# CV-Project2025/Project-NeRF

Hardware: AMD Instinct MI355X
Metric: train rays/sec + 800x800 render FPS, NeRF-Synthetic Lego; PSNR parity (higher is better)
Workload: dtype bf16; 1 GPU; Part 2 vanilla NeRF train step (L10/L4 Fourier, 8x256 skip-4 MLP, view 128), batch sampling included; rays_per_gpu=4096, samples_per_ray=64, global_rays=4096, parallelism=ray-dp1, weights=random init (seed 0), frames=100 x 800x800 RGBA resident in HBM (uniform noise)

## Files before the change

### include/nerf_hip.h

```cpp
#ifndef NERF_HIP_H
#define NERF_HIP_H

#include <stddef.h>
#include <stdint.h>

#ifdef __cplusplus
extern "C" {
#endif

#define NERF_OK 0
#define NERF_EINVAL (-22)
#define NERF_ELAUNCH (-5)
#define NERF_ENOSYS (-38)

#define NERF_ABI_VERSION 4

typedef void* nerf_stream_t;

const char* nerf_last_error(void);
int nerf_abi_version(void);

int nerf_set_option(const char* name, int value);
int nerf_get_option(const char* name, int* value_out);

int nerf_sample_rays(const float* rays_o, const float* rays_d, const float* u,
                     int64_t n_rays, int n_samples, float near_plane, float far_plane,
                     float* z_out, float* pts_out, float* dirs_out, nerf_stream_t stream);

int nerf_gather_rays(const float* images, const float* poses, const int64_t* img_idx, const int64_t* pix_y,
                     const int64_t* pix_x, int64_t batch, int n_images, int H, int W, float focal,
                     float scene_scale, float* rays_o, float* rays_d, float* rgba, nerf_stream_t stream);

int nerf_gather_batch(const float* images, const float* poses, const int64_t* flat_idx, int64_t batch, int n_images,
                      int H, int W, float focal, float scene_scale, const float* bg, float* rays_o, float* rays_d,
                      float* rgba, float* target, nerf_stream_t stream);

int nerf_train_batch(const float* images, const float* poses, int n_images, int H, int W, float focal,
                     float scene_scale, const float* bg, uint64_t seed, uint64_t counter, int64_t batch,
                     int n_samples, float near_plane, float far_plane, int perturb, float* rays_o, float* rays_d,
                     float* rgba, float* target, float* z_out, nerf_stream_t stream);

int nerf_train_batch_shard(const float* images, const float* poses, int n_images, int H, int W, float focal,
                     float scene_scale, const float* bg, uint64_t seed, uint64_t counter, int64_t first_ray, int64_t batch,
                     int n_samples, float near_plane, float far_plane, int perturb, float* rays_o, float* rays_d,
                     float* rgba, float* target, float* z_out, nerf_stream_t stream);

int nerf_active_mask(const float* pts, int64_t n, const uint8_t* binary_grid, int resolution,
                     float bound, uint8_t* mask_out, int64_t* idx_out, nerf_stream_t stream);

int nerf_sample_compact(const float* rays_o, const float* rays_d, const float* u, int64_t n_rays,
                        int n_samples, float near_plane, float far_plane, const uint8_t* binary_grid,
                        int resolution, float bound, float* z_out, int* slot_of_sample, float* pts_compact,
                        float* dirs_compact, unsigned* active_count, nerf_stream_t stream);
int nerf_sample_compact_jitter(const float* rays_o, const float* rays_d, uint64_t seed, uint64_t counter,
                               int64_t n_rays, int n_samples, float near_plane, float far_plane,
                               const uint8_t* binary_grid, int resolution, float bound, float* z_out,
                               int* slot_of_sample, float* pts_compact, float* dirs_compact,
                               unsigned* active_count, nerf_stream_t stream);
int nerf_sample_compact_jitter_shard(const float* rays_o, const float* rays_d, uint64_t seed, uint64_t counter,
                                     int64_t first_ray, int64_t n_rays, int n_samples, float near_plane, float far_plane,
                                     const uint8_t* binary_grid, int resolution, float bound, float* z_out,
                                     int* slot_of_sample, float* pts_compact, float* dirs_compact,
                                     unsigned* active_count, nerf_stream_t stream);
#define NERF_COMPACT_CHAIN_WORDS 40
int nerf_sample_compact_jitter_chain(const float* rays_o, const float* rays_d, uint64_t seed, uint64_t counter,
                                     int64_t first_ray, int64_t n_rays, int n_samples, float near_plane, float far_plane,
                                     const uint8_t* binary_grid, int resolution, float bound, float* z_out,
                                     int* slot_of_sample, float* pts_compact, float* dirs_compact,
                                     unsigned* chain_state, int turn, unsigned* count_host, unsigned seq, nerf_stream_t stream);

size_t nerf_sample_compact_ordered_scratch_bytes(int64_t n_rays, int n_samples);
int nerf_sample_compact_ordered(const float* rays_o, const float* rays_d, const float* u, int draw, uint64_t seed, uint64_t counter,
                                int64_t first_ray, int64_t n_rays, int n_samples, float near_plane, float far_plane,
                                const uint8_t* binary_grid, int resolution, float bound, float* z_out, int* slot_of_sample,
                                float* pts_compact, float* dirs_compact, unsigned* active_count, void* scratch,
                                size_t scratch_bytes, nerf_stream_t stream);

int nerf_sample_pdf(const float* z_coarse, const float* weights, const float* u, int64_t n_rays,
                    int n_coarse, int n_fine, float* z_out, nerf_stream_t stream);

int nerf_grid_lattice(float bound, int resolution, float* pts_out, nerf_stream_t stream);
int nerf_grid_update(const float* sigma, float* grid, uint8_t* binary_grid, int64_t n_cells,
                     float decay, int dynamic, float threshold, unsigned long long* active_count,
                     nerf_stream_t stream);

int nerf_fourier_encode(const float* x, int64_t n, int dim, int n_freq, float* out,
                        nerf_stream_t stream);

int nerf_composite_fwd(const float* rgb, const float* sigma, const float* z, const float* rays_d,
                       const float* bg, int64_t bg_rows, const float* extra,
                       int64_t n_rays, int n_samples,
                       float* out_rgb, float* out_depth, float* out_acc,
                       float* extra_map, float* weights_out, nerf_stream_t stream);

int nerf_composite_bwd(const float* rgb, const float* sigma, const float* z, const float* rays_d,
                       const float* bg, int64_t bg_rows, const float* extra,
                       const float* g_rgb, const float* g_depth, const float* g_acc,
                       const float* g_extra, int64_t n_rays, int n_samples,
                       float* d_rgb, float* d_sigma, float* d_extra, nerf_stream_t stream);

int nerf_composite_fwd_indexed(const float* rgb_compact, const float* sigma_compact, const int* slot_of_sample,
                               const float* z, const float* rays_d, const float* bg, int64_t bg_rows,
                               int64_t n_rays, int n_samples, float* out_rgb, float* out_depth,
                               float* out_acc, nerf_stream_t stream);
int nerf_composite_bwd_indexed(const float* rgb_compact, const float* sigma_compact, const int* slot_of_sample,
                               const float* z, const float* rays_d, const float* bg, int64_t bg_rows,
                               const float* g_rgb, const float* g_depth, const float* g_acc, int64_t n_rays,
                               int n_samples, float* d_rgb_compact, float* d_sigma_compact,
                               nerf_stream_t stream);

#define NERF_MLP_PARAM_COUNT 595844

size_t nerf_mlp_packed_bytes(void);
int nerf_mlp_pack(const float* params_f32, void* packed, nerf_stream_t stream);
int nerf_mlp_pack_streams(const float* params_f32, void* packed, int which, nerf_stream_t stream);

size_t nerf_mlp_stash_bytes(int64_t n);
int nerf_mlp_fwd(const void* packed, const float* rays_o, const float* rays_d, const float* z,
                 int64_t n, int n_samples, float* rgb, float* sigma, void* stash,
                 nerf_stream_t stream);

int nerf_mlp_fwd_encoded(const void* packed, const float* x_enc, const float* d_enc, int64_t n, float* rgb,
                         float* sigma, void* stash, nerf_stream_t stream);

size_t nerf_mlp_bwd_workspace_bytes(int64_t n);
int nerf_mlp_bwd(const void* packed, const void* stash, const float* rgb, const float* sigma,
                 const float* d_rgb, const float* d_sigma, int64_t n, float* grads_f32,
                 void* workspace, nerf_stream_t stream);
int nerf_mlp_bwd_dgrad(const void* packed, const void* stash, const float* rgb, const float* sigma,
                       const float* d_rgb, const float* d_sigma, int64_t n, void* workspace,
                       nerf_stream_t stream);
int nerf_mlp_bwd_dgrad_ex(const void* packed, const void* stash, const float* rgb, const float* sigma,
                          const float* d_rgb, const float* d_sigma, int64_t n, void* workspace,
                          const float* amax_dev, nerf_stream_t stream);
int64_t nerf_mlp_wgrad_part_split(void);
int nerf_mlp_bwd_wgrad_part(const void* stash, const void* workspace, int64_t n, float* grads_f32, int part,
                            nerf_stream_t stream);
int nerf_mlp_bwd_wgrad(const void* stash, const void* workspace, int64_t n, float* grads_f32,
                       nerf_stream_t stream);

int nerf_hash_encode_fwd(const float* pts, int64_t n, const float* table, int n_levels,
                         const float* scale_host, const unsigned* res_host, const unsigned* size_host,
                         const unsigned* offset_host, const unsigned* dense_host, float bound,
                         float* out_f32, void* out_nat_bf16, unsigned* idx_out, nerf_stream_t stream);
int nerf_hash_encode_fwd_f16(const float* pts, int64_t n, const void* table_f16, int n_levels,
                         const float* scale_host, const unsigned* res_host, const unsigned* size_host,
                         const unsigned* offset_host, const unsigned* dense_host, float bound,
                         float* out_f32, void* out_nat_bf16, nerf_stream_t stream);
int nerf_hash_encode_fwd_nat(const float* pts, int64_t n, const float* table_f32, const void* table_f16, int n_levels,
                             const float* scale_host, const unsigned* res_host, const unsigned* size_host,
                             const unsigned* offset_host, const unsigned* dense_host, float bound,
                             void* out_nat, int nat_dtype, nerf_stream_t stream);
int nerf_hash_encode_fwd_nat_tables(const float* pts, int64_t n, const void* tables_f16, int n_tables, int64_t table_stride,
                                    int n_levels, const float* scale_host, const unsigned* res_host, const unsigned* size_host,
                                    const unsigned* offset_host, const unsigned* dense_host, float bound, void* out_nat,
                                    int64_t out_stride_bytes, int nat_dtype, nerf_stream_t stream);
int nerf_f32_to_f16(const float* src, void* dst_f16, int64_t n, nerf_stream_t stream);
int nerf_hash_encode_bwd(const float* pts, int64_t n, int n_levels, const float* scale_host,
                         const unsigned* res_host, const unsigned* size_host, const unsigned* offset_host,
                         const unsigned* dense_host, float bound, const float* d_feat, float* d_table,
                         nerf_stream_t stream);
int nerf_hash_encode_bwd_levels(const float* pts, int64_t n, int n_levels, const float* scale_host,
                         const unsigned* res_host, const unsigned* size_host, const unsigned* offset_host,
                         const unsigned* dense_host, float bound, const float* d_feat, float* d_table, int first_level, int end_level,
                         nerf_stream_t stream);
size_t nerf_hash_encode_bwd_workspace_bytes(int64_t n, int n_levels);
int nerf_hash_encode_bwd_ws(const float* pts, int64_t n, int n_levels, const float* scale_host,
                         const unsigned* res_host, const unsigned* size_host, const unsigned* offset_host,
                         const unsigned* dense_host, float bound, const float* d_feat, float* d_table, int first_level, int end_level,
                         void* workspace, size_t workspace_bytes, nerf_stream_t stream);
int nerf_hash_encode_bwd_ws_store(const float* pts, int64_t n, int n_levels, const float* scale_host,
                                  const unsigned* res_host, const unsigned* size_host, const unsigned* offset_host,
                                  const unsigned* dense_host, float bound, const float* d_feat, float* d_table,
                                  int first_level, int end_level, void* workspace, size_t workspace_bytes,
                                  nerf_stream_t stream);
size_t nerf_hash_encode_bwd_tables_workspace_bytes(int64_t n, int n_levels, int n_tables);
int nerf_hash_encode_bwd_ws_store_tables(const float* pts, int64_t n, int n_tables, int64_t table_stride, int n_levels,
                                         const float* scale_host, const unsigned* res_host, const unsigned* size_host,
                                         const unsigned* offset_host, const unsigned* dense_host, float bound,
                                         const float* d_feat, int64_t dfeat_stride, float* d_table, void* workspace,
                                         size_t workspace_bytes, nerf_stream_t stream);
int nerf_hash_encode_bwd_ws_store_tables_spec(const float* pts, int64_t n, int n_tables, int64_t table_stride, int n_levels,
                                              const float* scale_host, const unsigned* res_host, const unsigned* size_host,
                                              const unsigned* offset_host, const unsigned* dense_host, float bound,
                                              const float* d_feat, int64_t dfeat_stride, float* d_table, void* workspace,
                                              size_t workspace_bytes, void* status_host, nerf_stream_t stream);
int nerf_hash_encode_fwd_f16_hist(const float* pts, int64_t n, const void* table_f16, int n_levels,
                                  const float* scale_host, const unsigned* res_host, const unsigned* size_host,
                                  const unsigned* offset_host, const unsigned* dense_host, float bound,
                                  void* out_nat_bf16, void* bwd_workspace, size_t bwd_workspace_bytes, nerf_stream_t stream);
#define NERF_AMAX_WORDS 32
int nerf_hash_encode_bwd_ws_slots(void* workspace, int64_t n, int n_levels, void** amax_bits_out, void** grad_lm_out);
int nerf_hash_encode_bwd_ws_store_precounted(const float* pts, int64_t n, int n_levels, const float* scale_host,
                                             const unsigned* res_host, const unsigned* size_host,
                                             const unsigned* offset_host, const unsigned* dense_host, float bound,
                                             float* d_table, void* workspace, size_t workspace_bytes, nerf_stream_t stream);
int nerf_hash_encode_bwd_spec_begin(void* workspace, nerf_stream_t stream);
int nerf_hash_encode_bwd_ws_store_spec(const float* pts, int64_t n, int n_levels, const float* scale_host,
                                       const unsigned* res_host, const unsigned* size_host, const unsigned* offset_host,
                                       const unsigned* dense_host, float bound, const float* d_feat, float* d_table, void* workspace,
                                       size_t workspace_bytes, void* status_host, nerf_stream_t stream);
int nerf_imlp_bwd_amax(const void* packed, void* workspace, const float* rgb, const float* sigma, const float* d_rgb,
                       const float* d_sigma, int64_t n, float* grads_f32, float* d_feat, void* amax_bits, nerf_stream_t stream);
const void* nerf_hash_encode_bwd_spec_status(const void* workspace);

int nerf_hash_encode_bwd_input(const float* pts, int64_t n, const float* table, int n_levels,
                               const float* scale_host, const unsigned* res_host, const unsigned* size_host,
                               const unsigned* offset_host, const unsigned* dense_host, float bound,
                               const float* d_feat, float* d_pts, nerf_stream_t stream);
int nerf_hash_encode_bwd_input_f16(const float* pts, int64_t n, const void* table_f16, int n_levels,
                                   const float* scale_host, const unsigned* res_host, const unsigned* size_host,
                                   const unsigned* offset_host, const unsigned* dense_host, float bound,
                                   const float* d_feat, float* d_pts, nerf_stream_t stream);
int nerf_hash_encode_bwd_input_f16_accum(const float* pts, int64_t n, const void* table_f16, int n_levels,
                                         const float* scale_host, const unsigned* res_host, const unsigned* size_host,
                                         const unsigned* offset_host, const unsigned* dense_host, float bound,
                                         const float* d_feat, float* d_pts, nerf_stream_t stream);
int nerf_hash_encode_bwd_input_lm_f16(const float* pts, int64_t n, const void* table_f16, int n_levels,
                                      const float* scale_host, const unsigned* res_host, const unsigned* size_host,
                                      const unsigned* offset_host, const unsigned* dense_host, float bound,
                                      const void* grad_lm, float* d_pts, int accumulate, nerf_stream_t stream);


size_t nerf_imlp_packed_bytes(void);
size_t nerf_imlp_workspace_bytes(int64_t n);
size_t nerf_imlp_hash_operand_offset(int64_t n);
int nerf_imlp_pack(const float* params_f32, void* packed, nerf_stream_t stream);
int nerf_imlp_fwd(const void* packed, void* workspace, const float* dirs, int64_t n, float* rgb,
                  float* sigma, int train, nerf_stream_t stream);
int nerf_imlp_fwd_encoded(const void* packed, void* workspace, const float* x_enc, const float* d_enc, int64_t n,
                          float* rgb, float* sigma, int train, nerf_stream_t stream);
int nerf_imlp_bwd(const void* packed, void* workspace, const float* rgb, const float* sigma,
                  const float* d_rgb, const float* d_sigma, int64_t n, float* grads_f32,
                  float* d_feat, nerf_stream_t stream);
int nerf_imlp_bwd_lm(const void* packed, void* workspace, const float* rgb, const float* sigma,
                     const float* d_rgb, const float* d_sigma, int64_t n, float* grads_f32,
                     void* grad_lm, void* amax_bits, nerf_stream_t stream);

size_t nerf_render_rays_workspace_bytes(int64_t chunk_rays, int n_samples);
int nerf_render_rays_fwd(const void* packed, const float* rays_o, const float* rays_d, int64_t n_rays,
                         int n_samples, float near_plane, float far_plane, const float* bg, int64_t bg_rows,
                         int64_t chunk_rays, void* workspace, float* out_rgb, float* out_depth, float* out_acc,
                         nerf_stream_t stream);

#define NERF_SUM_WS_FLOATS 12288
int nerf_composite_mse_bwd(const float* rgb, const float* sigma, const int* slot_of_sample, const float* z,
                           const float* rays_d, const float* bg, int64_t bg_rows, const float* target,
                           float loss_weight, int64_t n_rays, int n_samples, float* pred_out, float* loss_accum,
                           float* d_rgb, float* d_sigma, float* amax_accum, float* sum_ws, nerf_stream_t stream);
int nerf_composite_mse_reg_bwd(const float* rgb, const float* sigma, const int* slot_of_sample, const float* z,
                               const float* rays_d, const float* bg, int64_t bg_rows, const float* target,
                               float loss_weight, const float* extra, float reg_weight, int64_t n_rays, int n_samples,
                               float* pred_out, float* extra_map, float* loss_accum, float* reg_accum, float* d_rgb,
                               float* d_sigma, float* d_extra, float* sum_ws, nerf_stream_t stream);

int nerf_adam_step(float* params, const float* grads, float* exp_avg, float* exp_avg_sq,
                   int64_t n, int step, float lr, float beta1, float beta2, float eps,
                   float weight_decay, const float* grad_scale_dev, nerf_stream_t stream);

#define NERF_NORMSQ_WS_FLOATS 4136
int nerf_tv_normsq(const float* params, float* grads, int64_t n, float tv_weight, float grad_scale,
                   float* normsq_dev, nerf_stream_t stream);
int nerf_tv_normsq_accum(const float* params, float* grads, int64_t n, float tv_weight, float grad_scale,
                         float* normsq_dev, nerf_stream_t stream);
int nerf_tv_normsq_accum_tables(const float* params, float* grads, int64_t n, int n_tables, float tv_weight, float grad_scale,
                                float* normsq_dev, nerf_stream_t stream);
int nerf_adamw_clip_step(float* params, const float* grads, float* exp_avg, float* exp_avg_sq, int64_t n,
                         int step, float lr, float beta1, float beta2, float eps, float weight_decay,
                         const float* normsq_dev, float max_norm, float grad_scale, nerf_stream_t stream);
int nerf_adamw_clip_step_shadow(float* params, const float* grads, float* exp_avg, float* exp_avg_sq, int64_t n,
                         int step, float lr, float beta1, float beta2, float eps, float weight_decay,
                         const float* normsq_dev, float max_norm, float grad_scale, void* params_f16_out, nerf_stream_t stream);

size_t nerf_tv_codes_bytes(int64_t n);
int nerf_tv_normsq_codes(const float* params, const float* grads, int64_t n, int n_tables, float tv_weight, float grad_scale,
                         float* normsq_dev, int accumulate, void* tv_codes, nerf_stream_t stream);
int nerf_adamw_clip_step_tv(float* params, const float* grads, float* exp_avg, float* exp_avg_sq, int64_t n, int step, float lr,
                            float beta1, float beta2, float eps, float weight_decay, const float* normsq_dev, float max_norm,
                            float grad_scale, const void* tv_codes, int64_t tv_split, float tv_weight_lo, int64_t seg_lo,
                            float tv_weight_hi, int64_t seg_hi, int64_t lr_split, float lr_hi, void* params_f16_out,
                            nerf_stream_t stream);

int nerf_tv_normsq_codes_piece(const float* params, const float* grads, int64_t n, int64_t table_elems, int halo, float tv_weight,
                               float grad_scale, float* normsq_dev, int accumulate, void* tv_codes, nerf_stream_t stream);
int nerf_adamw_clip_step_tv_piece(float* params, const float* grads, float* exp_avg, float* exp_avg_sq, int64_t n, int step, float lr,
                                  float beta1, float beta2, float eps, float weight_decay, const float* normsq_dev, float max_norm,
                                  float grad_scale, const void* tv_codes, float tv_weight, int64_t table_elems, int halo_lo,
                                  void* params_f16_out, nerf_stream_t stream);

int nerf_clip_adamw_small(float* params, float* grads, float* exp_avg, float* exp_avg_sq, int64_t n, int step, float lr, float beta1,
                          float beta2, float eps, float weight_decay, float max_norm, float grad_scale, float* normsq_out,
                          int zero_grads, nerf_stream_t stream);

int64_t nerf_p4_param_count(void);
size_t nerf_p4_packed_bytes(void);
size_t nerf_p4_workspace_bytes(int64_t n);
size_t nerf_p4_workspace_offset(int64_t n, int which);
int nerf_p4_pack(const float* params_f32, void* packed, nerf_stream_t stream);
int nerf_p4_sample_inputs(const int* slot_of_sample, const float* pts_compact, const float* ray_times, int64_t n_rays,
                          int n_samples, float coord_noise_std, float time_noise_std, uint64_t seed, uint64_t counter,
                          int64_t first_ray, float* x_deform, float* t_deform, nerf_stream_t stream);
int nerf_p4_deform_fwd(const void* packed, const float* params_f32, void* workspace, const float* pts, const float* t_deform,
                       const float* blend, int64_t n, float* delta_x, float* x_canonical, int train, nerf_stream_t stream);
int nerf_p4_canon_fwd(const void* packed, void* workspace, const float* t_deform, const float* dirs, int64_t n, float* rgb,
                      float* sigma, int train, nerf_stream_t stream);
int nerf_p4_canon_bwd(const void* packed, void* workspace, const float* rgb, const float* sigma, const float* d_rgb,
                      const float* d_sigma, int64_t n, float* grads_f32, void* amax_bits, void* grad_lm, nerf_stream_t stream);
int nerf_p4_deform_bwd(const void* packed, const float* params_f32, void* workspace, const float* d_delta_x, int64_t n,
                       float* grads_f32, void* amax_bits, void* grad_lm, nerf_stream_t stream);

int64_t nerf_p3_deform_param_count(void);
size_t nerf_p3_deform_packed_bytes(void);
size_t nerf_p3_deform_workspace_bytes(int64_t n);
int nerf_p3_deform_pack(const float* params_f32, void* packed, nerf_stream_t stream);
int nerf_p3_deform_fwd(const void* packed, void* workspace, const float* x_code, const float* pts, const float* t_deform,
                       int64_t n, float* delta_x, float* x_canonical, int train, nerf_stream_t stream);
int nerf_p3_deform_bwd(const void* packed, void* workspace, const float* d_delta_x, int64_t n, float* grads_f32,
                       nerf_stream_t stream);

int64_t nerf_p3_canon_param_count(int time_dim);
size_t nerf_p3_canon_packed_bytes(void);
size_t nerf_p3_canon_workspace_bytes(int64_t n);
int nerf_p3_canon_pack(const float* params_f32, int time_dim, void* packed, nerf_stream_t stream);
int nerf_p3_canon_fwd(const void* packed, void* workspace, const float* x, const float* t, const float* dirs, int64_t n,
                      float* rgb, float* sigma, int train, nerf_stream_t stream);
int nerf_p3_canon_bwd(const void* packed, void* workspace, const float* x, const float* rgb, const float* sigma,
                      const float* d_rgb, const float* d_sigma, int64_t n, int time_dim, float* grads_f32, float* d_x,
                      nerf_stream_t stream);

#ifdef __cplusplus
}
#endif
#endif
```

### project-nerf_amd/_lib.py

```python
import ctypes
import os

_HERE = os.path.dirname(os.path.abspath(__file__))
LIB_PATH = os.path.join(_HERE, "libnerf_hip.so")

c_f32p = ctypes.c_void_p
c_ptr = ctypes.c_void_p
i64 = ctypes.c_int64
i32 = ctypes.c_int
f32 = ctypes.c_float
size_t = ctypes.c_size_t

PROTOTYPES = {
    "nerf_last_error": (ctypes.c_char_p, []),
    "nerf_abi_version": (i32, []),
    "nerf_set_option": (i32, [ctypes.c_char_p, i32]),
    "nerf_get_option": (i32, [ctypes.c_char_p, ctypes.POINTER(i32)]),
    "nerf_sample_rays": (i32, [c_ptr, c_ptr, c_ptr, i64, i32, f32, f32, c_ptr, c_ptr, c_ptr, c_ptr]),
    "nerf_gather_rays": (i32, [c_ptr, c_ptr, c_ptr, c_ptr, c_ptr, i64, i32, i32, i32, f32, f32, c_ptr, c_ptr, c_ptr, c_ptr]),
    "nerf_gather_batch": (i32, [c_ptr, c_ptr, c_ptr, i64, i32, i32, i32, f32, f32, c_ptr, c_ptr, c_ptr, c_ptr, c_ptr, c_ptr]),
    "nerf_train_batch": (i32, [c_ptr, c_ptr, i32, i32, i32, f32, f32, c_ptr, ctypes.c_uint64, ctypes.c_uint64, i64, i32, f32, f32,
                               i32, c_ptr, c_ptr, c_ptr, c_ptr, c_ptr, c_ptr]),
    "nerf_train_batch_shard": (i32, [c_ptr, c_ptr, i32, i32, i32, f32, f32, c_ptr, ctypes.c_uint64, ctypes.c_uint64, i64, i64, i32, f32, f32,
                                     i32, c_ptr, c_ptr, c_ptr, c_ptr, c_ptr, c_ptr]),
    "nerf_active_mask": (i32, [c_ptr, i64, c_ptr, i32, f32, c_ptr, c_ptr, c_ptr]),
    "nerf_sample_compact": (i32, [c_ptr, c_ptr, c_ptr, i64, i32, f32, f32, c_ptr, i32, f32, c_ptr, c_ptr, c_ptr, c_ptr, c_ptr, c_ptr]),
    "nerf_sample_compact_jitter": (i32, [c_ptr, c_ptr, ctypes.c_uint64, ctypes.c_uint64, i64, i32, f32, f32, c_ptr, i32, f32,
                                         c_ptr, c_ptr, c_ptr, c_ptr, c_ptr, c_ptr]),
    "nerf_sample_compact_jitter_shard": (i32, [c_ptr, c_ptr, ctypes.c_uint64, ctypes.c_uint64, i64, i64, i32, f32, f32, c_ptr, i32, f32,
                                               c_ptr, c_ptr, c_ptr, c_ptr, c_ptr, c_ptr]),
    "nerf_sample_compact_jitter_chain": (i32, [c_ptr, c_ptr, ctypes.c_uint64, ctypes.c_uint64, i64, i64, i32, f32, f32, c_ptr, i32, f32,
                                               c_ptr, c_ptr, c_ptr, c_ptr, c_ptr, i32, c_ptr, ctypes.c_uint32, c_ptr]),
    "nerf_composite_fwd_indexed": (i32, [c_ptr, c_ptr, c_ptr, c_ptr, c_ptr, c_ptr, i64, i64, i32, c_ptr, c_ptr, c_ptr, c_ptr]),
    "nerf_composite_bwd_indexed": (i32, [c_ptr, c_ptr, c_ptr, c_ptr, c_ptr, c_ptr, i64, c_ptr, c_ptr, c_ptr, i64, i32, c_ptr, c_ptr, c_ptr]),
    "nerf_sample_pdf": (i32, [c_ptr, c_ptr, c_ptr, i64, i32, i32, c_ptr, c_ptr]),
    "nerf_grid_lattice": (i32, [f32, i32, c_ptr, c_ptr]),
    "nerf_grid_update": (i32, [c_ptr, c_ptr, c_ptr, i64, f32, i32, f32, c_ptr, c_ptr]),
    "nerf_fourier_encode": (i32, [c_ptr, i64, i32, i32, c_ptr, c_ptr]),
    "nerf_composite_fwd": (i32, [c_ptr, c_ptr, c_ptr, c_ptr, c_ptr, i64, c_ptr, i64, i32,
                                 c_ptr, c_ptr, c_ptr, c_ptr, c_ptr, c_ptr]),
    "nerf_composite_bwd": (i32, [c_ptr, c_ptr, c_ptr, c_ptr, c_ptr, i64, c_ptr, c_ptr, c_ptr, c_ptr,
                                 c_ptr, i64, i32, c_ptr, c_ptr, c_ptr, c_ptr]),
    "nerf_render_rays_workspace_bytes": (size_t, [i64, i32]),
    "nerf_render_rays_fwd": (i32, [c_ptr, c_ptr, c_ptr, i64, i32, f32, f32, c_ptr, i64, i64, c_ptr, c_ptr, c_ptr, c_ptr, c_ptr]),
    "nerf_mlp_packed_bytes": (size_t, []),
    "nerf_mlp_pack": (i32, [c_ptr, c_ptr, c_ptr]),
    "nerf_mlp_pack_streams": (i32, [c_ptr, c_ptr, i32, c_ptr]),
    "nerf_mlp_stash_bytes": (size_t, [i64]),
    "nerf_mlp_fwd": (i32, [c_ptr, c_ptr, c_ptr, c_ptr, i64, i32, c_ptr, c_ptr, c_ptr, c_ptr]),
    "nerf_mlp_fwd_encoded": (i32, [c_ptr, c_ptr, c_ptr, i64, c_ptr, c_ptr, c_ptr, c_ptr]),
    "nerf_mlp_bwd_workspace_bytes": (size_t, [i64]),
    "nerf_mlp_bwd": (i32, [c_ptr, c_ptr, c_ptr, c_ptr, c_ptr, c_ptr, i64, c_ptr, c_ptr, c_ptr]),
    "nerf_mlp_bwd_dgrad": (i32, [c_ptr, c_ptr, c_ptr, c_ptr, c_ptr, c_ptr, i64, c_ptr, c_ptr]),
    "nerf_mlp_bwd_wgrad": (i32, [c_ptr, c_ptr, i64, c_ptr, c_ptr]),
    "nerf_mlp_bwd_dgrad_ex": (i32, [c_ptr, c_ptr, c_ptr, c_ptr, c_ptr, c_ptr, i64, c_ptr, c_ptr, c_ptr]),
    "nerf_composite_mse_bwd": (i32, [c_ptr, c_ptr, c_ptr, c_ptr, c_ptr, c_ptr, i64, c_ptr, f32, i64, i32, c_ptr, c_ptr,
                                     c_ptr, c_ptr, c_ptr, c_ptr, c_ptr]),
    "nerf_mlp_wgrad_part_split": (i64, []),
    "nerf_mlp_bwd_wgrad_part": (i32, [c_ptr, c_ptr, i64, c_ptr, i32, c_ptr]),
    "nerf_hash_encode_fwd": (i32, [c_ptr, i64, c_ptr, i32, c_ptr, c_ptr, c_ptr, c_ptr, c_ptr, f32, c_ptr, c_ptr, c_ptr, c_ptr]),
    "nerf_hash_encode_fwd_f16": (i32, [c_ptr, i64, c_ptr, i32, c_ptr, c_ptr, c_ptr, c_ptr, c_ptr, f32, c_ptr, c_ptr, c_ptr]),
    "nerf_hash_encode_fwd_nat": (i32, [c_ptr, i64, c_ptr, c_ptr, i32, c_ptr, c_ptr, c_ptr, c_ptr, c_ptr, f32, c_ptr, i32, c_ptr]),
    "nerf_hash_encode_fwd_nat_tables": (i32, [c_ptr, i64, c_ptr, i32, i64, i32, c_ptr, c_ptr, c_ptr, c_ptr, c_ptr, f32, c_ptr, i64, i32, c_ptr]),
    "nerf_f32_to_f16": (i32, [c_ptr, c_ptr, i64, c_ptr]),
    "nerf_hash_encode_bwd": (i32, [c_ptr, i64, i32, c_ptr, c_ptr, c_ptr, c_ptr, c_ptr, f32, c_ptr, c_ptr, c_ptr]),
    "nerf_hash_encode_bwd_levels": (i32, [c_ptr, i64, i32, c_ptr, c_ptr, c_ptr, c_ptr, c_ptr, f32, c_ptr, c_ptr, i32, i32, c_ptr]),
    "nerf_hash_encode_bwd_workspace_bytes": (size_t, [i64, i32]),
    "nerf_hash_encode_bwd_ws": (i32, [c_ptr, i64, i32, c_ptr, c_ptr, c_ptr, c_ptr, c_ptr, f32, c_ptr, c_ptr, i32, i32, c_ptr, size_t, c_ptr]),
    "nerf_hash_encode_bwd_ws_store": (i32, [c_ptr, i64, i32, c_ptr, c_ptr, c_ptr, c_ptr, c_ptr, f32, c_ptr, c_ptr, i32, i32, c_ptr, size_t, c_ptr]),
    "nerf_hash_encode_bwd_tables_workspace_bytes": (size_t, [i64, i32, i32]),
    "nerf_hash_encode_bwd_ws_store_tables": (i32, [c_ptr, i64, i32, i64, i32, c_ptr, c_ptr, c_ptr, c_ptr, c_ptr, f32, c_ptr, i64, c_ptr, c_ptr, size_t, c_ptr]),
    "nerf_hash_encode_bwd_ws_store_tables_spec": (i32, [c_ptr, i64, i32, i64, i32, c_ptr, c_ptr, c_ptr, c_ptr, c_ptr, f32, c_ptr, i64, c_ptr, c_ptr, size_t,
                                                        c_ptr, c_ptr]),
    "nerf_hash_encode_fwd_f16_hist": (i32, [c_ptr, i64, c_ptr, i32, c_ptr, c_ptr, c_ptr, c_ptr, c_ptr, f32, c_ptr, c_ptr, size_t, c_ptr]),
    "nerf_hash_encode_bwd_ws_slots": (i32, [c_ptr, i64, i32, ctypes.POINTER(c_ptr), ctypes.POINTER(c_ptr)]),
    "nerf_hash_encode_bwd_ws_store_precounted": (i32, [c_ptr, i64, i32, c_ptr, c_ptr, c_ptr, c_ptr, c_ptr, f32, c_ptr, c_ptr, size_t, c_ptr]),
    "nerf_hash_encode_bwd_spec_begin": (i32, [c_ptr, c_ptr]),
    "nerf_hash_encode_bwd_ws_store_spec": (i32, [c_ptr, i64, i32, c_ptr, c_ptr, c_ptr, c_ptr, c_ptr, f32, c_ptr, c_ptr, c_ptr, size_t, c_ptr, c_ptr]),
    "nerf_imlp_bwd_amax": (i32, [c_ptr, c_ptr, c_ptr, c_ptr, c_ptr, c_ptr, i64, c_ptr, c_ptr, c_ptr, c_ptr]),
    "nerf_hash_encode_bwd_spec_status": (c_ptr, [c_ptr]),
    "nerf_imlp_bwd_lm": (i32, [c_ptr, c_ptr, c_ptr, c_ptr, c_ptr, c_ptr, i64, c_ptr, c_ptr, c_ptr, c_ptr]),
    "nerf_hash_encode_bwd_input": (i32, [c_ptr, i64, c_ptr, i32, c_ptr, c_ptr, c_ptr, c_ptr, c_ptr, f32, c_ptr, c_ptr, c_ptr]),
    "nerf_hash_encode_bwd_input_f16": (i32, [c_ptr, i64, c_ptr, i32, c_ptr, c_ptr, c_ptr, c_ptr, c_ptr, f32, c_ptr, c_ptr, c_ptr]),
    "nerf_hash_encode_bwd_input_f16_accum": (i32, [c_ptr, i64, c_ptr, i32, c_ptr, c_ptr, c_ptr, c_ptr, c_ptr, f32, c_ptr, c_ptr, c_ptr]),
    "nerf_hash_encode_bwd_input_lm_f16": (i32, [c_ptr, i64, c_ptr, i32, c_ptr, c_ptr, c_ptr, c_ptr, c_ptr, f32, c_ptr, c_ptr, i32, c_ptr]),
    "nerf_imlp_packed_bytes": (size_t, []),
    "nerf_imlp_workspace_bytes": (size_t, [i64]),
    "nerf_imlp_hash_operand_offset": (size_t, [i64]),
    "nerf_imlp_pack": (i32, [c_ptr, c_ptr, c_ptr]),
    "nerf_imlp_fwd": (i32, [c_ptr, c_ptr, c_ptr, i64, c_ptr, c_ptr, i32, c_ptr]),
    "nerf_imlp_fwd_encoded": (i32, [c_ptr, c_ptr, c_ptr, c_ptr, i64, c_ptr, c_ptr, i32, c_ptr]),
    "nerf_imlp_bwd": (i32, [c_ptr, c_ptr, c_ptr, c_ptr, c_ptr, c_ptr, i64, c_ptr, c_ptr, c_ptr]),
    "nerf_adam_step": (i32, [c_ptr, c_ptr, c_ptr, c_ptr, i64, i32, f32, f32, f32, f32, f32, c_ptr, c_ptr]),
    "nerf_tv_normsq": (i32, [c_ptr, c_ptr, i64, f32, f32, c_ptr, c_ptr]),
    "nerf_tv_normsq_accum": (i32, [c_ptr, c_ptr, i64, f32, f32, c_ptr, c_ptr]),
    "nerf_tv_normsq_accum_tables": (i32, [c_ptr, c_ptr, i64, i32, f32, f32, c_ptr, c_ptr]),
    "nerf_composite_mse_reg_bwd": (i32, [c_ptr, c_ptr, c_ptr, c_ptr, c_ptr, c_ptr, i64, c_ptr, f32, c_ptr, f32, i64, i32, c_ptr, c_ptr,
                                         c_ptr, c_ptr, c_ptr, c_ptr, c_ptr, c_ptr, c_ptr]),
    "nerf_sample_compact_ordered_scratch_bytes": (size_t, [i64, i32]),
    "nerf_sample_compact_ordered": (i32, [c_ptr, c_ptr, c_ptr, i32, ctypes.c_uint64, ctypes.c_uint64, i64, i64, i32, f32, f32, c_ptr, i32, f32,
                                          c_ptr, c_ptr, c_ptr, c_ptr, c_ptr, c_ptr, size_t, c_ptr]),
    "nerf_p4_param_count": (i64, []),
    "nerf_p4_packed_bytes": (size_t, []),
    "nerf_p4_workspace_bytes": (size_t, [i64]),
    "nerf_p4_workspace_offset": (size_t, [i64, i32]),
    "nerf_p4_pack": (i32, [c_ptr, c_ptr, c_ptr]),
    "nerf_p4_sample_inputs": (i32, [c_ptr, c_ptr, c_ptr, i64, i32, f32, f32, ctypes.c_uint64, ctypes.c_uint64, i64, c_ptr, c_ptr, c_ptr]),
    "nerf_p4_deform_fwd": (i32, [c_ptr, c_ptr, c_ptr, c_ptr, c_ptr, c_ptr, i64, c_ptr, c_ptr, i32, c_ptr]),
    "nerf_p4_canon_fwd": (i32, [c_ptr, c_ptr, c_ptr, c_ptr, i64, c_ptr, c_ptr, i32, c_ptr]),
    "nerf_p4_canon_bwd": (i32, [c_ptr, c_ptr, c_ptr, c_ptr, c_ptr, c_ptr, i64, c_ptr, c_ptr, c_ptr, c_ptr]),
    "nerf_p4_deform_bwd": (i32, [c_ptr, c_ptr, c_ptr, c_ptr, i64, c_ptr, c_ptr, c_ptr, c_ptr]),
    "nerf_p3_deform_param_count": (i64, []),
    "nerf_p3_deform_packed_bytes": (size_t, []),
    "nerf_p3_deform_workspace_bytes": (size_t, [i64]),
    "nerf_p3_deform_pack": (i32, [c_ptr, c_ptr, c_ptr]),
    "nerf_p3_deform_fwd": (i32, [c_ptr, c_ptr, c_ptr, c_ptr, c_ptr, i64, c_ptr, c_ptr, i32, c_ptr]),
    "nerf_p3_deform_bwd": (i32, [c_ptr, c_ptr, c_ptr, i64, c_ptr, c_ptr]),
    "nerf_p3_canon_param_count": (i64, [i32]),
    "nerf_p3_canon_packed_bytes": (size_t, []),
    "nerf_p3_canon_workspace_bytes": (size_t, [i64]),
    "nerf_p3_canon_pack": (i32, [c_ptr, i32, c_ptr, c_ptr]),
    "nerf_p3_canon_fwd": (i32, [c_ptr, c_ptr, c_ptr, c_ptr, c_ptr, i64, c_ptr, c_ptr, i32, c_ptr]),
    "nerf_p3_canon_bwd": (i32, [c_ptr, c_ptr, c_ptr, c_ptr, c_ptr, c_ptr, c_ptr, i64, i32, c_ptr, c_ptr, c_ptr]),
    "nerf_tv_codes_bytes": (size_t, [i64]),
    "nerf_tv_normsq_codes": (i32, [c_ptr, c_ptr, i64, i32, f32, f32, c_ptr, i32, c_ptr, c_ptr]),
    "nerf_clip_adamw_small": (i32, [c_ptr, c_ptr, c_ptr, c_ptr, i64, i32, f32, f32, f32, f32, f32, f32, f32, c_ptr, i32, c_ptr]),
    "nerf_adamw_clip_step_tv": (i32, [c_ptr, c_ptr, c_ptr, c_ptr, i64, i32, f32, f32, f32, f32, f32, c_ptr, f32, f32, c_ptr, i64, f32, i64,
                                      f32, i64, i64, f32, c_ptr, c_ptr]),
    "nerf_tv_normsq_codes_piece": (i32, [c_ptr, c_ptr, i64, i64, i32, f32, f32, c_ptr, i32, c_ptr, c_ptr]),
    "nerf_adamw_clip_step_tv_piece": (i32, [c_ptr, c_ptr, c_ptr, c_ptr, i64, i32, f32, f32, f32, f32, f32, c_ptr, f32, f32, c_ptr, f32, i64, i32,
                                            c_ptr, c_ptr]),
    "nerf_adamw_clip_step": (i32, [c_ptr, c_ptr, c_ptr, c_ptr, i64, i32, f32, f32, f32, f32, f32, c_ptr, f32, f32, c_ptr]),
    "nerf_adamw_clip_step_shadow": (i32, [c_ptr, c_ptr, c_ptr, c_ptr, i64, i32, f32, f32, f32, f32, f32, c_ptr, f32, f32, c_ptr, c_ptr]),
}

ABI_VERSION = 4

_lib = None


class NerfHipError(RuntimeError):
    pass


def load():
    global _lib
    if _lib is not None:
        return _lib
    if not os.path.exists(LIB_PATH):
        raise NerfHipError(
            f"{LIB_PATH} not found: build it with `python project-nerf_amd/build.py` "
            "(hipcc --offload-arch=gfx950).  There is no fallback path.")
    import torch
    lib = ctypes.CDLL(LIB_PATH, mode=ctypes.RTLD_GLOBAL)
    for name, (res, args) in PROTOTYPES.items():
        fn = getattr(lib, name)
        fn.restype = res
        fn.argtypes = args
    if lib.nerf_abi_version() != ABI_VERSION:
        raise NerfHipError(f"ABI version mismatch: {LIB_PATH} reports {lib.nerf_abi_version()}, this binding was written against "
                           f"{ABI_VERSION} (rebuild with `python project-nerf_amd/build.py`)")
    _lib = lib
    return lib


NORMSQ_WS_FLOATS = 4136
COMPACT_CHAIN_WORDS = 40
SUM_WS_FLOATS = 12288


def set_option(name: str, value: int) -> None:
    check(load().nerf_set_option(name.encode(), int(value)), f"nerf_set_option({name})")


def get_option(name: str) -> int:
    out = i32(0)
    check(load().nerf_get_option(name.encode(), ctypes.byref(out)), f"nerf_get_option({name})")
    return out.value


def check(code, what):
    if code != 0:
        msg = load().nerf_last_error().decode("utf-8", "replace")
        raise NerfHipError(f"{what} failed ({code}): {msg}")
```

### project-nerf_amd/csrc/adam.hip

```cpp
#include "common.h"

namespace nerf {

typedef float f4 __attribute__((ext_vector_type(4)));

__device__ __forceinline__ void adam_update(float& p, float g, float& m, float& v, float lr, float beta1, float beta2,
                                            float eps, float wd, float inv_bc1, float inv_sqrt_bc2) {
  float pi = p;
  if (wd != 0.0f) pi *= (1.0f - lr * wd);
  const float mi = beta1 * m + (1.0f - beta1) * g;
  const float vi = beta2 * v + (1.0f - beta2) * g * g;
  m = mi;
  v = vi;
  p = pi - (lr * inv_bc1) * (mi / (sqrtf(vi) * inv_sqrt_bc2 + eps));
}

template <bool VEC>
__device__ __forceinline__ void adam_sweep(float* __restrict__ p, const float* __restrict__ g, float* __restrict__ m,
                                           float* __restrict__ v, int64_t n, float gs, float lr, float beta1, float beta2,
                                           float eps, float wd, float inv_bc1, float inv_sqrt_bc2, _Float16* __restrict__ shadow = nullptr) {
  const int64_t tid = blockIdx.x * (int64_t)blockDim.x + threadIdx.x, stride = (int64_t)gridDim.x * blockDim.x;
  const int64_t n4 = VEC ? n / 4 : 0;
  for (int64_t i = tid; i < n4; i += stride) {
    f4 pp = reinterpret_cast<f4*>(p)[i], mm = reinterpret_cast<f4*>(m)[i], vv = reinterpret_cast<f4*>(v)[i];
    const f4 gg = reinterpret_cast<const f4*>(g)[i];
#pragma unroll
    for (int e = 0; e < 4; ++e) {
      float pe = pp[e], me = mm[e], ve = vv[e];
      adam_update(pe, gg[e] * gs, me, ve, lr, beta1, beta2, eps, wd, inv_bc1, inv_sqrt_bc2);
      pp[e] = pe; mm[e] = me; vv[e] = ve;
    }
    reinterpret_cast<f4*>(m)[i] = mm;
    reinterpret_cast<f4*>(v)[i] = vv;
    reinterpret_cast<f4*>(p)[i] = pp;
    if (shadow != nullptr) {
      typedef _Float16 h4 __attribute__((ext_vector_type(4)));
      h4 hh = {(_Float16)pp[0], (_Float16)pp[1], (_Float16)pp[2], (_Float16)pp[3]};
      reinterpret_cast<h4*>(shadow)[i] = hh;
    }
  }
  for (int64_t i = 4 * n4 + tid; i < n; i += stride) {
    adam_update(p[i], g[i] * gs, m[i], v[i], lr, beta1, beta2, eps, wd, inv_bc1, inv_sqrt_bc2);
    if (shadow != nullptr) shadow[i] = (_Float16)p[i];
  }
}

template <bool VEC>
__global__ void __launch_bounds__(256)
adam_kernel(float* __restrict__ p, const float* __restrict__ g, float* __restrict__ m,
            float* __restrict__ v, int64_t n, float lr, float beta1, float beta2, float eps, float wd,
            float inv_bc1, float inv_sqrt_bc2, const float* __restrict__ grad_scale) {
  adam_sweep<VEC>(p, g, m, v, n, grad_scale ? *grad_scale : 1.0f, lr, beta1, beta2, eps, wd, inv_bc1, inv_sqrt_bc2);
}

__host__ inline bool aligned16(const void* a, const void* b, const void* c, const void* d) {
  return (((uintptr_t)a | (uintptr_t)b | (uintptr_t)c | (uintptr_t)d) & 15) == 0;
}

}

extern "C" int nerf_adam_step(float* params, const float* grads, float* exp_avg, float* exp_avg_sq,
                              int64_t n, int step, float lr, float beta1, float beta2, float eps,
                              float weight_decay, const float* grad_scale_dev, nerf_stream_t stream) {
  NERF_REQUIRE(n >= 0 && step >= 1, "nerf_adam_step: n=%lld step=%d", (long long)n, step);
  if (n == 0) return NERF_OK;
  NERF_REQUIRE(params && grads && exp_avg && exp_avg_sq, "nerf_adam_step: NULL pointer");
  const double bc1 = 1.0 - pow((double)beta1, step), bc2 = 1.0 - pow((double)beta2, step);
  int64_t blocks = (n / 4 + 255) / 256 + 1;
  if (blocks > 2048) blocks = 2048;
  if (nerf::aligned16(params, grads, exp_avg, exp_avg_sq))
    hipLaunchKernelGGL(nerf::adam_kernel<true>, dim3((int)blocks), dim3(256), 0, nerf::as_stream(stream), params,
                       grads, exp_avg, exp_avg_sq, n, lr, beta1, beta2, eps, weight_decay,
                       (float)(1.0 / bc1), (float)(1.0 / sqrt(bc2)), grad_scale_dev);
  else
    hipLaunchKernelGGL(nerf::adam_kernel<false>, dim3((int)blocks), dim3(256), 0, nerf::as_stream(stream), params,
                       grads, exp_avg, exp_avg_sq, n, lr, beta1, beta2, eps, weight_decay,
                       (float)(1.0 / bc1), (float)(1.0 / sqrt(bc2)), grad_scale_dev);
  return nerf::check_launch("nerf_adam_step");
}

namespace nerf {

__device__ __forceinline__ float sgn(float x) { return (x > 0.0f) - (x < 0.0f); }

__device__ __forceinline__ float tv_term(float prev, float cur, float next, bool has_prev, bool has_next) {
  float t = 0.0f;
  if (has_prev) t += sgn(cur - prev);
  if (has_next) t -= sgn(next - cur);
  return t;
}

template <bool VEC>
__global__ void __launch_bounds__(256)
tv_normsq_kernel(const float* __restrict__ p, float* __restrict__ g, int64_t n, float tv_scale, float grad_scale,
                 float* __restrict__ normsq, int64_t seg) {
  auto starts = [seg](int64_t e) { return e == 0 || e == seg || e == 2 * seg || e == 3 * seg; };
  const bool rewrite = tv_scale != 0.0f || grad_scale != 1.0f;
  float local = 0.0f;
  const int64_t tid = blockIdx.x * (int64_t)blockDim.x + threadIdx.x, stride = (int64_t)gridDim.x * blockDim.x;
  const int64_t n4 = VEC ? n / 4 : 0;
  for (int64_t i = tid; i < n4; i += stride) {
    f4 gg = reinterpret_cast<f4*>(g)[i];
    gg[0] *= grad_scale; gg[1] *= grad_scale; gg[2] *= grad_scale; gg[3] *= grad_scale;
    if (tv_scale != 0.0f) {
      const f4 pp = reinterpret_cast<const f4*>(p)[i];
      const int64_t e0 = 4 * i;
      const bool has_prev = !starts(e0), has_next = e0 + 4 < n && !starts(e0 + 4);
      const float before = has_prev ? p[e0 - 1] : 0.0f, after = has_next ? p[e0 + 4] : 0.0f;
      gg[0] += tv_scale * tv_term(before, pp[0], pp[1], has_prev, true);
      gg[1] += tv_scale * tv_term(pp[0], pp[1], pp[2], true, true);
      gg[2] += tv_scale * tv_term(pp[1], pp[2], pp[3], true, true);
      gg[3] += tv_scale * tv_term(pp[2], pp[3], after, true, has_next);
    }
    if (rewrite) reinterpret_cast<f4*>(g)[i] = gg;
    local += gg[0] * gg[0] + gg[1] * gg[1] + gg[2] * gg[2] + gg[3] * gg[3];
  }
  for (int64_t i = 4 * n4 + tid; i < n; i += stride) {
    float gi = g[i] * grad_scale;
    if (tv_scale != 0.0f) {
      const bool has_prev = !starts(i), has_next = i + 1 < n && !starts(i + 1);
      gi += tv_scale * tv_term(has_prev ? p[i - 1] : 0.0f, p[i], has_next ? p[i + 1] : 0.0f, has_prev, has_next);
    }
    if (rewrite) g[i] = gi;
    local += gi * gi;
  }
  __shared__ float part[4];
  local = wave_sum(local);
  if ((threadIdx.x & 63) == 0) part[threadIdx.x >> 6] = local;
  __syncthreads();
  const float val[1] = {(part[0] + part[1]) + (part[2] + part[3])};
  float* const out[1] = {normsq};
  ordered_block_sum<1>(val, out, reinterpret_cast<unsigned*>(normsq + 1));
}

template <bool VEC>
__global__ void __launch_bounds__(256)
adamw_clip_kernel(float* __restrict__ p, const float* __restrict__ g, float* __restrict__ m, float* __restrict__ v,
                  int64_t n, float lr, float beta1, float beta2, float eps, float wd, float inv_bc1,
                  float inv_sqrt_bc2, const float* __restrict__ normsq, float max_norm, float extra_scale,
                  _Float16* __restrict__ shadow) {
  float gs = extra_scale;
  if (normsq != nullptr && max_norm > 0.0f) {
    const float coef = max_norm / (sqrtf(*normsq * extra_scale * extra_scale) + 1e-6f);
    gs *= coef < 1.0f ? coef : 1.0f;
  }
  adam_sweep<VEC>(p, g, m, v, n, gs, lr, beta1, beta2, eps, wd, inv_bc1, inv_sqrt_bc2, shadow);
}

__device__ __forceinline__ int tv_code_at(const uint8_t* __restrict__ codes, int64_t i) {
  return i < 0 ? 0 : (int)((codes[i >> 2] >> (2 * (int)(i & 3))) & 3u) - 1;
}

__global__ void __launch_bounds__(256)
tv_normsq_codes_kernel(const float* __restrict__ p, const float* __restrict__ g, int64_t n, float tv_scale, float grad_scale,
                       float* __restrict__ normsq, int64_t seg, uint8_t* __restrict__ codes, int accumulate) {
  auto starts = [seg](int64_t e) { return e == 0 || e == seg || e == 2 * seg || e == 3 * seg; };
  float local = 0.0f;
  const int64_t n4 = (n + 3) / 4;
  for (int64_t q = blockIdx.x * (int64_t)blockDim.x + threadIdx.x; q < n4; q += (int64_t)gridDim.x * blockDim.x) {
    const int64_t e0 = 4 * q;
    float pp[6], gg[4];
#pragma unroll
    for (int e = 0; e < 4; ++e) { pp[1 + e] = e0 + e < n ? p[e0 + e] : 0.0f; gg[e] = e0 + e < n ? g[e0 + e] : 0.0f; }
    if (tv_scale != 0.0f) {
      pp[0] = e0 > 0 ? p[e0 - 1] : 0.0f;
      pp[5] = e0 + 4 < n ? p[e0 + 4] : 0.0f;
      unsigned byte = 0;
      int s_prev = !starts(e0) ? (int)sgn(pp[1] - pp[0]) : 0;
// ... 407 lines not shown
```

### project-nerf_amd/csrc/composite.hip

```cpp
#include "common.h"

namespace nerf {

constexpr int kMaxPerLane = 16;

template <int K>
struct RayCtx {
  float e[K];
  float alpha[K];
  float q[K];
  float T[K];
  float z[K];
  float delta[K];
};

__device__ __forceinline__ int64_t row_of(const int* __restrict__ slots, int64_t dense_index) {
  return slots == nullptr ? dense_index : (int64_t)slots[dense_index];
}

template <int K>
__device__ __forceinline__ void ray_setup(const float* __restrict__ sigma, const float* __restrict__ z,
                                          const float* __restrict__ rays_d, const int* __restrict__ slots,
                                          int64_t r, int S, int lane, RayCtx<K>& c, float* sig_out, int64_t* row_out) {
  const float dx = rays_d[r * 3 + 0], dy = rays_d[r * 3 + 1], dz = rays_d[r * 3 + 2];
// ... 25 lines not shown
    local *= c.q[k];
  }
  const float incl = wave_inclusive_prod(local);
  float run = dpp_row_shr<1>(incl, 1.0f);
  {
    const float p15 = lane_read(incl, 15), p31 = lane_read(incl, 31), p47 = lane_read(incl, 47);
    if (lane == 16) run = p15;
    if (lane == 32) run = p31;
    if (lane == 48) run = p47;
    if (lane == 0) run = 1.0f;
  }
#pragma unroll
  for (int k = 0; k < K; ++k) {
    c.T[k] = run;
    run *= c.q[k];
  }
}

template <int K>
__global__ void __launch_bounds__(256)
composite_fwd_kernel(const float* __restrict__ rgb, const float* __restrict__ sigma,
                     const float* __restrict__ z, const float* __restrict__ rays_d,
                     const float* __restrict__ bg, int64_t bg_rows, const float* __restrict__ extra,
                     const int* __restrict__ slots, int64_t R, int S, float* __restrict__ out_rgb,
                     float* __restrict__ out_depth, float* __restrict__ out_acc, float* __restrict__ extra_map,
                     float* __restrict__ weights_out) {
  const int lane = threadIdx.x & 63;
  const int64_t wave = (blockIdx.x * (int64_t)blockDim.x + threadIdx.x) >> 6;
  const int64_t nwave = ((int64_t)gridDim.x * blockDim.x) >> 6;
  for (int64_t r = wave; r < R; r += nwave) {
    RayCtx<K> c;
    float sg[K];
    int64_t row[K];
    ray_setup<K>(sigma, z, rays_d, slots, r, S, lane, c, sg, row);
    float a0 = 0.f, a1 = 0.f, a2 = 0.f, ad = 0.f, aw = 0.f, x0 = 0.f, x1 = 0.f, x2 = 0.f;
#pragma unroll
    for (int k = 0; k < K; ++k) {
      const int s = lane * K + k;
      if (s < S) {
        const float w = c.alpha[k] * c.T[k];
        if (row[k] >= 0) {
          const float* p = rgb + row[k] * 3;
          a0 += w * p[0];
          a1 += w * p[1];
          a2 += w * p[2];
        }
        ad += w * c.z[k];
        aw += w;
        if (extra != nullptr && row[k] >= 0) {
          const float* q = extra + row[k] * 3;
          x0 += w * q[0];
          x1 += w * q[1];
          x2 += w * q[2];
        }
        if (weights_out != nullptr) weights_out[r * S + s] = w;
      }
    }
    a0 = wave_sum(a0); a1 = wave_sum(a1); a2 = wave_sum(a2);
    ad = wave_sum(ad); aw = wave_sum(aw);
    if (extra != nullptr) { x0 = wave_sum(x0); x1 = wave_sum(x1); x2 = wave_sum(x2); }
    if (lane == 0) {
      if (bg != nullptr) {
        const float* b = bg + (bg_rows > 1 ? r * 3 : 0);
        const float rest = 1.0f - aw;
        a0 += rest * b[0];
        a1 += rest * b[1];
        a2 += rest * b[2];
      }
      out_rgb[r * 3 + 0] = a0;
      out_rgb[r * 3 + 1] = a1;
      out_rgb[r * 3 + 2] = a2;
      out_depth[r] = ad;
      out_acc[r] = aw;
      if (extra_map != nullptr) {
        extra_map[r * 3 + 0] = x0;
        extra_map[r * 3 + 1] = x1;
        extra_map[r * 3 + 2] = x2;
      }
    }
  }
}

template <int K>
__global__ void __launch_bounds__(256)
composite_bwd_kernel(const float* __restrict__ rgb, const float* __restrict__ sigma,
                     const float* __restrict__ z, const float* __restrict__ rays_d,
                     const float* __restrict__ bg, int64_t bg_rows, const float* __restrict__ extra,
                     const float* __restrict__ g_rgb, const float* __restrict__ g_depth,
                     const float* __restrict__ g_acc, const float* __restrict__ g_extra,
                     const int* __restrict__ slots, int64_t R, int S,
                     float* __restrict__ d_rgb, float* __restrict__ d_sigma, float* __restrict__ d_extra) {
  const int lane = threadIdx.x & 63;
  const int64_t wave = (blockIdx.x * (int64_t)blockDim.x + threadIdx.x) >> 6;
  const int64_t nwave = ((int64_t)gridDim.x * blockDim.x) >> 6;
  for (int64_t r = wave; r < R; r += nwave) {
    RayCtx<K> c;
    float sg[K];
    int64_t row[K];
    ray_setup<K>(sigma, z, rays_d, slots, r, S, lane, c, sg, row);
    const float gr0 = g_rgb[r * 3 + 0], gr1 = g_rgb[r * 3 + 1], gr2 = g_rgb[r * 3 + 2];
    const float gd = g_depth ? g_depth[r] : 0.0f;
    float ga = g_acc ? g_acc[r] : 0.0f;
    if (bg != nullptr) {
      const float* b = bg + (bg_rows > 1 ? r * 3 : 0);
      ga -= gr0 * b[0] + gr1 * b[1] + gr2 * b[2];
    }
    float gx0 = 0.f, gx1 = 0.f, gx2 = 0.f;
    if (g_extra != nullptr) { gx0 = g_extra[r * 3 + 0]; gx1 = g_extra[r * 3 + 1]; gx2 = g_extra[r * 3 + 2]; }
    float G[K], w[K];
    float local = 0.0f;
#pragma unroll
    for (int k = 0; k < K; ++k) {
      const int s = lane * K + k;
      G[k] = 0.0f;
      w[k] = 0.0f;
      if (s < S) {
        w[k] = c.alpha[k] * c.T[k];
        float g = gd * c.z[k] + ga;
        if (row[k] >= 0) {
          const float* p = rgb + row[k] * 3;
          g += gr0 * p[0] + gr1 * p[1] + gr2 * p[2];
          float* o = d_rgb + row[k] * 3;
          o[0] = w[k] * gr0;
          o[1] = w[k] * gr1;
          o[2] = w[k] * gr2;
        }
        if (extra != nullptr && g_extra != nullptr && row[k] >= 0) {
          const float* q = extra + row[k] * 3;
          g += gx0 * q[0] + gx1 * q[1] + gx2 * q[2];
          if (d_extra != nullptr) {
            float* oe = d_extra + row[k] * 3;
            oe[0] = w[k] * gx0;
            oe[1] = w[k] * gx1;
            oe[2] = w[k] * gx2;
          }
        }
        G[k] = g;
        local += g * w[k];
      }
    }
    float after = wave_exclusive_suffix_sum(local);
#pragma unroll
    for (int k = K - 1; k >= 0; --k) {
      const int s = lane * K + k;
      if (s < S && row[k] >= 0) {
        const float dalpha = G[k] * c.T[k] - after / c.q[k];
        d_sigma[row[k]] = dalpha * c.delta[k] * c.e[k];
      }
      after += G[k] * w[k];
    }
  }
}

template <int K>
__global__ void __launch_bounds__(256)
composite_mse_bwd_kernel(const float* __restrict__ rgb, const float* __restrict__ sigma, const float* __restrict__ z,
                         const float* __restrict__ rays_d, const float* __restrict__ bg, int64_t bg_rows,
                         const float* __restrict__ target, float loss_weight, const int* __restrict__ slots, int64_t R, int S,
                         float* __restrict__ pred_out, float* __restrict__ loss_out, float* __restrict__ d_rgb,
                         float* __restrict__ d_sigma, float* __restrict__ amax_out,
                         const float* __restrict__ extra, float reg_weight, float* __restrict__ d_extra,
                         float* __restrict__ reg_out, float* __restrict__ extra_map, unsigned* __restrict__ sum_ws) {
  const int lane = threadIdx.x & 63;
  const int64_t wave = (blockIdx.x * (int64_t)blockDim.x + threadIdx.x) >> 6;
  const int64_t nwave = ((int64_t)gridDim.x * blockDim.x) >> 6;
  float loss_local = 0.0f, amax = 0.0f, reg_local = 0.0f;
  for (int64_t r = wave; r < R; r += nwave) {
    RayCtx<K> c;
    float sg[K];
    int64_t row[K];
    ray_setup<K>(sigma, z, rays_d, slots, r, S, lane, c, sg, row);
    float col[K][3], w[K];
    float a0 = 0.f, a1 = 0.f, a2 = 0.f, aw = 0.f;
    float m0 = 0.f, m1 = 0.f, m2 = 0.f;
#pragma unroll
    for (int k = 0; k < K; ++k) {
      const int s = lane * K + k;
      w[k] = 0.0f;
      col[k][0] = col[k][1] = col[k][2] = 0.0f;
      if (s < S) {
        w[k] = c.alpha[k] * c.T[k];
        if (row[k] >= 0) {
          const float* p = rgb + row[k] * 3;
          col[k][0] = p[0]; col[k][1] = p[1]; col[k][2] = p[2];
          a0 += w[k] * p[0]; a1 += w[k] * p[1]; a2 += w[k] * p[2];
          if (extra != nullptr) {
            const float* e = extra + row[k] * 3;
            m0 += w[k] * e[0]; m1 += w[k] * e[1]; m2 += w[k] * e[2];
          }
        }
        aw += w[k];
      }
    }
    a0 = wave_sum(a0); a1 = wave_sum(a1); a2 = wave_sum(a2); aw = wave_sum(aw);
    float gm0 = 0.f, gm1 = 0.f, gm2 = 0.f;
    if (extra != nullptr) {
      m0 = wave_sum(m0); m1 = wave_sum(m1); m2 = wave_sum(m2);
      gm0 = 2.0f * reg_weight * m0; gm1 = 2.0f * reg_weight * m1; gm2 = 2.0f * reg_weight * m2;
      if (lane == 0) {
        reg_local += reg_weight * (m0 * m0 + m1 * m1 + m2 * m2);
        if (extra_map != nullptr) { extra_map[r * 3 + 0] = m0; extra_map[r * 3 + 1] = m1; extra_map[r * 3 + 2] = m2; }
      }
    }
    float b0 = 0.f, b1 = 0.f, b2 = 0.f;
    if (bg != nullptr) {
      const float* b = bg + (bg_rows > 1 ? r * 3 : 0);
      b0 = b[0]; b1 = b[1]; b2 = b[2];
      const float rest = 1.0f - aw;
      a0 += rest * b0; a1 += rest * b1; a2 += rest * b2;
    }
    const float e0 = a0 - target[r * 3 + 0], e1 = a1 - target[r * 3 + 1], e2 = a2 - target[r * 3 + 2];
    if (lane == 0) {
      loss_local += (e0 * e0 + e1 * e1 + e2 * e2) * loss_weight;
      if (pred_out != nullptr) { pred_out[r * 3 + 0] = a0; pred_out[r * 3 + 1] = a1; pred_out[r * 3 + 2] = a2; }
    }
    const float gr0 = 2.0f * e0 * loss_weight, gr1 = 2.0f * e1 * loss_weight, gr2 = 2.0f * e2 * loss_weight;
    const float ga = -(gr0 * b0 + gr1 * b1 + gr2 * b2);
    float G[K], local = 0.0f;
#pragma unroll
    for (int k = 0; k < K; ++k) {
      const int s = lane * K + k;
      G[k] = 0.0f;
      if (s < S) {
        float g = ga;
        if (row[k] >= 0) {
          g += gr0 * col[k][0] + gr1 * col[k][1] + gr2 * col[k][2];
          if (extra != nullptr) {
            const float* e = extra + row[k] * 3;
            g += gm0 * e[0] + gm1 * e[1] + gm2 * e[2];
            float* oe = d_extra + row[k] * 3;
            oe[0] = w[k] * gm0; oe[1] = w[k] * gm1; oe[2] = w[k] * gm2;
          }
          float* o = d_rgb + row[k] * 3;
          const float d0 = w[k] * gr0, d1 = w[k] * gr1, d2 = w[k] * gr2;
          o[0] = d0; o[1] = d1; o[2] = d2;
          if (amax_out != nullptr)
            amax = fmaxf(amax, fmaxf(fabsf(d0 * col[k][0] * (1.0f - col[k][0])),
                                     fmaxf(fabsf(d1 * col[k][1] * (1.0f - col[k][1])), fabsf(d2 * col[k][2] * (1.0f - col[k][2])))));
        }
        G[k] = g;
        local += g * w[k];
      }
    }
    float after = wave_exclusive_suffix_sum(local);
#pragma unroll
    for (int k = K - 1; k >= 0; --k) {
      const int s = lane * K + k;
      if (s < S && row[k] >= 0) {
        const float dalpha = G[k] * c.T[k] - after / c.q[k];
        const float ds = dalpha * c.delta[k] * c.e[k];
        d_sigma[row[k]] = ds;
        if (amax_out != nullptr && sg[k] > 0.0f) amax = fmaxf(amax, fabsf(ds));
      }
      after += G[k] * w[k];
    }
  }
  __shared__ float part[12];
  loss_local = wave_sum(loss_local);
  reg_local = wave_sum(reg_local);
#pragma unroll
  for (int off = 32; off > 0; off >>= 1) amax = fmaxf(amax, __shfl_xor(amax, off));
  if (lane == 0) { part[threadIdx.x >> 6] = loss_local; part[4 + (threadIdx.x >> 6)] = amax; part[8 + (threadIdx.x >> 6)] = reg_local; }
  __syncthreads();
  if (sum_ws != nullptr) {
    if (threadIdx.x == 0) {
      float* ws = reinterpret_cast<float*>(sum_ws);
      ws[blockIdx.x] = (part[0] + part[1]) + (part[2] + part[3]);
      ws[gridDim.x + blockIdx.x] = (part[8] + part[9]) + (part[10] + part[11]);
      ws[2 * gridDim.x + blockIdx.x] = fmaxf(fmaxf(part[4], part[5]), fmaxf(part[6], part[7]));
    }
    return;
  }
  if (threadIdx.x == 0) {
    atomicAdd(loss_out, (part[0] + part[1]) + (part[2] + part[3]));
    if (reg_out != nullptr) atomicAdd(reg_out, (part[8] + part[9]) + (part[10] + part[11]));
    if (amax_out != nullptr) {
      const float m = fmaxf(fmaxf(part[4], part[5]), fmaxf(part[6], part[7]));
      if (m == m && m < 3.0e38f) atomicMax(reinterpret_cast<unsigned*>(amax_out), __builtin_bit_cast(unsigned, m));
    }
  }
}

__global__ void __launch_bounds__(256) composite_sums_kernel(const float* __restrict__ ws, int n_blocks, float* __restrict__ loss_out,
                                                             float* __restrict__ reg_out, float* __restrict__ amax_out) {
  __shared__ float part[3][4];
  float s0 = 0.0f, s1 = 0.0f, m = 0.0f;
  for (int b = threadIdx.x; b < n_blocks; b += 256) {
    s0 += ws[b];
    s1 += ws[n_blocks + b];
    const float v = ws[2 * n_blocks + b];
    if (v == v && v < 3.0e38f) m = fmaxf(m, v);
  }
  s0 = wave_sum(s0);
  s1 = wave_sum(s1);
#pragma unroll
  for (int off = 32; off > 0; off >>= 1) m = fmaxf(m, __shfl_xor(m, off));
  if ((threadIdx.x & 63) == 0) { part[0][threadIdx.x >> 6] = s0; part[1][threadIdx.x >> 6] = s1; part[2][threadIdx.x >> 6] = m; }
  __syncthreads();
  if (threadIdx.x == 0) {
    *loss_out += (part[0][0] + part[0][1]) + (part[0][2] + part[0][3]);
    if (reg_out != nullptr) *reg_out += (part[1][0] + part[1][1]) + (part[1][2] + part[1][3]);
    if (amax_out != nullptr) *amax_out = fmaxf(*amax_out, fmaxf(fmaxf(part[2][0], part[2][1]), fmaxf(part[2][2], part[2][3])));
  }
}

static int per_lane(int S) {
  const int k = (S + 63) / 64;
  return k <= 4 ? k : (k <= 6 ? 6 : (k <= 8 ? 8 : (k <= 12 ? 12 : 16)));
}

}

using namespace nerf;

#define DISPATCH_K(K, KERNEL, ...)                                                        \
  switch (K) {                                                                            \
    case 1: hipLaunchKernelGGL(KERNEL<1>, grid, dim3(256), 0, as_stream(stream), __VA_ARGS__); break; \
    case 2: hipLaunchKernelGGL(KERNEL<2>, grid, dim3(256), 0, as_stream(stream), __VA_ARGS__); break; \
    case 3: hipLaunchKernelGGL(KERNEL<3>, grid, dim3(256), 0, as_stream(stream), __VA_ARGS__); break; \
    case 4: hipLaunchKernelGGL(KERNEL<4>, grid, dim3(256), 0, as_stream(stream), __VA_ARGS__); break; \
    case 6: hipLaunchKernelGGL(KERNEL<6>, grid, dim3(256), 0, as_stream(stream), __VA_ARGS__); break; \
    case 8: hipLaunchKernelGGL(KERNEL<8>, grid, dim3(256), 0, as_stream(stream), __VA_ARGS__); break; \
    case 12: hipLaunchKernelGGL(KERNEL<12>, grid, dim3(256), 0, as_stream(stream), __VA_ARGS__); break; \
    default: hipLaunchKernelGGL(KERNEL<16>, grid, dim3(256), 0, as_stream(stream), __VA_ARGS__); break; \
  }

static int composite_fwd_impl(const float* rgb, const float* sigma, const float* z, const float* rays_d,
                              const float* bg, int64_t bg_rows, const float* extra, const int* slots,
                              int64_t n_rays, int n_samples, float* out_rgb, float* out_depth, float* out_acc,
                              float* extra_map, float* weights_out, nerf_stream_t stream) {
  NERF_REQUIRE(n_rays >= 0 && n_samples >= 1 && n_samples <= 64 * kMaxPerLane,
               "nerf_composite_fwd: n_rays=%lld n_samples=%d (max %d)", (long long)n_rays, n_samples,
               64 * kMaxPerLane);
  if (n_rays == 0) return NERF_OK;
  NERF_REQUIRE(rgb && sigma && z && rays_d && out_rgb && out_depth && out_acc,
               "nerf_composite_fwd: NULL pointer");
  NERF_REQUIRE(bg == nullptr || bg_rows == 1 || bg_rows == n_rays, "nerf_composite_fwd: bg_rows=%lld",
               (long long)bg_rows);
  NERF_REQUIRE((extra == nullptr) == (extra_map == nullptr), "nerf_composite_fwd: extra/extra_map mismatch");
  int64_t blocks = (n_rays + 3) / 4;
  if (blocks > 256 * 8) blocks = 256 * 8;
  const dim3 grid((int)blocks);
  DISPATCH_K(per_lane(n_samples), composite_fwd_kernel, rgb, sigma, z, rays_d, bg, bg_rows, extra, slots, n_rays,
             n_samples, out_rgb, out_depth, out_acc, extra_map, weights_out);
  return check_launch("nerf_composite_fwd");
}

extern "C" int nerf_composite_fwd(const float* rgb, const float* sigma, const float* z,
                                  const float* rays_d, const float* bg, int64_t bg_rows,
                                  const float* extra, int64_t n_rays, int n_samples, float* out_rgb,
                                  float* out_depth, float* out_acc, float* extra_map,
                                  float* weights_out, nerf_stream_t stream) {
  return composite_fwd_impl(rgb, sigma, z, rays_d, bg, bg_rows, extra, nullptr, n_rays, n_samples, out_rgb, out_depth,
                            out_acc, extra_map, weights_out, stream);
}

extern "C" int nerf_composite_fwd_indexed(const float* rgb_compact, const float* sigma_compact, const int* slot_of_sample,
                                          const float* z, const float* rays_d, const float* bg, int64_t bg_rows,
                                          int64_t n_rays, int n_samples, float* out_rgb, float* out_depth,
                                          float* out_acc, nerf_stream_t stream) {
  NERF_REQUIRE(n_rays == 0 || slot_of_sample != nullptr, "nerf_composite_fwd_indexed: slot map is NULL");
  return composite_fwd_impl(rgb_compact, sigma_compact, z, rays_d, bg, bg_rows, nullptr, slot_of_sample, n_rays, n_samples,
                            out_rgb, out_depth, out_acc, nullptr, nullptr, stream);
}

static int composite_bwd_impl(const float* rgb, const float* sigma, const float* z, const float* rays_d,
                              const float* bg, int64_t bg_rows, const float* extra, const float* g_rgb,
                              const float* g_depth, const float* g_acc, const float* g_extra, const int* slots,
                              int64_t n_rays, int n_samples, float* d_rgb, float* d_sigma, float* d_extra,
                              nerf_stream_t stream) {
  NERF_REQUIRE(n_rays >= 0 && n_samples >= 1 && n_samples <= 64 * kMaxPerLane,
               "nerf_composite_bwd: n_rays=%lld n_samples=%d", (long long)n_rays, n_samples);
  if (n_rays == 0) return NERF_OK;
  NERF_REQUIRE(rgb && sigma && z && rays_d && g_rgb && d_rgb && d_sigma, "nerf_composite_bwd: NULL pointer");
  NERF_REQUIRE(bg == nullptr || bg_rows == 1 || bg_rows == n_rays, "nerf_composite_bwd: bg_rows=%lld",
               (long long)bg_rows);
  int64_t blocks = (n_rays + 3) / 4;
  if (blocks > 256 * 8) blocks = 256 * 8;
  const dim3 grid((int)blocks);
  DISPATCH_K(per_lane(n_samples), composite_bwd_kernel, rgb, sigma, z, rays_d, bg, bg_rows, extra, g_rgb,
             g_depth, g_acc, g_extra, slots, n_rays, n_samples, d_rgb, d_sigma, d_extra);
  return check_launch("nerf_composite_bwd");
}

extern "C" int nerf_composite_bwd(const float* rgb, const float* sigma, const float* z,
                                  const float* rays_d, const float* bg, int64_t bg_rows,
                                  const float* extra, const float* g_rgb, const float* g_depth,
                                  const float* g_acc, const float* g_extra, int64_t n_rays,
                                  int n_samples, float* d_rgb, float* d_sigma, float* d_extra,
                                  nerf_stream_t stream) {
  return composite_bwd_impl(rgb, sigma, z, rays_d, bg, bg_rows, extra, g_rgb, g_depth, g_acc, g_extra, nullptr, n_rays,
                            n_samples, d_rgb, d_sigma, d_extra, stream);
}

extern "C" int nerf_composite_bwd_indexed(const float* rgb_compact, const float* sigma_compact, const int* slot_of_sample,
                                          const float* z, const float* rays_d, const float* bg, int64_t bg_rows,
                                          const float* g_rgb, const float* g_depth, const float* g_acc, int64_t n_rays,
                                          int n_samples, float* d_rgb_compact, float* d_sigma_compact,
                                          nerf_stream_t stream) {
  NERF_REQUIRE(n_rays == 0 || slot_of_sample != nullptr, "nerf_composite_bwd_indexed: slot map is NULL");
  return composite_bwd_impl(rgb_compact, sigma_compact, z, rays_d, bg, bg_rows, nullptr, g_rgb, g_depth, g_acc, nullptr,
                            slot_of_sample, n_rays, n_samples, d_rgb_compact, d_sigma_compact, nullptr, stream);
}

static int64_t mse_blocks(int64_t n_rays, bool partials) {
  int n_cu = 256;
  (void)device_cu_count(&n_cu);
  const int per_cu = partials ? 8 : (options().composite_wgs_per_cu < 1 ? 1 : options().composite_wgs_per_cu);
  int64_t cap = (int64_t)n_cu * per_cu;
  if (cap > kOrderedSumMaxBlocks) cap = kOrderedSumMaxBlocks;
  const int64_t blocks = (n_rays + 3) / 4;
  return blocks < cap ? blocks : cap;
}
static int finish_sums(const float* sum_ws, unsigned n_blocks, float* loss, float* reg, float* amax, nerf_stream_t stream) {
  static_assert(NERF_SUM_WS_FLOATS >= 3 * kOrderedSumMaxBlocks, "three partials per workgroup");
  if (sum_ws == nullptr) return NERF_OK;
  hipLaunchKernelGGL(composite_sums_kernel, dim3(1), dim3(256), 0, as_stream(stream), sum_ws, (int)n_blocks, loss, reg, amax);
  return check_launch("nerf_composite_mse_bwd (sums)");
}

extern "C" int nerf_composite_mse_bwd(const float* rgb, const float* sigma, const int* slot_of_sample, const float* z,
                                      const float* rays_d, const float* bg, int64_t bg_rows, const float* target,
                                      float loss_weight, int64_t n_rays, int n_samples, float* pred_out, float* loss_accum,
                                      float* d_rgb, float* d_sigma, float* amax_accum, float* sum_ws, nerf_stream_t stream) {
  NERF_REQUIRE(n_rays >= 0 && n_samples >= 1 && n_samples <= 64 * kMaxPerLane,
               "nerf_composite_mse_bwd: n_rays=%lld n_samples=%d (max %d)", (long long)n_rays, n_samples, 64 * kMaxPerLane);
  if (n_rays == 0) return NERF_OK;
  NERF_REQUIRE(rgb && sigma && z && rays_d && target && loss_accum && d_rgb && d_sigma, "nerf_composite_mse_bwd: NULL pointer");
  NERF_REQUIRE(bg == nullptr || bg_rows == 1 || bg_rows == n_rays, "nerf_composite_mse_bwd: bg_rows=%lld", (long long)bg_rows);
  const dim3 grid((unsigned)mse_blocks(n_rays, sum_ws != nullptr));
  DISPATCH_K(per_lane(n_samples), composite_mse_bwd_kernel, rgb, sigma, z, rays_d, bg, bg_rows, target, loss_weight,
             slot_of_sample, n_rays, n_samples, pred_out, loss_accum, d_rgb, d_sigma, amax_accum,
             (const float*)nullptr, 0.0f, (float*)nullptr, (float*)nullptr, (float*)nullptr, reinterpret_cast<unsigned*>(sum_ws));
  if (int rc = check_launch("nerf_composite_mse_bwd"); rc != NERF_OK) return rc;
  return finish_sums(sum_ws, grid.x, loss_accum, nullptr, amax_accum, stream);
}

extern "C" int nerf_composite_mse_reg_bwd(const float* rgb, const float* sigma, const int* slot_of_sample, const float* z,
                                          const float* rays_d, const float* bg, int64_t bg_rows, const float* target,
                                          float loss_weight, const float* extra, float reg_weight, int64_t n_rays, int n_samples,
                                          float* pred_out, float* extra_map, float* loss_accum, float* reg_accum, float* d_rgb,
                                          float* d_sigma, float* d_extra, float* sum_ws, nerf_stream_t stream) {
  NERF_REQUIRE(n_rays >= 0 && n_samples >= 1 && n_samples <= 64 * kMaxPerLane,
               "nerf_composite_mse_reg_bwd: n_rays=%lld n_samples=%d (max %d)", (long long)n_rays, n_samples, 64 * kMaxPerLane);
  if (n_rays == 0) return NERF_OK;
  NERF_REQUIRE(rgb && sigma && z && rays_d && target && loss_accum && d_rgb && d_sigma && extra && d_extra && reg_accum,
               "nerf_composite_mse_reg_bwd: NULL pointer");
  NERF_REQUIRE(bg == nullptr || bg_rows == 1 || bg_rows == n_rays, "nerf_composite_mse_reg_bwd: bg_rows=%lld", (long long)bg_rows);
  const dim3 grid((unsigned)mse_blocks(n_rays, sum_ws != nullptr));
  DISPATCH_K(per_lane(n_samples), composite_mse_bwd_kernel, rgb, sigma, z, rays_d, bg, bg_rows, target, loss_weight,
             slot_of_sample, n_rays, n_samples, pred_out, loss_accum, d_rgb, d_sigma, (float*)nullptr, extra, reg_weight, d_extra,
             reg_accum, extra_map, reinterpret_cast<unsigned*>(sum_ws));
  if (int rc = check_launch("nerf_composite_mse_reg_bwd"); rc != NERF_OK) return rc;
  return finish_sums(sum_ws, grid.x, loss_accum, reg_accum, nullptr, stream);
}
```

### project-nerf_amd/csrc/mlp_bwd.hip

```cpp
#include "mlp_chain.h"
#include "mlp_stash.h"

namespace nerf {
using namespace plan;

struct BwdArgs {
  const char* packed;
  const float* rgb;
  const float* sigma;
  const float* d_rgb;
  const float* d_sigma;
  int64_t n, n_pad;
  const uint4* st_mask;
  __bf16* dsmall;
  __bf16* dhv;
  __bf16* dfeat;
  __bf16* dh;
  float* amax;
  const float* amax_src;
};

__device__ __forceinline__ void out_derivs(const BwdArgs& a, int64_t n, float& g0, float& g1, float& g2, float& gs) {
  const float r0 = a.rgb[n * 3 + 0], r1 = a.rgb[n * 3 + 1], r2 = a.rgb[n * 3 + 2];
  g0 = a.d_rgb[n * 3 + 0] * r0 * (1.0f - r0);
  g1 = a.d_rgb[n * 3 + 1] * r1 * (1.0f - r1);
  g2 = a.d_rgb[n * 3 + 2] * r2 * (1.0f - r2);
  gs = a.sigma[n] > 0.0f ? a.d_sigma[n] : 0.0f;
}

__global__ void __launch_bounds__(256) bwd_amax_kernel(const BwdArgs a) {
  float m = 0.0f;
  for (int64_t n = blockIdx.x * 256 + threadIdx.x; n < a.n; n += (int64_t)gridDim.x * 256) {
    float g0, g1, g2, gs;
    out_derivs(a, n, g0, g1, g2, gs);
    m = fmaxf(fmaxf(m, fabsf(g0)), fmaxf(fmaxf(fabsf(g1), fabsf(g2)), fabsf(gs)));
  }
#pragma unroll
  for (int off = 32; off > 0; off >>= 1) m = fmaxf(m, __shfl_xor(m, off));
  __shared__ float part[4];
  if ((threadIdx.x & 63) == 0) part[threadIdx.x >> 6] = m;
  __syncthreads();
  if (threadIdx.x == 0) {
    m = fmaxf(fmaxf(part[0], part[1]), fmaxf(part[2], part[3]));
    if (m == m && m < 3.0e38f) atomicMax(reinterpret_cast<unsigned*>(a.amax), __builtin_bit_cast(unsigned, m));
  }
}

__global__ void __launch_bounds__(kChainThreads, 2) mlp_bwd_kernel(const BwdArgs a) {
  extern __shared__ __attribute__((aligned(16))) char smem[];
  const int tid = threadIdx.x, lane = tid & 63;
  const int wave = __builtin_amdgcn_readfirstlane(tid >> 6);
  const int col = lane & 31, half = lane >> 5;

  WeightRing<true> ring;
  ring.init(a.packed + kPackBwdOff, smem + kBiasLdsBytes, wave, lane);
  ring.prologue();
  const char* a_base = nullptr;

  const int64_t n_tiles = a.n_pad / kTileSamples;
  for (int64_t tile = blockIdx.x; tile < n_tiles; tile += gridDim.x) {
    const bool more = tile + gridDim.x < n_tiles;
    const int64_t wave_tile = tile * 8 + wave;
    const int64_t n = wave_tile * kWaveSamples + col;
    const bool live = n < a.n;

    float g0 = 0.f, g1 = 0.f, g2 = 0.f, gs = 0.f;
    if (live) out_derivs(a, n, g0, g1, g2, gs);
    bf16x8 small;
#pragma unroll
    for (int j = 0; j < 8; ++j) small[j] = (__bf16)0.0f;
    if (half == 0) {
      small[0] = (__bf16)g0; small[1] = (__bf16)g1; small[2] = (__bf16)g2; small[3] = (__bf16)gs;
    }
    stash_nat(a.dsmall, wave_tile, 1, 0, col, half, small);

    uint4 mask;
    auto load_mask = [&](int layer) { mask = a.st_mask[(tile * 9 + layer) * kChainThreads + tid]; };
    auto grad_epi = [&](bf16x8* out, __bf16* stash, int width, bool masked) {
      return [=, &mask](auto mc, f32x16 acc) {
        constexpr int m = decltype(mc)::value;
        if (masked) {
          const uint32_t words[4] = {mask.x, mask.y, mask.z, mask.w};
          const uint32_t bits = words[m >> 1] >> (16 * (m & 1));
#pragma unroll
          for (int r = 0; r < 16; ++r) acc[r] = (bits >> r) & 1u ? acc[r] : 0.0f;
        }
        acc_to_operand(acc, out[2 * m], out[2 * m + 1]);
        stash_block(stash, wave_tile, width / 32, m, col, half, out[2 * m], out[2 * m + 1]);
      };
    };

    bf16x8 gA[16], gB[16];
    {
      bf16x8 in[1];
      in[0] = small;
      if (half == 0) in[0][3] = (__bf16)0.0f;
      load_mask(8);
      run_step<true, B_RGB, 1, true>(ring, a_base, more, in, nullptr, half, grad_epi(gA, a.dhv, 128, true));
    }
    {
      bf16x8 in[8];
#pragma unroll
      for (int i = 0; i < 8; ++i) in[i] = gA[i];
      run_step<true, B_VIEW, 8, true>(ring, a_base, more, in, nullptr, half, grad_epi(gB, a.dfeat, 256, false));
    }
    {
      bf16x8 in[17];
#pragma unroll
      for (int i = 0; i < 16; ++i) in[i] = gB[i];
#pragma unroll
      for (int j = 0; j < 8; ++j) in[16][j] = (__bf16)0.0f;
      if (half == 0) in[16][0] = (__bf16)gs;
      load_mask(7);
      run_step<true, B_HEAD, 17, true>(ring, a_base, more, in, nullptr, half, grad_epi(gA, a.dh + 7 * a.n_pad * 256, 256, true));
    }
    load_mask(6);
    run_step<true, B_PTS7, 16, true>(ring, a_base, more, gA, nullptr, half, grad_epi(gB, a.dh + 6 * a.n_pad * 256, 256, true));
    load_mask(5);
    run_step<true, B_PTS6, 16, true>(ring, a_base, more, gB, nullptr, half, grad_epi(gA, a.dh + 5 * a.n_pad * 256, 256, true));
    load_mask(4);
    run_step<true, B_PTS5, 16, true>(ring, a_base, more, gA, nullptr, half, grad_epi(gB, a.dh + 4 * a.n_pad * 256, 256, true));
    load_mask(3);
    run_step<true, B_PTS4, 16, true>(ring, a_base, more, gB, nullptr, half, grad_epi(gA, a.dh + 3 * a.n_pad * 256, 256, true));
    load_mask(2);
    run_step<true, B_PTS3, 16, true>(ring, a_base, more, gA, nullptr, half, grad_epi(gB, a.dh + 2 * a.n_pad * 256, 256, true));
    load_mask(1);
    run_step<true, B_PTS2, 16, true>(ring, a_base, more, gB, nullptr, half, grad_epi(gA, a.dh + 1 * a.n_pad * 256, 256, true));
    load_mask(0);
    run_step<true, B_PTS1, 16, true>(ring, a_base, more, gA, nullptr, half, grad_epi(gB, a.dh + 0 * a.n_pad * 256, 256, true));
  }
}

}

#include <stddef.h>
#include "mlp_stream_asm.h"

namespace nerf {

static_assert(offsetof(BwdArgs, n_pad) == 48 && offsetof(BwdArgs, st_mask) == 56 && offsetof(BwdArgs, dhv) == 72 &&
              offsetof(BwdArgs, dfeat) == 80 && offsetof(BwdArgs, dh) == 88, "kernarg offsets used by the stream asm");

template <bool IMG16>
__global__ void __launch_bounds__(kChainThreads, 2) mlp_bwd_stream_kernel(const BwdArgs a) {
  extern __shared__ __attribute__((aligned(16))) char smem[];
  const int tid = threadIdx.x, lane = tid & 63;
  const int wave = __builtin_amdgcn_readfirstlane(tid >> 6);
  const int col = lane & 31, half = lane >> 5;

  WeightRing<true> ring;
  ring.init(a.packed + kPackBwdOff, smem + kBiasLdsBytes, wave, lane);
  ring.template issue<0>(0);
  ring.template issue<1>(1);
  asm volatile("s_waitcnt vmcnt(0)" ::: "memory");
  __syncthreads();

  const unsigned ab0 = lds_addr(smem + kBiasLdsBytes) + 16u * lane, ab1 = ab0 + kRingSlotBytes;
  const unsigned ldsw = __builtin_amdgcn_readfirstlane(lds_addr(smem + kBiasLdsBytes) + 1024u * wave);
  const unsigned voff = 1024u * wave + 16u * lane;
  const char* src = a.packed + kPackBwdOff;
  const void* karg = (const void*)__builtin_amdgcn_kernarg_segment_ptr();

  float gscale = 1.0f;
  if constexpr (!IMG16) {
    set_fp8_saturate();
    const float amax_in = *a.amax_src;
    if (a.amax_src != a.amax && blockIdx.x == 0 && tid == 0) *a.amax = amax_in;
    gscale = __builtin_bit_cast(float, __builtin_amdgcn_readfirstlane(__builtin_bit_cast(int, grad_image_scale(amax_in))));
  }
  const int64_t n_tiles = a.n_pad / kTileSamples;
  for (int64_t tile = blockIdx.x; tile < n_tiles; tile += gridDim.x) {
    const int64_t wave_tile = tile * 8 + wave;
    const int64_t n = wave_tile * kWaveSamples + col;
    const bool live = n < a.n;
    float g0 = 0.f, g1 = 0.f, g2 = 0.f, gs = 0.f;
    if (live) out_derivs(a, n, g0, g1, g2, gs);
    bf16x8 small, in_rgb, in_sigma;
#pragma unroll
    for (int j = 0; j < 8; ++j) small[j] = in_sigma[j] = (__bf16)0.0f;
    if (half == 0) {
      small[0] = (__bf16)g0; small[1] = (__bf16)g1; small[2] = (__bf16)g2; small[3] = (__bf16)gs;
      in_sigma[0] = (__bf16)gs;
    }
    if constexpr (IMG16) stash_nat(a.dsmall, wave_tile, 1, 0, col, half, small);
    else stash_nat8<true>(reinterpret_cast<char*>(a.dsmall), wave_tile, 1, 0, col, half, small, gscale);
    in_rgb = small;
    in_rgb[3] = (__bf16)0.0f;

    const unsigned lane32 = IMG16 ? block_lane_offset(col, half) : block8_lane_offset(col, half);
    const unsigned blk = IMG16 ? 2048u : 1024u;
    const unsigned so8 = (unsigned)wave_tile * (8u * blk) + lane32, so4 = (unsigned)wave_tile * (4u * blk) + lane32;
    const unsigned mo0 = (unsigned)tile * (72u * 512u * 2u) + 2u * tid;
    const bool more = tile + gridDim.x < n_tiles;
    const unsigned mo0n = more ? (unsigned)(tile + gridDim.x) * (72u * 512u * 2u) + 2u * tid : mo0;
    const unsigned first = __builtin_amdgcn_readfirstlane(tile == (int64_t)blockIdx.x ? 1u : 0u);
    if constexpr (IMG16) bwd16_stream_pass(ab0, ab1, in_rgb, in_sigma, src, voff, ldsw, so8, so4, mo0, mo0n, first, karg, gscale);
    else bwd_stream_pass(ab0, ab1, in_rgb, in_sigma, src, voff, ldsw, so8, so4, mo0, mo0n, first, karg, gscale);
  }
  asm volatile("s_waitcnt vmcnt(0)" ::: "memory");
}

}

using namespace nerf;

int nerf_launch_wgrad(const char* stash, const StashLayout& sl, const char* work, const BwdLayout& bl,
                      int64_t n, float* grads, int part, hipStream_t stream, size_t zero_lo, size_t zero_hi);

extern "C" size_t nerf_mlp_bwd_workspace_bytes(int64_t n) { return n > 0 ? bwd_layout(n).total : 0; }

static int launch_dgrad(const void* packed, const void* stash, const float* rgb, const float* sigma,
                        const float* d_rgb, const float* d_sigma, int64_t n, void* workspace,
                        const float* amax_dev, nerf_stream_t stream) {
  NERF_REQUIRE(n > 0 && n < (int64_t)1 << 31, "nerf_mlp_bwd: n=%lld out of range", (long long)n);
  NERF_REQUIRE(packed && stash && rgb && sigma && d_rgb && d_sigma && workspace, "nerf_mlp_bwd: NULL pointer");
  NERF_REQUIRE(((uintptr_t)packed & 255) == 0 && ((uintptr_t)stash & 255) == 0 && ((uintptr_t)workspace & 255) == 0,
               "nerf_mlp_bwd: packed/stash/workspace must be 256-byte aligned");
  const StashLayout sl = stash_layout(n);
  const BwdLayout bl = bwd_layout(n);
  BwdArgs a{};
  a.packed = static_cast<const char*>(packed);
  a.rgb = rgb; a.sigma = sigma; a.d_rgb = d_rgb; a.d_sigma = d_sigma;
  a.n = n; a.n_pad = bl.n_pad;
  a.st_mask = reinterpret_cast<const uint4*>(static_cast<const char*>(stash) + sl.mask);
  char* w = static_cast<char*>(workspace);
  a.dsmall = reinterpret_cast<__bf16*>(w + bl.dsmall);
  a.dhv = reinterpret_cast<__bf16*>(w + bl.dhv);
  a.dfeat = reinterpret_cast<__bf16*>(w + bl.dfeat);
  a.dh = reinterpret_cast<__bf16*>(w + bl.dh);
  a.amax = reinterpret_cast<float*>(w + bl.amax);
  a.amax_src = amax_dev != nullptr ? amax_dev : a.amax;
  int n_cu = 0;
  if (int rc = device_cu_count(&n_cu); rc != NERF_OK) return rc;
  const bool stream_family = chain_use_stream(n, true);
  const void* kernel = stream_family ? (bl.fp8 ? (const void*)mlp_bwd_stream_kernel<false> : (const void*)mlp_bwd_stream_kernel<true>)
                                     : (const void*)mlp_bwd_kernel;
  if (int rc = ensure_dynamic_lds(kernel, kChainLds, "nerf_mlp_bwd"); rc != NERF_OK) return rc;
  const int64_t tiles = bl.n_pad / kTileSamples;
  if (options().chain_grid > 0 && options().chain_grid < n_cu) n_cu = options().chain_grid;
  const int grid = (int)(tiles < n_cu ? tiles : n_cu);
  if (bl.fp8 && amax_dev == nullptr) {
    if (hipMemsetAsync(a.amax, 0, sizeof(float), as_stream(stream)) != hipSuccess)
      return fail(NERF_ELAUNCH, "nerf_mlp_bwd: memset failed");
    const int64_t want = (n + 1023) / 1024;
    hipLaunchKernelGGL(bwd_amax_kernel, dim3((int)(want < 1024 ? want : 1024)), dim3(256), 0, as_stream(stream), a);
  }
  if (stream_family && bl.fp8)
    hipLaunchKernelGGL(mlp_bwd_stream_kernel<false>, dim3(grid), dim3(kChainThreads), kChainLds, as_stream(stream), a);
  else if (stream_family)
    hipLaunchKernelGGL(mlp_bwd_stream_kernel<true>, dim3(grid), dim3(kChainThreads), kChainLds, as_stream(stream), a);
  else
    hipLaunchKernelGGL(mlp_bwd_kernel, dim3(grid), dim3(kChainThreads), kChainLds, as_stream(stream), a);
  return check_launch("nerf_mlp_bwd (dgrad chain)");
}

static int launch_wgrad(const void* stash, const void* workspace, int64_t n, float* grads_f32, int part,
                        nerf_stream_t stream) {
  NERF_REQUIRE(grads_f32 != nullptr, "nerf_mlp_bwd: grads_f32 is NULL");
  NERF_REQUIRE(part >= 0 && part <= 2, "nerf_mlp_bwd_wgrad_part: part=%d (0 all, 1 late layers, 2 early layers)", part);
  const size_t lo = part == 1 ? (size_t)plan::kW4 : 0, hi = part == 2 ? (size_t)plan::kW4 : (size_t)plan::kParamCount;
  if (n == 0) {
    if (hipMemsetAsync(grads_f32 + lo, 0, sizeof(float) * (hi - lo), as_stream(stream)) != hipSuccess)
      return fail(NERF_ELAUNCH, "nerf_mlp_bwd: memset failed");
    return NERF_OK;
  }
  NERF_REQUIRE(stash && workspace, "nerf_mlp_bwd: NULL pointer");
  return nerf_launch_wgrad(static_cast<const char*>(stash), stash_layout(n), static_cast<const char*>(workspace),
                           bwd_layout(n), n, grads_f32, part, as_stream(stream), lo, hi);
}

extern "C" int nerf_mlp_bwd_dgrad(const void* packed, const void* stash, const float* rgb, const float* sigma,
                                  const float* d_rgb, const float* d_sigma, int64_t n, void* workspace,
                                  nerf_stream_t stream) {
  if (n == 0) return NERF_OK;
  return launch_dgrad(packed, stash, rgb, sigma, d_rgb, d_sigma, n, workspace, nullptr, stream);
}

extern "C" int nerf_mlp_bwd_dgrad_ex(const void* packed, const void* stash, const float* rgb, const float* sigma,
                                     const float* d_rgb, const float* d_sigma, int64_t n, void* workspace,
                                     const float* amax_dev, nerf_stream_t stream) {
  if (n == 0) return NERF_OK;
  return launch_dgrad(packed, stash, rgb, sigma, d_rgb, d_sigma, n, workspace, amax_dev, stream);
}

extern "C" int nerf_mlp_bwd_wgrad(const void* stash, const void* workspace, int64_t n, float* grads_f32,
                                  nerf_stream_t stream) {
  return launch_wgrad(stash, workspace, n, grads_f32, 0, stream);
}

extern "C" int64_t nerf_mlp_wgrad_part_split(void) { return plan::kW4; }

extern "C" int nerf_mlp_bwd_wgrad_part(const void* stash, const void* workspace, int64_t n, float* grads_f32, int part,
                                       nerf_stream_t stream) {
  return launch_wgrad(stash, workspace, n, grads_f32, part, stream);
}

extern "C" int nerf_mlp_bwd(const void* packed, const void* stash, const float* rgb, const float* sigma,
                            const float* d_rgb, const float* d_sigma, int64_t n, float* grads_f32,
                            void* workspace, nerf_stream_t stream) {
  NERF_REQUIRE(n >= 0, "nerf_mlp_bwd: n=%lld", (long long)n);
  if (n > 0) {
    const int rc = launch_dgrad(packed, stash, rgb, sigma, d_rgb, d_sigma, n, workspace, nullptr, stream);
    if (rc != NERF_OK) return rc;
  }
  return launch_wgrad(stash, workspace, n, grads_f32, 0, stream);
}
```

### project-nerf_amd/csrc/mlp_pack.hip

```cpp
#include "common.h"
#include "mlp_plan.h"

namespace nerf {
using namespace plan;

struct FragTable {
  int v[kFwdFrags + kBwdFrags];
};

constexpr FragTable make_frag_table() {
  FragTable t{};
  int f = 0;
  for (int kind = 0; kind < kNumKinds; ++kind) {
    const int ks = step_ks(kind);
    for (int m = 0; m < step_of(kind).mt; ++m)
      for (int k = 0; k < ks; ++k) t.v[f++] = (kind << 16) | (m << 8) | k;
  }
  return t;
}
__constant__ FragTable g_frag_table = make_frag_table();

__device__ __forceinline__ int src_index(int kind, int row, int k, bool nat) {
  if (kind <= F_PTS7) {
    const int l = kind;
    const int in_dim = pts_in_dim(l);
    int col;
    if (l == 0) col = k < 63 ? k : -1;
    else if (l == 4) col = nat ? (k < 63 ? 256 + k : -1) : k;
    else col = k;
    return col < 0 ? -1 : pts_weight_off(l) + row * in_dim + col;
  }
  switch (kind) {
    case F_HEAD: return row < 256 ? kWFeat + row * 256 + k : (row == 256 ? kWSigma + k : -1);
    case F_VIEW: return nat ? (k < 27 ? kWView + row * 283 + 256 + k : -1) : kWView + row * 283 + k;
    case F_RGB: return row < 3 ? kWRgb + row * 128 + k : -1;
    case B_RGB: return k < 3 ? kWRgb + k * 128 + row : -1;
    case B_VIEW: return kWView + k * 283 + row;
    case B_HEAD: return nat ? (k == 0 ? kWSigma + row : -1) : kWFeat + k * 256 + row;
    default: {
      const int l = 7 - (kind - B_PTS7);
      return pts_weight_off(l) + k * pts_in_dim(l) + row;
    }
  }
}

__global__ void __launch_bounds__(256) pack16_kernel(const float* __restrict__ params, __bf16* __restrict__ packed_fwd16) {
  const int total = kFwdFrags * 64;
  for (int t = blockIdx.x * blockDim.x + threadIdx.x; t < total; t += gridDim.x * blockDim.x) {
    const int frag = t >> 6, lane = t & 63;
    const int desc = g_frag_table.v[frag];
    const int kind = desc >> 16, mt = (desc >> 8) & 0xFF, ks = desc & 0xFF;
    const Step st = step_of(kind);
    const int row = mt * 32 + 16 * (ks & 1) + (lane & 15), q = lane >> 4;
    const bool nat = ks >= st.ks_acc;
    const int kk = nat ? (ks - st.ks_acc) >> 1 : ks >> 1;
    typedef __bf16 bf16x8 __attribute__((ext_vector_type(8)));
    bf16x8 out;
#pragma unroll
    for (int j = 0; j < 8; ++j) {
      const int k = nat ? 32 * kk + 8 * q + j : 32 * kk + 16 * (j >> 2) + 4 * q + (j & 3);
      const int src = src_index(kind, row, k, nat);
      out[j] = (__bf16)(src >= 0 ? params[src] : 0.0f);
    }
    *reinterpret_cast<bf16x8*>(packed_fwd16 + (size_t)frag * 512 + lane * 8) = out;
  }
}

__global__ void __launch_bounds__(256)
pack_kernel(const float* __restrict__ params, __bf16* __restrict__ packed_fwd,
            __bf16* __restrict__ packed_bwd, float* __restrict__ bias) {
  const int total = (kFwdFrags + kBwdFrags) * 64;
  for (int t = blockIdx.x * blockDim.x + threadIdx.x; t < total; t += gridDim.x * blockDim.x) {
    const int frag = t >> 6, lane = t & 63;
    const int desc = g_frag_table.v[frag];
    const int kind = desc >> 16, mt = (desc >> 8) & 0xFF, ks = desc & 0xFF;
    const Step st = step_of(kind);
    const int row = mt * 32 + (lane & 31), h = lane >> 5;
    const bool nat = ks >= st.ks_acc;
    typedef __bf16 bf16x8 __attribute__((ext_vector_type(8)));
    bf16x8 out;
#pragma unroll
    for (int j = 0; j < 8; ++j) {
      int k;
      if (nat) k = 16 * (ks - st.ks_acc) + 8 * h + j;
      else k = 32 * (ks >> 1) + 16 * (ks & 1) + 8 * (j >> 2) + 4 * h + (j & 3);
      const int src = src_index(kind, row, k, nat);
      out[j] = (__bf16)(src >= 0 ? params[src] : 0.0f);
    }
    __bf16* dst = frag < kFwdFrags ? packed_fwd + (size_t)frag * 512 : packed_bwd + (size_t)(frag - kFwdFrags) * 512;
    *reinterpret_cast<bf16x8*>(dst + lane * 8) = out;
  }
  for (int i = blockIdx.x * blockDim.x + threadIdx.x; i < kBiasFloats; i += gridDim.x * blockDim.x) {
    float b = 0.0f;
    if (i < 2048) b = params[pts_bias_off(i >> 8) + (i & 255)];
    else if (i < 2048 + 288) { const int r = i - 2048; b = r < 256 ? params[kBFeat + r] : (r == 256 ? params[kBSigma] : 0.0f); }
    else if (i < 2048 + 288 + 128) b = params[kBView + (i - 2048 - 288)];
    else { const int r = i - 2048 - 288 - 128; b = r < 3 ? params[kBRgb + r] : 0.0f; }
    bias[i] = b;
  }
}

}

extern "C" size_t nerf_mlp_packed_bytes(void) { return nerf::plan::kPackBytes; }

extern "C" int nerf_mlp_pack_streams(const float* params_f32, void* packed, int which, nerf_stream_t stream) {
  using namespace nerf;
  NERF_REQUIRE(params_f32 && packed, "nerf_mlp_pack: NULL pointer");
  NERF_REQUIRE(((uintptr_t)packed & 255) == 0, "nerf_mlp_pack: packed buffer must be 256-byte aligned");
  NERF_REQUIRE(which >= 1 && which <= 3, "nerf_mlp_pack_streams: which=%d (1 training streams + biases, 2 inference stream, 3 all)", which);
  char* base = static_cast<char*>(packed);
  if (which & 1)
    hipLaunchKernelGGL(pack_kernel, dim3(512), dim3(256), 0, as_stream(stream), params_f32,
                       reinterpret_cast<__bf16*>(base + plan::kPackFwdOff),
                       reinterpret_cast<__bf16*>(base + plan::kPackBwdOff),
                       reinterpret_cast<float*>(base + plan::kPackBiasOff));
  if (which & 2)
    hipLaunchKernelGGL(pack16_kernel, dim3(304), dim3(256), 0, as_stream(stream), params_f32,
                       reinterpret_cast<__bf16*>(base + plan::kPackFwd16Off));
  return check_launch("nerf_mlp_pack");
}

extern "C" int nerf_mlp_pack(const float* params_f32, void* packed, nerf_stream_t stream) {
  return nerf_mlp_pack_streams(params_f32, packed, 3, stream);
}
```

### project-nerf_amd/csrc/mlp_wgrad.h

```cpp
#pragma once
#include <hip/hip_runtime.h>
#include <stdint.h>

namespace nerf {

constexpr int kMaxJobs = 12;
constexpr int kWgStages = 4;
constexpr int kWgStageA = 16 * 1024, kWgStageB = 16 * 1024, kWgStageN = 4 * 1024;
constexpr int kWgStageBytes = kWgStageA + kWgStageB + kWgStageN;
constexpr int kWgLds = kWgStages * kWgStageBytes;
constexpr int kWgScratch = 256;
constexpr int kMaxTiles = 10;
constexpr size_t kSmallSlabBytes = 8u << 20;

struct WgradJob {
  const char* a;
  const char* b_acc;
  const char* b_nat;
  int a_bytes;
  int b_acc_bytes, b_nat_bytes;
  int a_nat;
  int mt_a;
  int nt_acc, nt_nat, ones;
  int split_n;
  int kind;
  int w_off, w_ld;
  int o_row0, o_valid;
  int acc_valid, acc_col0;
  int nat_valid, nat_col0;
  int bias_off, bias_nat_col;
  const char* a2;
  int w2_off, bias2_off, o2_row, n2;
  long long cost0;
  int cost;
  long long slab_off;
  int part0, n_parts, p_stride;
};

struct WgradArgs {
  WgradJob jobs[kMaxJobs];
  int n_jobs;
  int wave_tiles;
  long long total_cost;
  float* grads;
  float* slab;
  int slab_accumulate;
  const float* amax;
  int k16;
  int debug;
};


int wgrad_launch(WgradArgs& args, int64_t n_samples, float* grads, hipStream_t stream, float* slab = nullptr,
                 size_t slab_bytes = 0, size_t zero_lo = 0, size_t zero_hi = 0);

}
```

### project-nerf_amd/csrc/mlp_wgrad.hip

```cpp
#include <stdlib.h>
#include "mlp_chain.h"
#include "mlp_stash.h"
#include "mlp_wgrad.h"

namespace nerf {
using namespace plan;

typedef short s16x4 __attribute__((ext_vector_type(4)));
typedef short s16x8 __attribute__((ext_vector_type(8)));
typedef __attribute__((address_space(3))) s16x4* lds_s16x4_t;

__device__ __forceinline__ void dma_1k(const char* gsrc_lane, unsigned lds_dst) {
  unsigned keep;
  asm volatile("s_mov_b32 %0, m0\n\ts_mov_b32 m0, %2\n\ts_nop 0\n\tglobal_load_lds_dwordx4 %1, off nt\n\ts_mov_b32 m0, %0"
               : "=&s"(keep) : "v"(gsrc_lane), "s"(lds_dst) : "memory");
}

template <int STRIDE>
__device__ __forceinline__ bf16x8 tr_frag(const char* p) {
  const s16x4 lo = __builtin_amdgcn_ds_read_tr16_b64_v4i16((lds_s16x4_t)(p));
  const s16x4 hi = __builtin_amdgcn_ds_read_tr16_b64_v4i16((lds_s16x4_t)(p + STRIDE));
  s16x8 v = {lo[0], lo[1], lo[2], lo[3], hi[0], hi[1], hi[2], hi[3]};
  return __builtin_bit_cast(bf16x8, v);
}
// ... 495 lines not shown
      continue;
    }
#pragma unroll
    for (int s = 0; s < 2; ++s) {
      bf16x8 af = SPLIT ? tr_frag<128>(pa + 512 * s) : tr_frag<256>(pa + 1024 * s);
      if (SPLIT && g.fhalf) {
#pragma unroll
        for (int e = 0; e < 8; ++e) af[e] = (__bf16)0.0f;
      }
      if constexpr (SPLIT) {
        if (wave < NT_ACC) acc[0] = __builtin_amdgcn_mfma_f32_32x32x16_bf16(af, tr_frag<256>(pb + 1024 * s), acc[0], 0, 0, 0);
        if (ONES && wave == NT_ACC % 8) acc[1] = __builtin_amdgcn_mfma_f32_32x32x16_bf16(af, ones, acc[1], 0, 0, 0);
      } else {
        bf16x8 bf[NT_ACC + NT_NAT + 1];
#pragma unroll
        for (int k = 0; k < NT_ACC; ++k) bf[k] = tr_frag<256>(pb + k * 2048 + 1024 * s);
#pragma unroll
        for (int k = 0; k < NT_NAT; ++k) bf[NT_ACC + k] = tr_frag<128>(pn + k * 2048 + 512 * s);
        bf[NT_ACC + NT_NAT] = ones;
#pragma unroll
        for (int k = 0; k < NT; ++k) acc[k] = __builtin_amdgcn_mfma_f32_32x32x16_bf16(af, bf[k], acc[k], 0, 0, 0);
        __builtin_amdgcn_sched_group_barrier(0x100, 2 * (1 + NT_ACC + NT_NAT), 0);
        __builtin_amdgcn_sched_group_barrier(0x008, NT, 0);
        __builtin_amdgcn_sched_barrier(0);
      }
    }
  }

  flush_tiles<NT_ACC, NT_NAT, ONES, SPLIT, FP8, NT>(args, job, acc, g, active);
}

template <bool FP8>
__global__ void __launch_bounds__(512, 2) mlp_wgrad_kernel(const WgradArgs args) {
  extern __shared__ __attribute__((aligned(16))) char smem[];
  LaneGeo g;
  g.lane = threadIdx.x & 63;
  g.wave = __builtin_amdgcn_readfirstlane(threadIdx.x >> 6);
  const int grp = g.lane >> 4, i16 = g.lane & 15, q = i16 >> 2, p = i16 & 3;
  const int hh = grp >> 1;
  g.fhalf = grp & 1;
  g.off_acc = 512 * hh + 128 * g.fhalf + 64 * (p & 1) + 16 * q + 8 * (p >> 1);
  g.off_nat = 32 * (8 * hh + q) + 16 * (p >> 1) + 8 * (p & 1) + 1024 * g.fhalf;
  const int q8 = i16 >> 1, p8 = i16 & 1;
  g.off_acc8 = 256 * hh + 32 * q8 + 16 * g.fhalf + 8 * p8;
  g.off_nat8 = 512 * g.fhalf + 16 * (8 * hh + q8) + 8 * p8;

  const long long lo = args.total_cost * blockIdx.x / gridDim.x;
  const long long hi = args.total_cost * (blockIdx.x + 1) / gridDim.x;
  for (int j = 0; j < args.n_jobs; ++j) {
    const WgradJob job = args.jobs[j];
    const long long j0 = job.cost0, j1 = job.cost0 + (long long)job.cost * args.wave_tiles;
    if (hi <= j0 || lo >= j1) continue;
    const long long a0 = lo > j0 ? lo - j0 : 0, a1 = (hi < j1 ? hi : j1) - j0;
    const int wt0 = (int)((a0 + job.cost - 1) / job.cost), wt1 = (int)((a1 + job.cost - 1) / job.cost);
    if (wt0 >= wt1) continue;
    if constexpr (FP8) {
      switch (job.kind) {
        case 0: run_job8<8, 0, true>(args, job, wt0, wt1, smem, g); break;
        case 1: run_job8<8, 2, false>(args, job, wt0, wt1, smem, g); break;
        case 2: run_job8<0, 2, false>(args, job, wt0, wt1, smem, g); break;
        case 3: run_job8<8, 1, false>(args, job, wt0, wt1, smem, g); break;
        case 4: run_job<8, 0, true, true, true>(args, job, wt0, wt1, smem, g); break;
        default: run_job<4, 0, true, true, true>(args, job, wt0, wt1, smem, g); break;
      }
    } else {
    switch (job.kind) {
      case 0: run_job16<16, 16, 0, 8, 0, true, false>(args, job, wt0, wt1, smem, g); break;
      case 1: run_job16<16, 16, 4, 8, 2, false, false>(args, job, wt0, wt1, smem, g); break;
      case 2: run_job16<16, 0, 4, 0, 2, false, false>(args, job, wt0, wt1, smem, g); break;
      case 3: run_job16<8, 16, 2, 8, 1, false, false>(args, job, wt0, wt1, smem, g); break;
      case 4: run_job16<1, 16, 0, 8, 0, true, true>(args, job, wt0, wt1, smem, g); break;
      case 5: run_job16<1, 8, 0, 4, 0, true, true>(args, job, wt0, wt1, smem, g); break;
      case 13: run_job16<16, 16, 0, 8, 0, true, false, true>(args, job, wt0, wt1, smem, g); break;
      case 14: run_job16<16, 0, 6, 0, 3, false, false, false, NatStage>(args, job, wt0, wt1, smem, g); break;
      case 6: run_job<0, 1, false, false, false>(args, job, wt0, wt1, smem, g); break;
      case 7: run_job<2, 0, false, false, false>(args, job, wt0, wt1, smem, g); break;
      case 8: run_job<1, 1, false, false, false>(args, job, wt0, wt1, smem, g); break;
      default: run_job<2, 0, false, true, false>(args, job, wt0, wt1, smem, g); break;
    }
    }
  }
}

template <bool P4>
__global__ void __launch_bounds__(512, P4 ? 4 : 6) mlp_wgrad_small_kernel(const WgradArgs args) {
  using Stage = std::conditional_t<P4, SmallStageP4, SmallStage>;
  extern __shared__ __attribute__((aligned(16))) char smem[];
  LaneGeo g;
  g.lane = threadIdx.x & 63;
  g.wave = __builtin_amdgcn_readfirstlane(threadIdx.x >> 6);
  const int grp = g.lane >> 4, i16 = g.lane & 15, q = i16 >> 2, p = i16 & 3;
  const int hh = grp >> 1;
  g.fhalf = grp & 1;
  g.off_acc = 512 * hh + 128 * g.fhalf + 64 * (p & 1) + 16 * q + 8 * (p >> 1);
  g.off_nat = 32 * (8 * hh + q) + 16 * (p >> 1) + 8 * (p & 1) + 1024 * g.fhalf;
  g.off_acc8 = g.off_nat8 = 0;
  const long long lo = args.total_cost * blockIdx.x / gridDim.x;
  const long long hi = args.total_cost * (blockIdx.x + 1) / gridDim.x;
  for (int j = 0; j < args.n_jobs; ++j) {
    const WgradJob job = args.jobs[j];
    const long long j0 = job.cost0, j1 = job.cost0 + (long long)job.cost * args.wave_tiles;
    if (hi <= j0 || lo >= j1) continue;
    const long long a0 = lo > j0 ? lo - j0 : 0, a1 = (hi < j1 ? hi : j1) - j0;
    const int wt0 = (int)((a0 + job.cost - 1) / job.cost), wt1 = (int)((a1 + job.cost - 1) / job.cost);
    if (wt0 >= wt1) continue;
    if constexpr (P4) {
      switch (job.kind) {
        case 10: run_job16<4, 4, 0, 2, 0, true, false, false, Stage>(args, job, wt0, wt1, smem, g); continue;
        case 11: run_job16<4, 4, 2, 2, 1, false, false, false, Stage>(args, job, wt0, wt1, smem, g); continue;
        case 12: run_job16<4, 0, 4, 0, 2, false, false, false, Stage>(args, job, wt0, wt1, smem, g); continue;
        default: break;
      }
    }
    switch (job.kind) {
      case 6: run_job16<4, 0, 2, 0, 1, false, false, false, Stage>(args, job, wt0, wt1, smem, g); break;
      case 7:
        if (job.mt_a == 2) run_job16<4, 4, 0, 2, 0, false, false, false, Stage>(args, job, wt0, wt1, smem, g);
        else run_job16<2, 4, 0, 2, 0, false, false, false, Stage>(args, job, wt0, wt1, smem, g);
        break;
      case 8: run_job16<4, 2, 2, 1, 1, false, false, false, Stage>(args, job, wt0, wt1, smem, g); break;
      default: run_job16<1, 4, 0, 2, 0, false, true, false, Stage>(args, job, wt0, wt1, smem, g); break;
    }
  }
}

__global__ void __launch_bounds__(256) wgrad_reduce_kernel(const WgradArgs args) {
  const WgradJob& job = args.jobs[blockIdx.y];
  const int n_w = job.o_valid * job.w_ld, n_b = n_w + job.o_valid, n_all = n_b + job.n2;
  const float* tile = args.slab + job.slab_off;
  for (int i = blockIdx.x * blockDim.x + threadIdx.x; i < n_all; i += gridDim.x * blockDim.x) {
    float s0 = 0.0f, s1 = 0.0f, s2 = 0.0f, s3 = 0.0f;
    int t = 0;
    for (; t + 4 <= job.n_parts; t += 4) {
      s0 += tile[(long long)(t + 0) * job.p_stride + i];
      s1 += tile[(long long)(t + 1) * job.p_stride + i];
      s2 += tile[(long long)(t + 2) * job.p_stride + i];
      s3 += tile[(long long)(t + 3) * job.p_stride + i];
    }
    for (; t < job.n_parts; ++t) s0 += tile[(long long)t * job.p_stride + i];
    const float sum = (s0 + s1) + (s2 + s3);
    float* dst = i < n_w ? args.grads + job.w_off + i
               : i < n_b ? ((job.ones || job.bias_nat_col >= 0) ? args.grads + job.bias_off + (i - n_w) : nullptr)
               : i < n_all - 1 ? args.grads + job.w2_off + (i - n_b)
                               : args.grads + job.bias2_off;
    if (dst != nullptr) *dst = args.slab_accumulate ? *dst + sum : sum;
  }
}

}

using namespace nerf;

int nerf_launch_wgrad(const char* stash, const StashLayout& sl, const char* work, const BwdLayout& bl,
                      int64_t n, float* grads, int part, hipStream_t stream, size_t zero_lo, size_t zero_hi) {
  WgradArgs args{};
  const size_t np = (size_t)sl.n_pad, eb = sl.fp8 ? 1 : 2;
  if (sl.fp8 != bl.fp8) return fail(NERF_EINVAL, "nerf_mlp_bwd: stash and workspace disagree on the image width");
  args.amax = sl.fp8 ? reinterpret_cast<const float*>(work + bl.amax) : nullptr;
  const char* xenc = stash + sl.xenc;
  const char* denc = stash + sl.denc;
  auto st_h = [&](int l) { return stash + sl.h + (size_t)l * np * 256 * eb; };
  auto dh = [&](int l) { return work + bl.dh + (size_t)l * np * 256 * eb; };
  int nj = 0;
  auto add = [&](WgradJob j) {
    args.jobs[nj++] = j;
  };
  {
    WgradJob j{};
    j.a = dh(0); j.a_bytes = 16384; j.mt_a = 8;
    j.b_nat = xenc; j.b_nat_bytes = 4096; j.nt_nat = 2;
    j.w_off = kW0; j.w_ld = 63; j.o_valid = 256; j.nat_valid = 63; j.nat_col0 = 0;
    j.bias_off = kB0; j.bias_nat_col = 63; j.kind = 2;
    add(j);
  }
  for (int l = 1; l < 8; ++l) {
    WgradJob j{};
    j.a = dh(l); j.a_bytes = 16384; j.mt_a = 8;
    j.b_acc = st_h(l - 1); j.b_acc_bytes = 16384; j.nt_acc = 8;
    j.w_off = pts_weight_off(l); j.w_ld = pts_in_dim(l); j.o_valid = 256; j.acc_valid = 256;
    j.bias_off = pts_bias_off(l);
    if (l == 4) {
      j.b_nat = xenc; j.b_nat_bytes = 4096; j.nt_nat = 2; j.nat_valid = 63; j.nat_col0 = 256; j.bias_nat_col = 63;
      j.kind = 1;
    } else {
      j.ones = 1; j.bias_nat_col = -1; j.kind = 0;
    }
    add(j);
  }
  {
    WgradJob j{};
    j.a = work + bl.dfeat; j.a_bytes = 16384; j.mt_a = 8;
    j.b_acc = st_h(7); j.b_acc_bytes = 16384; j.nt_acc = 8; j.ones = 1; j.bias_nat_col = -1;
    j.w_off = kWFeat; j.w_ld = 256; j.o_valid = 256; j.acc_valid = 256; j.bias_off = kBFeat; j.kind = 0;
    if (!sl.fp8) {
      j.a2 = work + bl.dsmall; j.w2_off = kWSigma; j.bias2_off = kBSigma; j.o2_row = 3; j.n2 = 257; j.kind = 13;
    }
    add(j);
  }
  if (sl.fp8) {
    WgradJob j{};
    j.a = work + bl.dsmall; j.a_bytes = 1024; j.a_nat = 1; j.mt_a = 1; j.split_n = 1;
    j.b_acc = st_h(7); j.b_acc_bytes = 16384; j.nt_acc = 8; j.ones = 1; j.bias_nat_col = -1;
    j.w_off = kWSigma; j.w_ld = 256; j.o_row0 = 3; j.o_valid = 1; j.acc_valid = 256; j.bias_off = kBSigma; j.kind = 4;
    add(j);
  }
  {
    WgradJob j{};
    j.a = work + bl.dhv; j.a_bytes = 8192; j.mt_a = 4;
    j.b_acc = stash + sl.feat; j.b_acc_bytes = 16384; j.nt_acc = 8;
    j.b_nat = denc; j.b_nat_bytes = 2048; j.nt_nat = 1; j.nat_valid = 27; j.nat_col0 = 256; j.bias_nat_col = 27;
    j.w_off = kWView; j.w_ld = 283; j.o_valid = 128; j.acc_valid = 256; j.bias_off = kBView; j.kind = 3;
    add(j);
  }
  {
    WgradJob j{};
    j.a = work + bl.dsmall; j.a_bytes = 1024; j.a_nat = 1; j.mt_a = 1; j.split_n = 1;
    j.b_acc = stash + sl.hv; j.b_acc_bytes = 8192; j.nt_acc = 4; j.ones = 1; j.bias_nat_col = -1;
    j.w_off = kWRgb; j.w_ld = 128; j.o_row0 = 0; j.o_valid = 3; j.acc_valid = 128; j.bias_off = kBRgb; j.kind = 5;
    add(j);
  }
  if (part != 0) {
    const int lo = part == 1 ? 4 : 0, hi = part == 1 ? nj : 4;
    for (int j = lo; j < hi; ++j) args.jobs[j - lo] = args.jobs[j];
    nj = hi - lo;
  }
  args.n_jobs = nj;
  float* slab = bl.slab_bytes ? reinterpret_cast<float*>(const_cast<char*>(work) + bl.slab) : nullptr;
  return wgrad_launch(args, n, grads, stream, slab, bl.slab_bytes, zero_lo, zero_hi);
}

int nerf::wgrad_launch(WgradArgs& args, int64_t n, float* grads, hipStream_t stream, float* slab, size_t slab_bytes,
                       size_t zero_lo, size_t zero_hi) {
  int nj = args.n_jobs;
  const int overhead = options().wgrad_overhead;
  for (int j = 0; j < nj; ++j) {
    WgradJob& jb = args.jobs[j];
    const int bytes = jb.a_bytes + jb.b_acc_bytes + jb.b_nat_bytes + (jb.a2 ? 1024 : 0);
    jb.cost = bytes + overhead;
    if (args.amax != nullptr) {
      const int nt = jb.nt_acc + jb.nt_nat + jb.ones;
      const int per_simd = jb.split_n ? (jb.nt_acc > 4 ? 3 : 2) : (jb.mt_a > 4 ? 2 : 1) * nt;
      const int t_mfma = (jb.split_n || options().wgrad_k16 ? 32 * 4 : 64) * per_simd, t_dma = bytes * 16 / options().wgrad_bw_x16;
      jb.cost = (t_mfma > t_dma ? t_mfma : t_dma) + options().wgrad_fixed;
    }
  }
  args.wave_tiles = args.amax != nullptr ? (int)((n + 63) / 64) : (int)((n + 31) / 32);
  long long c = 0;
  for (int j = 0; j < nj; ++j) {
    args.jobs[j].cost0 = c;
    c += (long long)args.jobs[j].cost * args.wave_tiles;
  }
  args.total_cost = c;
  args.grads = grads;
  args.debug = options().wgrad_debug;
  args.k16 = options().wgrad_k16;
  if (options().wgrad_only >= 0) {
    const int kind = options().wgrad_only;
    int m = 0;
    for (int j = 0; j < args.n_jobs; ++j) if (args.jobs[j].kind == kind) args.jobs[m++] = args.jobs[j];
    args.n_jobs = m;
    nj = m;
    long long cc = 0;
    for (int j = 0; j < nj; ++j) { args.jobs[j].cost0 = cc; cc += (long long)args.jobs[j].cost * args.wave_tiles; }
    args.total_cost = cc;
  }

  int n_cu = 0;
  if (int rc = device_cu_count(&n_cu); rc != NERF_OK) return rc;
  const bool fp8 = args.amax != nullptr;
  if (int rc = ensure_dynamic_lds(fp8 ? (const void*)mlp_wgrad_kernel<true> : (const void*)mlp_wgrad_kernel<false>, kWgLds + kWgScratch,
                                  "nerf_mlp_bwd (wgrad)"); rc != NERF_OK) return rc;
  bool small = args.amax == nullptr && !options().wgrad_big_only, p4 = false;
  for (int j = 0; j < args.n_jobs; ++j) {
    const WgradJob& jb = args.jobs[j];
    p4 = p4 || (jb.kind >= 10 && jb.kind <= 12);
    small = small && jb.kind >= 6 && jb.a_bytes <= SmallStage::A && jb.b_acc_bytes <= SmallStage::B && jb.b_nat_bytes <= SmallStageP4::N;
  }
  if (p4 && !small) return fail(NERF_EINVAL, "wgrad: Part 4 job kinds run on the small-stage kernel only");
  long long want = (long long)args.wave_tiles * nj / 4;
  if (options().wgrad_grid > 0 && options().wgrad_grid < n_cu) n_cu = options().wgrad_grid;
  int grid = (int)(want < 1 ? 1 : (want > n_cu ? n_cu : want));
  if (small) {
    const long long span = options().wgrad_small_span > 0 ? options().wgrad_small_span : 4;
    const long long cap = (long long)(slab != nullptr ? 1 : (options().wgrad_small_cap > 0 ? options().wgrad_small_cap : 3)) * n_cu;
    const long long want3 = (long long)args.wave_tiles * nj / span;
    grid = (int)(want3 < 1 ? 1 : (want3 > cap ? cap : want3));
  }
  args.slab = nullptr;
  args.slab_accumulate = small ? 1 : 0;
  if (slab != nullptr && args.n_jobs > 0 && args.total_cost > 0) {
    bool ok = true;
    long long off = 0;
    for (int j = 0; j < args.n_jobs && ok; ++j) {
      WgradJob& jb = args.jobs[j];
      const long long j0 = jb.cost0, j1 = jb.cost0 + (long long)jb.cost * args.wave_tiles;
      int first = -1, last = -1, count = 0;
      for (int b = 0; b < grid; ++b) {
        const long long lo = args.total_cost * b / grid, hi = args.total_cost * (b + 1) / grid;
        if (hi <= j0 || lo >= j1) continue;
        const long long a0 = lo > j0 ? lo - j0 : 0, a1 = (hi < j1 ? hi : j1) - j0;
        const int wt0 = (int)((a0 + jb.cost - 1) / jb.cost), wt1 = (int)((a1 + jb.cost - 1) / jb.cost);
        if (wt0 >= wt1) continue;
        if (first < 0) first = b;
        last = b;
        ++count;
      }
      ok = count > 0 && count == last - first + 1;
      jb.part0 = first;
      jb.n_parts = count;
      jb.p_stride = (jb.o_valid * jb.w_ld + jb.o_valid + jb.n2 + 63) / 64 * 64;
      jb.slab_off = off;
      off += (long long)count * jb.p_stride;
    }
    if (ok && (size_t)off * sizeof(float) <= slab_bytes) args.slab = slab;
    if (args.slab != nullptr && small && hipMemsetAsync(slab, 0, (size_t)off * sizeof(float), stream) != hipSuccess)
      return fail(NERF_ELAUNCH, "tiny-MLP wgrad: memset failed");
    if (args.slab == nullptr && small) return fail(NERF_EINVAL, "tiny-MLP wgrad (option \"deterministic\"): partial tiles need %zu bytes, %zu given%s",
                                (size_t)off * sizeof(float), slab_bytes, ok ? "" : " (a job's workgroups are not contiguous)");
  }
  if (args.slab == nullptr && zero_hi > zero_lo &&
      hipMemsetAsync(grads + zero_lo, 0, sizeof(float) * (zero_hi - zero_lo), stream) != hipSuccess)
    return fail(NERF_ELAUNCH, "nerf_mlp_bwd: memset failed");
  if (small) {
    if (p4) hipLaunchKernelGGL(mlp_wgrad_small_kernel<true>, dim3(grid), dim3(512), kWgStages * SmallStageP4::Bytes, stream, args);
    else hipLaunchKernelGGL(mlp_wgrad_small_kernel<false>, dim3(grid), dim3(512), kWgStages * SmallStage::Bytes, stream, args);
    if (args.slab != nullptr) {
      if (int rc = check_launch("tiny-MLP wgrad"); rc != NERF_OK) return rc;
      hipLaunchKernelGGL(wgrad_reduce_kernel, dim3(16, args.n_jobs), dim3(256), 0, stream, args);
      return check_launch("tiny-MLP wgrad (reduce)");
    }
    return check_launch("tiny-MLP wgrad");
  }
  if (fp8) hipLaunchKernelGGL(mlp_wgrad_kernel<true>, dim3(grid), dim3(512), kWgLds + kWgScratch, stream, args);
  else hipLaunchKernelGGL(mlp_wgrad_kernel<false>, dim3(grid), dim3(512), kWgLds + kWgScratch, stream, args);
  if (args.slab != nullptr) {
    if (int rc = check_launch("nerf_mlp_bwd (wgrad)"); rc != NERF_OK) return rc;
    hipLaunchKernelGGL(wgrad_reduce_kernel, dim3(160, args.n_jobs), dim3(256), 0, stream, args);
    return check_launch("nerf_mlp_bwd (wgrad reduce)");
  }
  return check_launch("nerf_mlp_bwd (wgrad)");
}
```

### project-nerf_amd/engine.py

```python
from __future__ import annotations

import os
from typing import Dict, Optional, Tuple

import torch

from . import ops

Tensor = torch.Tensor


def param_shapes():
    out = []
    for i in range(8):
        k = 63 if i == 0 else (319 if i == 4 else 256)
        out += [(f"pts_layers.{i}.weight", (256, k)), (f"pts_layers.{i}.bias", (256,))]
    out += [("sigma_layer.weight", (1, 256)), ("sigma_layer.bias", (1,)),
            ("feature_layer.weight", (256, 256)), ("feature_layer.bias", (256,)),
            ("view_layer.weight", (128, 283)), ("view_layer.bias", (128,)),
            ("rgb_layer.weight", (3, 128)), ("rgb_layer.bias", (3,))]
    return out


def default_init(seed: int = 0) -> Tensor:
    g = torch.Generator().manual_seed(seed)
    parts, fan_in = [], 1
    for name, shape in param_shapes():
        if name.endswith("weight"):
            fan_in = shape[1]
        parts.append(((torch.rand(shape, generator=g) * 2 - 1) / fan_in ** 0.5).reshape(-1))
    return torch.cat(parts)


def flatten_state_dict(sd: Dict[str, Tensor], prefix: str = "decoder.") -> Tensor:
    return torch.cat([sd[prefix + k].reshape(-1).float() for k, _ in param_shapes()])


def unflatten(flat: Tensor, prefix: str = "decoder.") -> Dict[str, Tensor]:
    out, off = {}, 0
    for k, shape in param_shapes():
        n = 1
        for s in shape:
            n *= s
        out[prefix + k] = flat[off:off + n].view(shape)
        off += n
    return out


class VanillaNerfEngine:
    def __init__(self, params: Optional[Tensor] = None, device: str = "cuda", lr: float = 5e-4,
                 near: float = 2.0, far: float = 6.0, white_bkgd: bool = True, seed: int = 0,
                 world_size: int = 1):
        self.device = torch.device(device)
        flat = default_init(seed) if params is None else params.detach().float().reshape(-1)
        assert flat.numel() == ops.MLP_PARAM_COUNT
        self.params = flat.to(self.device).contiguous()
        self.exp_avg = torch.zeros_like(self.params)
        self.exp_avg_sq = torch.zeros_like(self.params)
        self.grads = torch.empty_like(self.params)
        self.packed = torch.empty(ops.mlp_packed_bytes(), dtype=torch.uint8, device=self.device)
        self.lr, self.near, self.far = lr, near, far
        self.bg = (torch.ones(3) if white_bkgd else torch.zeros(3)).to(self.device)
        self.step_count = 0
        self.world_size = world_size
        self.grad_scale = torch.full((1,), 1.0 / world_size, device=self.device)
        self._ws: Dict[Tuple[str, int], Tensor] = {}
        self._scalars = torch.zeros(2, 1024, device=self.device)
        self.repack()

    def repack(self, training_only: bool = False) -> None:
        ops.mlp_pack(self.params, self.packed, which=1 if training_only else 3)
        self._infer_stale = training_only

    def _inference_weights(self) -> Tensor:
        if getattr(self, "_infer_stale", False):
            ops.mlp_pack(self.params, self.packed, which=2)
            self._infer_stale = False
        return self.packed

    def state_dict(self, prefix: str = "decoder.") -> Dict[str, Tensor]:
        return {k: v.clone() for k, v in unflatten(self.params, prefix).items()}

    def load_state_dict(self, sd: Dict[str, Tensor], prefix: str = "decoder.") -> None:
        self.params.copy_(flatten_state_dict(sd, prefix).to(self.device))
        self.repack()

    def _buf(self, kind: str, nbytes: int) -> Tensor:
        key = (kind, nbytes)
        if key not in self._ws:
            self._ws[key] = torch.empty(nbytes, dtype=torch.uint8, device=self.device)
        return self._ws[key]

    def compute_gradients(self, rays_o: Tensor, rays_d: Tensor, target: Tensor, n_samples: int = 64,
                   u: Optional[Tensor] = None, sync_grads=None, sync_grads_async=None, mark=None,
                   z: Optional[Tensor] = None) -> Tensor:
        mark = mark or (lambda name: None)
        R = rays_o.shape[0]
        n = R * n_samples
        if z is None:
            if u is None:
                u = torch.rand(R, n_samples, device=self.device)
            z = ops.sample_rays(rays_o, rays_d, self.near, self.far, n_samples, u=u)
            mark("sample")
        stash = self._buf("stash", ops.mlp_stash_bytes(n))
        rgb, sigma = ops.mlp_fwd(self.packed, rays_o, rays_d, z, stash)
        mark("fwd")
        self._grad_calls = getattr(self, "_grad_calls", -1) + 1
        slot = self._grad_calls % self._scalars.shape[1]
        if slot == 0:
            self._scalars.zero_()
        loss, amax = self._scalars[0, slot:slot + 1], self._scalars[1, slot:slot + 1]
        d_rgb, d_sigma, _ = ops.composite_mse_bwd(rgb.view(R, n_samples, 3), sigma.view(R, n_samples), z, rays_d, self.bg,
                                                  target, loss, amax_accum=amax)
        mark("loss")
        if sync_grads_async is not None:
            ops.mlp_bwd_overlapped(self.packed, stash, rgb, sigma, d_rgb.view(n, 3), d_sigma.view(n), self.grads,
                                   self._buf("bwd", ops.mlp_bwd_workspace_bytes(n)), sync_grads_async, amax=amax, mark=mark)
        else:
            ops.mlp_bwd(self.packed, stash, rgb, sigma, d_rgb.view(n, 3), d_sigma.view(n), self.grads,
                        self._buf("bwd", ops.mlp_bwd_workspace_bytes(n)), amax=amax, mark=mark)
        mark("wgrad")
        if sync_grads is not None:
            sync_grads(self.grads)
        return loss[0].clone()

    def apply_gradients(self) -> None:
        self.step_count += 1
        ops.adam_step(self.params, self.grads, self.exp_avg, self.exp_avg_sq, self.step_count, self.lr,
                      grad_scale=self.grad_scale if self.world_size > 1 else None)
        self.repack(training_only=True)

    def train_step(self, rays_o: Tensor, rays_d: Tensor, target: Tensor, n_samples: int = 64,
                   u: Optional[Tensor] = None, sync_grads=None, sync_grads_async=None, mark=None,
                   z: Optional[Tensor] = None) -> Tensor:
        loss = self.compute_gradients(rays_o, rays_d, target, n_samples, u=u, sync_grads=sync_grads,
                                      sync_grads_async=sync_grads_async, mark=mark, z=z)
        self.apply_gradients()
        if mark is not None:
            mark("adam+pack")
        return loss

    @torch.no_grad()
    def render_rays(self, rays_o: Tensor, rays_d: Tensor, n_samples: int, u: Optional[Tensor] = None):
        z = ops.sample_rays(rays_o, rays_d, self.near, self.far, n_samples, u=u)
        rgb, sigma = ops.mlp_fwd(self._inference_weights(), rays_o, rays_d, z)
        R = rays_o.shape[0]
        c, depth, acc, _, _ = ops.composite_fwd(rgb.view(R, n_samples, 3), sigma.view(R, n_samples), z, rays_d, self.bg)
        return c, depth, acc

    @torch.no_grad()
    def render_rays_hierarchical(self, rays_o: Tensor, rays_d: Tensor, n_coarse: int, n_fine: int):
        R = rays_o.shape[0]
        z = ops.sample_rays(rays_o, rays_d, self.near, self.far, n_coarse)
        rgb, sigma = ops.mlp_fwd(self._inference_weights(), rays_o, rays_d, z)
        w = ops.composite_fwd(rgb.view(R, n_coarse, 3), sigma.view(R, n_coarse), z, rays_d, self.bg, want_weights=True)[4]
        z_all = ops.sample_pdf(z, w, n_fine)
        S = n_coarse + n_fine
        rgb, sigma = ops.mlp_fwd(self._inference_weights(), rays_o, rays_d, z_all)
        c, depth, acc, _, _ = ops.composite_fwd(rgb.view(R, S, 3), sigma.view(R, S), z_all, rays_d, self.bg)
        return c, depth, acc

    @torch.no_grad()
    def render_image(self, rays_o: Tensor, rays_d: Tensor, n_samples: int, chunk: int = 65536, n_fine: int = 0) -> Tensor:
        shape = rays_o.shape[:-1]
        o, d = rays_o.reshape(-1, 3), rays_d.reshape(-1, 3)
        if n_fine == 0:
            chunk = max(1, min(chunk, o.shape[0]))
            ws = self._buf("render", ops._lib.load().nerf_render_rays_workspace_bytes(chunk, n_samples))
            return ops.render_rays_fwd(self._inference_weights(), o, d, n_samples, self.near, self.far, self.bg, chunk, ws)[0].view(*shape, 3)
        out = torch.empty(o.shape[0], 3, device=self.device)
        for i in range(0, o.shape[0], chunk):
            out[i:i + chunk] = self.render_rays_hierarchical(o[i:i + chunk], d[i:i + chunk], n_samples, n_fine)[0]
        return out.view(*shape, 3)


class InstantNgpEngine:

    def __init__(self, cfg: Optional[dict] = None, device: str = "cuda", seed: int = 0, world_size: int = 1):
        cfg = dict(cfg or {})
        self.device = torch.device(device)
        self.seed = int(seed)
        self.bound = float(cfg.get("scene_bound", 1.5))
        if cfg.get("n_levels", 16) != 16 or cfg.get("n_features_per_level", 2) != 2 or cfg.get("hidden_dim", 64) != 64:
            raise NotImplementedError("libnerf_hip's tiny-MLP kernels are compiled for 16 levels x 2 features (32 hash "
                                      "channels) and 64 hidden units")
        self.levels = ops.HashLevelTable(cfg.get("n_levels", 16), cfg.get("log2_hashmap_size", 19),
                                         cfg.get("base_resolution", 16), cfg.get("per_level_scale", 1.5))
        g = torch.Generator().manual_seed(seed)
        from .sharded import padded_length
        n_tab = self.levels.entries * 2
        n_pad = padded_length(n_tab, max(int(world_size), 1))
        self._table_buf = torch.zeros(n_pad, device=self.device)
        self._table_buf[:n_tab] = ((torch.rand(n_tab, generator=g) * 2 - 1) * 1e-4).to(self.device)
        self.table = self._table_buf[:n_tab]
        self.shard = None

        def xavier(rows, cols, fi, fo):
            return (torch.rand(rows, cols, generator=g) * 2 - 1) * (6.0 / (fi + fo)) ** 0.5
        w1 = xavier(64, 48, 43, 64)
        w1[:, 43:] = 0
        w3 = xavier(16, 64, 64, 3)
        w3[3:] = 0
        self.net = torch.cat([xavier(64, 32, 32, 64).reshape(-1), xavier(16, 64, 64, 16).reshape(-1), w1.reshape(-1),
                              xavier(64, 64, 64, 64).reshape(-1), w3.reshape(-1)]).to(self.device)
        self._m_buf, self._v_buf = torch.zeros(n_pad, device=self.device), torch.zeros(n_pad, device=self.device)
        self.state = {"table": (self._m_buf[:n_tab], self._v_buf[:n_tab]), "net": (torch.zeros_like(self.net), torch.zeros_like(self.net))}
        self._g_table_buf = torch.zeros(n_pad, device=self.device)
        self.g_table = self._g_table_buf[:n_tab]
        self.g_net = torch.empty_like(self.net)
        self._hash_ws = None
        self.half_table = bool(cfg.get("half_table", True))
        self.precount = bool(cfg.get("precount", False))
        from .specbwd import SpeculativeScatter
        self.spec = SpeculativeScatter(bool(cfg.get("speculative_hash_backward", True)) and not os.environ.get("NERF_NO_SPECULATIVE_BWD"))
        self._table_h_buf = torch.zeros(n_pad, device=self.device, dtype=torch.float16) if self.half_table else None
        self.table_h = self._table_h_buf[:n_tab] if self.half_table else None
        self._table_version = None
        self.packed = ops.imlp_pack(self.net)
        self.near, self.far = float(cfg.get("near", 2.0)), float(cfg.get("far", 6.0))
        self.lr0, self.eta_min = float(cfg.get("learning_rate", 1e-2)), float(cfg.get("eta_min", 1e-4))
        self.t_max = int(cfg.get("train_iters", 2000))
        self.wd = float(cfg.get("weight_decay", 1e-5))
        self.tv_weight = float(cfg.get("tv_loss_weight", 1e-6)) if cfg.get("use_tv_loss", True) else 0.0
        self.bg = (torch.ones(3) if cfg.get("white_bkgd", True) else torch.zeros(3)).to(self.device)
        res = int(cfg.get("grid_resolution", 128))
        self.grid_threshold = float(cfg.get("grid_threshold", 0.12))
        self.grid = torch.zeros(res, res, res, device=self.device)
        self.binary_grid = torch.ones(res, res, res, dtype=torch.bool, device=self.device)
        self.step_count, self.world_size = 0, world_size
        self._scratch = ops.normsq_ws(self.device)
        self._net_scratch = ops.normsq_ws(self.device)
        self._loss_ring = torch.zeros(65536, device=self.device)

    def lr(self) -> float:
        import math
        return self.eta_min + (self.lr0 - self.eta_min) * (1 + math.cos(math.pi * self.step_count / self.t_max)) / 2

    def _gather_table(self) -> Tensor:
        if not self.half_table:
            return self.table.view(-1, 2)
        if self._table_version != self.table._version:
            ops.f32_to_f16(self.table, self.table_h)
            self._table_version = self.table._version
        return self.table_h.view(-1, 2)

    def _field(self, pts: Tensor, dirs: Tensor, train: bool, hist_ws: Optional[Tensor] = None):
        lib = ops._lib.load()
        n = pts.shape[0]
        ws = torch.empty(lib.nerf_imlp_workspace_bytes(n), device=self.device, dtype=torch.uint8)
        if hist_ws is not None:
            ops._lib.check(lib.nerf_hash_encode_fwd_f16_hist(pts.data_ptr(), n, self._gather_table().data_ptr(), self.levels.n_levels,
                                                             *self.levels.host_args(), float(self.bound), ws.data_ptr(), hist_ws.data_ptr(),
                                                             hist_ws.numel(), ops._stream()), "nerf_hash_encode_fwd_f16_hist")
        else:
            ops.hash_encode_fwd(pts, self._gather_table(), self.levels, self.bound, want_f32=False, out_nat=ws)
        rgb, sigma = torch.empty(n, 3, device=self.device), torch.empty(n, device=self.device)
        ops._lib.check(lib.nerf_imlp_fwd(self.packed.data_ptr(), ws.data_ptr(), dirs.data_ptr(), n, rgb.data_ptr(),
                                         sigma.data_ptr(), 1 if train else 0, ops._stream()), "nerf_imlp_fwd")
        return rgb, sigma, ws

    def level_groups(self, n_groups: int = 4):
        off = [int(o) for o in self.levels.offset] + [self.levels.entries]
        cuts, target = [0], self.levels.entries / n_groups
        for l in range(1, self.levels.n_levels):
            if off[l] >= target * len(cuts) and len(cuts) < n_groups:
                cuts.append(l)
        cuts.append(self.levels.n_levels)
        return [(cuts[k], cuts[k + 1]) for k in range(len(cuts) - 1) if cuts[k] < cuts[k + 1]]

    def prepare_batch(self, rays_o: Tensor, rays_d: Tensor, n_samples: int = 128, u: Optional[Tensor] = None, first_ray: int = 0):
        jitter = None
        if u is None:
            self._jitter_counter = getattr(self, "_jitter_counter", -1) + 1
            jitter = (self.seed, self._jitter_counter)
        return ops.sample_compact_async(rays_o, rays_d, self.near, self.far, n_samples, self.binary_grid, self.bound, u=u,
                                        jitter=jitter, first_ray=first_ray)

    def compute_gradients(self, rays_o: Tensor, rays_d: Tensor, target: Tensor, n_samples: int = 128,
                          u: Optional[Tensor] = None, sync_grads_async=None, reduce_dtype=None, prepared=None,
                          shard_grads: bool = False) -> Tensor:
        if shard_grads and self.shard is not None:
            import torch.distributed as dist
            loss = self._compute_gradients(rays_o, rays_d, target, n_samples, u=u, prepared=prepared)
            self.shard.reduce_scatter_grads()
            if self.world_size > 1:
                dist.all_reduce(self.g_net, op=dist.ReduceOp.SUM)
            return loss
        return self._compute_gradients(rays_o, rays_d, target, n_samples, u=u, sync_grads_async=sync_grads_async, reduce_dtype=reduce_dtype,
                                       prepared=prepared)

    def _compute_gradients(self, rays_o: Tensor, rays_d: Tensor, target: Tensor, n_samples: int = 128,
                           u: Optional[Tensor] = None, sync_grads_async=None, reduce_dtype=None, prepared=None) -> Tensor:
# ... 178 lines not shown
```

### project-nerf_amd/ops.py

```python
from __future__ import annotations

from typing import Optional, Tuple

import torch

from . import _lib

Tensor = torch.Tensor


def _stream() -> int:
    return torch._C._cuda_getCurrentRawStream(torch._C._cuda_getDevice())


def _dev(t: Tensor, name: str, dtype=torch.float32) -> Tensor:
    if not isinstance(t, Tensor):
        raise TypeError(f"{name}: expected a tensor")
    if t.device.type != "cuda":
        raise _lib.NerfHipError(f"{name} is on {t.device}; the hot path only runs on a HIP device (no CPU fallback)")
    if t.dtype != dtype:
        raise TypeError(f"{name}: expected {dtype}, got {t.dtype}")
    return t if t.is_contiguous() else t.contiguous()


# ... 228 lines not shown
        import weakref
        out = CompactedSamples(z, slots, pts, dirs, count[0], None, seq=count[1])
        count[2].owner[count[3]] = weakref.ref(out)
        return out
    count_host = torch.empty(1, dtype=torch.int32, pin_memory=True)
    count_host.copy_(count, non_blocking=True)
    event = torch.cuda.Event()
    event.record()
    return CompactedSamples(z, slots, pts, dirs, count_host, event)


class _CompositeIndexed(torch.autograd.Function):
    @staticmethod
    def forward(ctx, rgb_c, sigma_c, slots, z, rays_d, bg):
        lib = _lib.load()
        R, S = z.shape
        rgb_c, sigma_c = _dev(rgb_c, "rgb_c"), _dev(sigma_c, "sigma_c")
        out_rgb = torch.empty(R, 3, device=z.device)
        depth = torch.empty(R, device=z.device)
        acc = torch.empty(R, device=z.device)
        bg_rows = 0 if bg is None else (1 if bg.dim() == 1 else bg.shape[0])
        _lib.check(lib.nerf_composite_fwd_indexed(_p(rgb_c), _p(sigma_c), _p(slots), _p(z), _p(rays_d), _p(bg), bg_rows,
                                                  R, S, _p(out_rgb), _p(depth), _p(acc), _stream()),
                   "nerf_composite_fwd_indexed")
        ctx.save_for_backward(rgb_c, sigma_c, slots, z, rays_d, bg)
        return out_rgb, depth, acc

    @staticmethod
    def backward(ctx, g_rgb, g_depth, g_acc):
        lib = _lib.load()
        rgb_c, sigma_c, slots, z, rays_d, bg = ctx.saved_tensors
        R, S = z.shape
        d_rgb, d_sigma = torch.empty_like(rgb_c), torch.empty_like(sigma_c)
        bg_rows = 0 if bg is None else (1 if bg.dim() == 1 else bg.shape[0])
        _lib.check(lib.nerf_composite_bwd_indexed(_p(rgb_c), _p(sigma_c), _p(slots), _p(z), _p(rays_d), _p(bg), bg_rows,
                                                  _p(g_rgb.contiguous()), _p(g_depth.contiguous()), _p(g_acc.contiguous()),
                                                  R, S, _p(d_rgb), _p(d_sigma), _stream()), "nerf_composite_bwd_indexed")
        return d_rgb, d_sigma, None, None, None, None


def composite_indexed(rgb_c: Tensor, sigma_c: Tensor, slots: Tensor, z: Tensor, rays_d: Tensor,
                      bg: Optional[Tensor] = None):
    return _CompositeIndexed.apply(rgb_c, sigma_c.reshape(-1), slots, z, rays_d, bg)


def sample_pdf(z_coarse: Tensor, weights: Tensor, n_fine: int, u: Optional[Tensor] = None) -> Tensor:
    lib = _lib.load()
    z_coarse, weights = _dev(z_coarse, "z_coarse"), _dev(weights, "weights")
    R, S = z_coarse.shape
    if u is not None:
        u = _dev(u, "u")
    out = torch.empty(R, S + n_fine, device=z_coarse.device)
    _lib.check(lib.nerf_sample_pdf(_p(z_coarse), _p(weights), _p(u), R, S, n_fine, _p(out), _stream()), "nerf_sample_pdf")
    return out


def grid_lattice(bound: float, resolution: int, device) -> Tensor:
    lib = _lib.load()
    pts = torch.empty(resolution ** 3, 3, device=device, dtype=torch.float32)
    if pts.device.type != "cuda":
        raise _lib.NerfHipError("grid_lattice: the hot path only runs on a HIP device")
    _lib.check(lib.nerf_grid_lattice(float(bound), resolution, _p(pts), _stream()), "nerf_grid_lattice")
    return pts


def grid_threshold(sigma_grid: Tensor, threshold: float, prev: Optional[Tensor] = None, decay: float = 1.0):
    lib = _lib.load()
    cur = _dev(sigma_grid, "sigma_grid")
    grid = cur if prev is None else _dev(prev, "prev")
    binary = torch.empty(cur.shape, device=cur.device, dtype=torch.bool)
    count = torch.zeros(1, device=cur.device, dtype=torch.int64)
    _lib.check(lib.nerf_grid_update(_p(cur), _p(grid), _p(binary), cur.numel(), float(decay),
                                    0 if prev is None else 1, float(threshold), _p(count), _stream()),
               "nerf_grid_update")
    return binary, float(count.item()) / cur.numel()


def fourier_encode(x: Tensor, n_freq: int) -> Tensor:
    lib = _lib.load()
    x = _dev(x, "x")
    n, dim = x.shape
    out = torch.empty(n, dim + 2 * dim * n_freq, device=x.device, dtype=torch.float32)
    _lib.check(lib.nerf_fourier_encode(_p(x), n, dim, n_freq, _p(out), _stream()), "nerf_fourier_encode")
    return out


def composite_fwd(rgb: Tensor, sigma: Tensor, z: Tensor, rays_d: Tensor, bg: Optional[Tensor] = None,
                  extra: Optional[Tensor] = None, want_weights: bool = False):
    lib = _lib.load()
    rgb, sigma, z, rays_d = _dev(rgb, "rgb"), _dev(sigma, "sigma"), _dev(z, "z"), _dev(rays_d, "rays_d")
    R, S = z.shape
    bg_rows = 0
    if bg is not None:
        bg = _dev(bg, "bg")
        bg_rows = 1 if bg.dim() == 1 else bg.shape[0]
    out_rgb = torch.empty(R, 3, device=z.device, dtype=torch.float32)
    depth = torch.empty(R, device=z.device, dtype=torch.float32)
    acc = torch.empty(R, device=z.device, dtype=torch.float32)
    extra_map = None
    if extra is not None:
        extra = _dev(extra, "extra")
        extra_map = torch.empty(R, 3, device=z.device, dtype=torch.float32)
    w = torch.empty(R, S, device=z.device, dtype=torch.float32) if want_weights else None
    _lib.check(lib.nerf_composite_fwd(_p(rgb), _p(sigma), _p(z), _p(rays_d), _p(bg), bg_rows, _p(extra),
                                      R, S, _p(out_rgb), _p(depth), _p(acc), _p(extra_map), _p(w), _stream()),
               "nerf_composite_fwd")
    return out_rgb, depth, acc, extra_map, w


def composite_bwd(rgb, sigma, z, rays_d, bg, extra, g_rgb, g_depth, g_acc, g_extra):
    lib = _lib.load()
    rgb, sigma, z, rays_d = _dev(rgb, "rgb"), _dev(sigma, "sigma"), _dev(z, "z"), _dev(rays_d, "rays_d")
    R, S = z.shape
    bg_rows = 0
    if bg is not None:
        bg = _dev(bg, "bg")
        bg_rows = 1 if bg.dim() == 1 else bg.shape[0]
    g_rgb = _dev(g_rgb, "g_rgb")
    g_depth = None if g_depth is None else _dev(g_depth, "g_depth")
    g_acc = None if g_acc is None else _dev(g_acc, "g_acc")
    d_rgb = torch.empty(R, S, 3, device=z.device, dtype=torch.float32)
    d_sigma = torch.empty(R, S, device=z.device, dtype=torch.float32)
    d_extra = None
    if extra is not None and g_extra is not None:
        extra, g_extra = _dev(extra, "extra"), _dev(g_extra, "g_extra")
        d_extra = torch.empty(R, S, 3, device=z.device, dtype=torch.float32)
    else:
        extra = g_extra = None
    _lib.check(lib.nerf_composite_bwd(_p(rgb), _p(sigma), _p(z), _p(rays_d), _p(bg), bg_rows, _p(extra),
                                      _p(g_rgb), _p(g_depth), _p(g_acc), _p(g_extra), R, S,
                                      _p(d_rgb), _p(d_sigma), _p(d_extra), _stream()), "nerf_composite_bwd")
    return d_rgb, d_sigma, d_extra


def composite_mse_bwd(rgb: Tensor, sigma: Tensor, z: Tensor, rays_d: Tensor, bg: Optional[Tensor], target: Tensor,
                      loss_accum: Tensor, slots: Optional[Tensor] = None, amax_accum: Optional[Tensor] = None,
                      loss_weight: Optional[float] = None, want_pred: bool = False):
    lib = _lib.load()
    rgb, sigma, z, rays_d, target = _dev(rgb, "rgb"), _dev(sigma, "sigma"), _dev(z, "z"), _dev(rays_d, "rays_d"), _dev(target, "target")
    R, S = z.shape
    bg_rows = 0
    if bg is not None:
        bg = _dev(bg, "bg")
        bg_rows = 1 if bg.dim() == 1 else bg.shape[0]
    d_rgb, d_sigma = torch.empty_like(rgb), torch.empty_like(sigma)
    pred = torch.empty(R, 3, device=z.device) if want_pred else None
    w = 1.0 / (3 * R) if loss_weight is None else loss_weight
    _lib.check(lib.nerf_composite_mse_bwd(_p(rgb), _p(sigma), _p(slots), _p(z), _p(rays_d), _p(bg), bg_rows, _p(target), w, R, S,
                                          _p(pred), _p(loss_accum), _p(d_rgb), _p(d_sigma), _p(amax_accum), _p(sum_ws(z.device)), _stream()),
               "nerf_composite_mse_bwd")
    return d_rgb, d_sigma, pred


class _Composite(torch.autograd.Function):

    @staticmethod
    def forward(ctx, rgb, sigma, z, rays_d, bg, extra):
        out_rgb, depth, acc, extra_map, _ = composite_fwd(rgb, sigma, z, rays_d, bg, extra)
        ctx.save_for_backward(rgb, sigma, z, rays_d, bg, extra)
        if extra_map is None:
            extra_map = out_rgb.new_zeros(0)
        return out_rgb, depth, acc, extra_map

    @staticmethod
    def backward(ctx, g_rgb, g_depth, g_acc, g_extra):
        rgb, sigma, z, rays_d, bg, extra = ctx.saved_tensors
        d_rgb, d_sigma, d_extra = composite_bwd(rgb, sigma, z, rays_d, bg, extra, g_rgb.contiguous(),
                                                g_depth.contiguous(), g_acc.contiguous(),
                                                None if extra is None else g_extra.contiguous())
        return d_rgb, d_sigma, None, None, None, d_extra


def composite(rgb: Tensor, sigma: Tensor, z: Tensor, rays_d: Tensor, bg: Optional[Tensor] = None,
              extra: Optional[Tensor] = None):
    out_rgb, depth, acc, extra_map = _Composite.apply(rgb, sigma, z, rays_d, bg, extra)
    return out_rgb, depth, acc, (extra_map if extra is not None else None)


MLP_PARAM_COUNT = 595844


def mlp_packed_bytes() -> int:
    return _lib.load().nerf_mlp_packed_bytes()


def mlp_pack(params: Tensor, packed: Optional[Tensor] = None, which: int = 3) -> Tensor:
    lib = _lib.load()
    params = _dev(params, "params")
    if params.numel() != MLP_PARAM_COUNT:
        raise ValueError(f"params must have {MLP_PARAM_COUNT} elements, got {params.numel()}")
    if packed is None:
        packed = torch.empty(lib.nerf_mlp_packed_bytes(), device=params.device, dtype=torch.uint8)
    _lib.check(lib.nerf_mlp_pack_streams(_p(params), _p(packed), which, _stream()), "nerf_mlp_pack")
    return packed


def mlp_stash_bytes(n: int) -> int:
    return _lib.load().nerf_mlp_stash_bytes(n)


def mlp_fwd(packed: Tensor, rays_o: Tensor, rays_d: Tensor, z: Optional[Tensor],
            stash: Optional[Tensor] = None) -> Tuple[Tensor, Tensor]:
    lib = _lib.load()
    rays_o, rays_d = _dev(rays_o, "rays_o"), _dev(rays_d, "rays_d")
    if z is not None:
        z = _dev(z, "z")
        n, S = z.numel(), z.shape[1]
    else:
        n, S = rays_o.shape[0], 0
    rgb = torch.empty(n, 3, device=rays_o.device, dtype=torch.float32)
    sigma = torch.empty(n, device=rays_o.device, dtype=torch.float32)
    _lib.check(lib.nerf_mlp_fwd(_p(packed), _p(rays_o), _p(rays_d), _p(z), n, S, _p(rgb), _p(sigma),
                                _p(stash), _stream()), "nerf_mlp_fwd")
    return rgb, sigma


def render_rays_fwd(packed: Tensor, rays_o: Tensor, rays_d: Tensor, n_samples: int, near: float, far: float,
                    bg: Optional[Tensor] = None, chunk: int = 65536, workspace: Optional[Tensor] = None):
    lib = _lib.load()
    rays_o, rays_d = _dev(rays_o, "rays_o"), _dev(rays_d, "rays_d")
    R = rays_o.shape[0]
    chunk = max(1, min(chunk, max(R, 1)))
    need = lib.nerf_render_rays_workspace_bytes(chunk, n_samples)
    if workspace is None or workspace.numel() < need:
        workspace = torch.empty(need, device=rays_o.device, dtype=torch.uint8)
    bg_rows = 0
    if bg is not None:
        bg = _dev(bg, "bg")
        bg_rows = 1 if bg.dim() == 1 else bg.shape[0]
    out = torch.empty(R, 3, device=rays_o.device)
    depth, acc = torch.empty(R, device=rays_o.device), torch.empty(R, device=rays_o.device)
    _lib.check(lib.nerf_render_rays_fwd(_p(packed), _p(rays_o), _p(rays_d), R, n_samples, float(near), float(far), _p(bg), bg_rows,
                                        chunk, _p(workspace), _p(out), _p(depth), _p(acc), _stream()), "nerf_render_rays_fwd")
    return out, depth, acc


def mlp_bwd_workspace_bytes(n: int) -> int:
    return _lib.load().nerf_mlp_bwd_workspace_bytes(n)


def mlp_bwd(packed: Tensor, stash: Tensor, rgb: Tensor, sigma: Tensor, d_rgb: Tensor, d_sigma: Tensor,
            grads: Optional[Tensor] = None, workspace: Optional[Tensor] = None, amax: Optional[Tensor] = None,
            mark=None) -> Tensor:
    lib = _lib.load()
    rgb, sigma = _dev(rgb, "rgb"), _dev(sigma, "sigma")
    d_rgb, d_sigma = _dev(d_rgb, "d_rgb"), _dev(d_sigma, "d_sigma")
    n = sigma.numel()
    if grads is None:
        grads = torch.empty(MLP_PARAM_COUNT, device=rgb.device, dtype=torch.float32)
    if workspace is None:
        workspace = torch.empty(lib.nerf_mlp_bwd_workspace_bytes(n), device=rgb.device, dtype=torch.uint8)
    if amax is None:
        _lib.check(lib.nerf_mlp_bwd(_p(packed), _p(stash), _p(rgb), _p(sigma), _p(d_rgb), _p(d_sigma), n,
                                    _p(grads), _p(workspace), _stream()), "nerf_mlp_bwd")
    else:
        _lib.check(lib.nerf_mlp_bwd_dgrad_ex(_p(packed), _p(stash), _p(rgb), _p(sigma), _p(d_rgb), _p(d_sigma), n,
                                             _p(workspace), _p(amax), _stream()), "nerf_mlp_bwd_dgrad_ex")
        if mark is not None:
            mark("dgrad")
        _lib.check(lib.nerf_mlp_bwd_wgrad(_p(stash), _p(workspace), n, _p(grads), _stream()), "nerf_mlp_bwd_wgrad")
    return grads


def mlp_bwd_overlapped(packed: Tensor, stash: Tensor, rgb: Tensor, sigma: Tensor, d_rgb: Tensor, d_sigma: Tensor,
                       grads: Tensor, workspace: Tensor, reduce_async, amax: Optional[Tensor] = None, mark=None) -> None:
    lib = _lib.load()
    n = sigma.numel()
    _lib.check(lib.nerf_mlp_bwd_dgrad_ex(_p(packed), _p(stash), _p(rgb), _p(sigma), _p(d_rgb), _p(d_sigma), n,
                                         _p(workspace), _p(amax), _stream()), "nerf_mlp_bwd_dgrad")
    if mark is not None:
        mark("dgrad")
    split = lib.nerf_mlp_wgrad_part_split()
    handles = []
    for part, view in ((1, grads[split:]), (2, grads[:split])):
        _lib.check(lib.nerf_mlp_bwd_wgrad_part(_p(stash), _p(workspace), n, _p(grads), part, _stream()),
                   "nerf_mlp_bwd_wgrad_part")
        handles.append(reduce_async(view))
    for h in handles:
        if h is not None:
            h.wait()


class _Decoder(torch.autograd.Function):

    @staticmethod
    def forward(ctx, params, packed, rays_o, rays_d, z):
        n = z.numel() if z is not None else rays_o.shape[0]
        stash = torch.empty(mlp_stash_bytes(n), device=params.device, dtype=torch.uint8)
        rgb, sigma = mlp_fwd(packed, rays_o, rays_d, z, stash)
        ctx.save_for_backward(packed, stash, rgb, sigma)
        return rgb, sigma

    @staticmethod
    def backward(ctx, d_rgb, d_sigma):
        packed, stash, rgb, sigma = ctx.saved_tensors
        grads = mlp_bwd(packed, stash, rgb, sigma, d_rgb.contiguous(), d_sigma.contiguous())
        return grads, None, None, None, None


class _DecoderEncoded(torch.autograd.Function):

    @staticmethod
    def forward(ctx, params, packed, x_enc, d_enc, train):
        lib = _lib.load()
        n = x_enc.shape[0]
        rgb = torch.empty(n, 3, device=x_enc.device)
        sigma = torch.empty(n, device=x_enc.device)
        stash = torch.empty(mlp_stash_bytes(n), device=x_enc.device, dtype=torch.uint8) if train else None
        _lib.check(lib.nerf_mlp_fwd_encoded(_p(packed), _p(x_enc), _p(d_enc), n, _p(rgb), _p(sigma), _p(stash), _stream()),
                   "nerf_mlp_fwd_encoded")
        if train:
            ctx.save_for_backward(packed, stash, rgb, sigma)
        return rgb, sigma

    @staticmethod
    def backward(ctx, d_rgb, d_sigma):
        packed, stash, rgb, sigma = ctx.saved_tensors
        return mlp_bwd(packed, stash, rgb, sigma, d_rgb.contiguous(), d_sigma.contiguous()), None, None, None, None


def decoder_encoded(params: Tensor, packed: Tensor, x_enc: Tensor, d_enc: Tensor):
    x_enc, d_enc = _dev(x_enc, "x_enc"), _dev(d_enc, "d_enc")
    if x_enc.shape[1] != 63 or d_enc.shape[1] != 27 or x_enc.shape[0] != d_enc.shape[0]:
        raise ValueError(f"expected x_enc [n,63] and d_enc [n,27], got {tuple(x_enc.shape)} and {tuple(d_enc.shape)}")
    if x_enc.requires_grad or d_enc.requires_grad:
        raise NotImplementedError("gradients w.r.t. the Fourier codes are not produced (positions are not trainable)")
    if x_enc.shape[0] == 0:
        return x_enc.new_zeros(0, 3), x_enc.new_zeros(0)
    train = torch.is_grad_enabled() and params.requires_grad
    return _DecoderEncoded.apply(params, packed, x_enc, d_enc, train)


def decoder(params: Tensor, packed: Tensor, rays_o: Tensor, rays_d: Tensor, z: Optional[Tensor]):
    if torch.is_grad_enabled() and params.requires_grad:
        return _Decoder.apply(params, packed, rays_o, rays_d, z)
    return mlp_fwd(packed, rays_o, rays_d, z)


import ctypes as _ct
import math as _math

import numpy as _np


class HashLevelTable:

    def __init__(self, n_levels=16, log2_hashmap_size=19, base_resolution=16, per_level_scale=1.5):
        budget = 1 << log2_hashmap_size
        scale, res, size, offset, dense, off = [], [], [], [], [], 0
        for l in range(n_levels):
            s64 = base_resolution * (per_level_scale ** l) - 1.0
            r = int(_math.ceil(round(s64, 9))) + 1
            is_dense = r ** 3 <= budget
            sz = ((r ** 3 + 7) // 8) * 8 if is_dense else budget
            scale.append(s64); res.append(r); size.append(sz); offset.append(off); dense.append(int(is_dense))
            off += sz
        self.n_levels, self.entries = n_levels, off
        self.scale = _np.asarray(scale, dtype=_np.float32)
        self.res = _np.asarray(res, dtype=_np.uint32)
        self.size = _np.asarray(size, dtype=_np.uint32)
        self.offset = _np.asarray(offset, dtype=_np.uint32)
        self.dense = _np.asarray(dense, dtype=_np.uint32)

    def host_args(self):
        args = getattr(self, "_host_args", None)
        if args is None:
            args = self._host_args = tuple(a.ctypes.data_as(_ct.c_void_p) for a in (self.scale, self.res, self.size, self.offset, self.dense))
        return args


def hash_encode_fwd(pts: Tensor, table: Tensor, levels: HashLevelTable, bound: float,
                    want_f32: bool = True, out_nat: Optional[Tensor] = None, want_index: bool = False):
    lib = _lib.load()
    pts = _dev(pts, "pts")
    n = pts.shape[0]
    out = torch.empty(n, 2 * levels.n_levels, device=pts.device) if want_f32 else None
    if table.dtype == torch.float16:
        if want_index:
            raise ValueError("hash_encode_fwd: corner indices come with the fp32 table only")
        table = _dev(table, "table", torch.float16)
        _lib.check(lib.nerf_hash_encode_fwd_f16(_p(pts), n, _p(table), levels.n_levels, *levels.host_args(), float(bound),
                                                _p(out), _p(out_nat), _stream()), "nerf_hash_encode_fwd_f16")
        return out, None
    table = _dev(table, "table")
    idx = torch.empty(n, levels.n_levels, 8, device=pts.device, dtype=torch.int32) if want_index else None
    _lib.check(lib.nerf_hash_encode_fwd(_p(pts), n, _p(table), levels.n_levels, *levels.host_args(), float(bound),
                                        _p(out), _p(out_nat), _p(idx), _stream()), "nerf_hash_encode_fwd")
    return out, idx


def hash_encode_fwd_nat(pts: Tensor, table: Tensor, levels: HashLevelTable, bound: float, out_nat: Tensor, fp16: bool) -> None:
    lib = _lib.load()
    pts = _dev(pts, "pts")
    half = table.dtype == torch.float16
    table = _dev(table, "table", torch.float16 if half else torch.float32)
    _lib.check(lib.nerf_hash_encode_fwd_nat(_p(pts), pts.shape[0], None if half else _p(table), _p(table) if half else None, levels.n_levels,
                                            *levels.host_args(), float(bound), _p(out_nat), 1 if fp16 else 0, _stream()),
               "nerf_hash_encode_fwd_nat")


def hash_encode_fwd_nat_tables(pts: Tensor, tables, levels: HashLevelTable, bound: float, outs, fp16: bool) -> bool:
    if len(tables) < 2 or any(t.dtype != torch.float16 or not t.is_contiguous() for t in tables):
        return False
    t_step = tables[1].data_ptr() - tables[0].data_ptr()
    o_step = outs[1].data_ptr() - outs[0].data_ptr()
    if t_step <= 0 or o_step <= 0 or t_step % 4 or o_step % 2:
        return False
    for k in range(1, len(tables)):
        if tables[k].data_ptr() - tables[0].data_ptr() != k * t_step or outs[k].data_ptr() - outs[0].data_ptr() != k * o_step:
            return False
    pts = _dev(pts, "pts")
    _lib.check(_lib.load().nerf_hash_encode_fwd_nat_tables(_p(pts), pts.shape[0], _p(tables[0]), len(tables), t_step // 4, levels.n_levels,
                                                           *levels.host_args(), float(bound), _p(outs[0]), o_step, 1 if fp16 else 0,
                                                           _stream()), "nerf_hash_encode_fwd_nat_tables")
# ... 271 lines not shown
```

Before: 3.922 million rays/s.

## Fuse loss reduction into composite kernel and Adam+pack into wgrad tail

The composite MSE backward kernel now finishes its own cross-block loss/amax reduction: the last block to arrive, tracked with an atomic ticket, does the reduction, so the separate sums kernel launch is gone. For single-GPU training, weight-gradient computation is fused with the Adam update and bf16 repack through a tail hook in the wgrad launch, replacing separate adam and pack kernels. The engine also drops the slotted scalar buffer and the loss clone. These cut kernel launches and host overhead per step, at the cost of atomic/fence ordering complexity and a fallback path for fp8 or debug options.

```diff
diff --git a/include/nerf_hip.h b/include/nerf_hip.h
--- a/include/nerf_hip.h
+++ b/include/nerf_hip.h
@@ -13,7 +13,7 @@
 #define NERF_ELAUNCH (-5)
 #define NERF_ENOSYS (-38)
 
-#define NERF_ABI_VERSION 4
+#define NERF_ABI_VERSION 5
 
 typedef void* nerf_stream_t;
 
@@ -138,6 +138,9 @@
                             nerf_stream_t stream);
 int nerf_mlp_bwd_wgrad(const void* stash, const void* workspace, int64_t n, float* grads_f32,
                        nerf_stream_t stream);
+int nerf_mlp_bwd_wgrad_adam(const void* stash, const void* workspace, int64_t n, float* grads_f32, float* params_f32,
+                            float* exp_avg, float* exp_avg_sq, void* packed, int step, float lr, float beta1, float beta2,
+                            float eps, nerf_stream_t stream);
 
 int nerf_hash_encode_fwd(const float* pts, int64_t n, const float* table, int n_levels,
                          const float* scale_host, const unsigned* res_host, const unsigned* size_host,
@@ -248,6 +251,11 @@
                            const float* rays_d, const float* bg, int64_t bg_rows, const float* target,
                            float loss_weight, int64_t n_rays, int n_samples, float* pred_out, float* loss_accum,
                            float* d_rgb, float* d_sigma, float* amax_accum, float* sum_ws, nerf_stream_t stream);
+int nerf_composite_mse_bwd_fused(const float* rgb, const float* sigma, const int* slot_of_sample, const float* z,
+                                 const float* rays_d, const float* bg, int64_t bg_rows, const float* target,
+                                 float loss_weight, int64_t n_rays, int n_samples, float* pred_out, float* loss_out,
+                                 float* d_rgb, float* d_sigma, float* amax_out, float* sum_ws, uint32_t* ticket,
+                                 nerf_stream_t stream);
 int nerf_composite_mse_reg_bwd(const float* rgb, const float* sigma, const int* slot_of_sample, const float* z,
                                const float* rays_d, const float* bg, int64_t bg_rows, const float* target,
                                float loss_weight, const float* extra, float reg_weight, int64_t n_rays, int n_samples,
diff --git a/project-nerf_amd/_lib.py b/project-nerf_amd/_lib.py
--- a/project-nerf_amd/_lib.py
+++ b/project-nerf_amd/_lib.py
@@ -53,9 +53,12 @@
     "nerf_mlp_bwd": (i32, [c_ptr, c_ptr, c_ptr, c_ptr, c_ptr, c_ptr, i64, c_ptr, c_ptr, c_ptr]),
     "nerf_mlp_bwd_dgrad": (i32, [c_ptr, c_ptr, c_ptr, c_ptr, c_ptr, c_ptr, i64, c_ptr, c_ptr]),
     "nerf_mlp_bwd_wgrad": (i32, [c_ptr, c_ptr, i64, c_ptr, c_ptr]),
+    "nerf_mlp_bwd_wgrad_adam": (i32, [c_ptr, c_ptr, i64, c_ptr, c_ptr, c_ptr, c_ptr, c_ptr, i32, f32, f32, f32, f32, c_ptr]),
     "nerf_mlp_bwd_dgrad_ex": (i32, [c_ptr, c_ptr, c_ptr, c_ptr, c_ptr, c_ptr, i64, c_ptr, c_ptr, c_ptr]),
     "nerf_composite_mse_bwd": (i32, [c_ptr, c_ptr, c_ptr, c_ptr, c_ptr, c_ptr, i64, c_ptr, f32, i64, i32, c_ptr, c_ptr,
                                      c_ptr, c_ptr, c_ptr, c_ptr, c_ptr]),
+    "nerf_composite_mse_bwd_fused": (i32, [c_ptr, c_ptr, c_ptr, c_ptr, c_ptr, c_ptr, i64, c_ptr, f32, i64, i32, c_ptr, c_ptr,
+                                           c_ptr, c_ptr, c_ptr, c_ptr, c_ptr, c_ptr]),
     "nerf_mlp_wgrad_part_split": (i64, []),
     "nerf_mlp_bwd_wgrad_part": (i32, [c_ptr, c_ptr, i64, c_ptr, i32, c_ptr]),
     "nerf_hash_encode_fwd": (i32, [c_ptr, i64, c_ptr, i32, c_ptr, c_ptr, c_ptr, c_ptr, c_ptr, f32, c_ptr, c_ptr, c_ptr, c_ptr]),
@@ -134,7 +137,7 @@
     "nerf_adamw_clip_step_shadow": (i32, [c_ptr, c_ptr, c_ptr, c_ptr, i64, i32, f32, f32, f32, f32, f32, c_ptr, f32, f32, c_ptr, c_ptr]),
 }
 
-ABI_VERSION = 4
+ABI_VERSION = 5
 
 _lib = None
 
diff --git a/project-nerf_amd/csrc/adam.hip b/project-nerf_amd/csrc/adam.hip
--- a/project-nerf_amd/csrc/adam.hip
+++ b/project-nerf_amd/csrc/adam.hip
@@ -1,19 +1,9 @@
 #include "common.h"
+#include "adam_update.h"
 
 namespace nerf {
 
 typedef float f4 __attribute__((ext_vector_type(4)));
-
-__device__ __forceinline__ void adam_update(float& p, float g, float& m, float& v, float lr, float beta1, float beta2,
-                                            float eps, float wd, float inv_bc1, float inv_sqrt_bc2) {
-  float pi = p;
-  if (wd != 0.0f) pi *= (1.0f - lr * wd);
-  const float mi = beta1 * m + (1.0f - beta1) * g;
-  const float vi = beta2 * v + (1.0f - beta2) * g * g;
-  m = mi;
-  v = vi;
-  p = pi - (lr * inv_bc1) * (mi / (sqrtf(vi) * inv_sqrt_bc2 + eps));
-}
 
 template <bool VEC>
 __device__ __forceinline__ void adam_sweep(float* __restrict__ p, const float* __restrict__ g, float* __restrict__ m,
diff --git a/project-nerf_amd/csrc/adam_update.h b/project-nerf_amd/csrc/adam_update.h
--- /dev/null
+++ b/project-nerf_amd/csrc/adam_update.h
@@ -0,0 +1,17 @@
+#pragma once
+#include <hip/hip_runtime.h>
+
+namespace nerf {
+
+__device__ __forceinline__ void adam_update(float& p, float g, float& m, float& v, float lr, float beta1, float beta2,
+                                            float eps, float wd, float inv_bc1, float inv_sqrt_bc2) {
+  float pi = p;
+  if (wd != 0.0f) pi *= (1.0f - lr * wd);
+  const float mi = beta1 * m + (1.0f - beta1) * g;
+  const float vi = beta2 * v + (1.0f - beta2) * g * g;
+  m = mi;
+  v = vi;
+  p = pi - (lr * inv_bc1) * (mi / (sqrtf(vi) * inv_sqrt_bc2 + eps));
+}
+
+}
diff --git a/project-nerf_amd/csrc/composite.hip b/project-nerf_amd/csrc/composite.hip
--- a/project-nerf_amd/csrc/composite.hip
+++ b/project-nerf_amd/csrc/composite.hip
@@ -201,6 +201,9 @@
   }
 }
 
+__device__ __forceinline__ void composite_sums(const float* __restrict__ ws, int n_blocks, float* __restrict__ loss_out,
+                                               float* __restrict__ reg_out, float* __restrict__ amax_out, bool store);
+
 template <int K>
 __global__ void __launch_bounds__(256)
 composite_mse_bwd_kernel(const float* __restrict__ rgb, const float* __restrict__ sigma, const float* __restrict__ z,
@@ -209,7 +212,8 @@
                          float* __restrict__ pred_out, float* __restrict__ loss_out, float* __restrict__ d_rgb,
                          float* __restrict__ d_sigma, float* __restrict__ amax_out,
                          const float* __restrict__ extra, float reg_weight, float* __restrict__ d_extra,
-                         float* __restrict__ reg_out, float* __restrict__ extra_map, unsigned* __restrict__ sum_ws) {
+                         float* __restrict__ reg_out, float* __restrict__ extra_map, unsigned* __restrict__ sum_ws,
+                         unsigned* __restrict__ ticket) {
   const int lane = threadIdx.x & 63;
   const int64_t wave = (blockIdx.x * (int64_t)blockDim.x + threadIdx.x) >> 6;
   const int64_t nwave = ((int64_t)gridDim.x * blockDim.x) >> 6;
@@ -304,7 +308,7 @@
       after += G[k] * w[k];
     }
   }
-  __shared__ float part[12];
+  __shared__ float part[13];
   loss_local = wave_sum(loss_local);
   reg_local = wave_sum(reg_local);
 #pragma unroll
@@ -318,6 +322,23 @@
       ws[gridDim.x + blockIdx.x] = (part[8] + part[9]) + (part[10] + part[11]);
       ws[2 * gridDim.x + blockIdx.x] = fmaxf(fmaxf(part[4], part[5]), fmaxf(part[6], part[7]));
     }
+    if (ticket == nullptr) return;
+    asm volatile("s_waitcnt vmcnt(0)" ::: "memory");
+    __syncthreads();
+    if (threadIdx.x == 0) {
+      __builtin_amdgcn_fence(__ATOMIC_RELEASE, "agent");
+      asm volatile("s_waitcnt vmcnt(0)" ::: "memory");
+      const unsigned drawn = __hip_atomic_fetch_add(ticket, 1u, __ATOMIC_RELAXED, __HIP_MEMORY_SCOPE_AGENT);
+      part[12] = drawn == gridDim.x - 1 ? 1.0f : 0.0f;
+      if (drawn == gridDim.x - 1) {
+        __hip_atomic_store(ticket, 0u, __ATOMIC_RELAXED, __HIP_MEMORY_SCOPE_AGENT);
+        __builtin_amdgcn_fence(__ATOMIC_ACQUIRE, "agent");
+        asm volatile("s_waitcnt vmcnt(0)" ::: "memory");
+      }
+    }
+    __syncthreads();
+    if (part[12] == 0.0f) return;
+    composite_sums(reinterpret_cast<const float*>(sum_ws), (int)gridDim.x, loss_out, reg_out, amax_out, true);
     return;
   }
   if (threadIdx.x == 0) {
@@ -330,8 +351,8 @@
   }
 }
 
-__global__ void __launch_bounds__(256) composite_sums_kernel(const float* __restrict__ ws, int n_blocks, float* __restrict__ loss_out,
-                                                             float* __restrict__ reg_out, float* __restrict__ amax_out) {
+__device__ __forceinline__ void composite_sums(const float* __restrict__ ws, int n_blocks, float* __restrict__ loss_out,
+                                               float* __restrict__ reg_out, float* __restrict__ amax_out, bool store) {
   __shared__ float part[3][4];
   float s0 = 0.0f, s1 = 0.0f, m = 0.0f;
   for (int b = threadIdx.x; b < n_blocks; b += 256) {
@@ -347,10 +368,17 @@
   if ((threadIdx.x & 63) == 0) { part[0][threadIdx.x >> 6] = s0; part[1][threadIdx.x >> 6] = s1; part[2][threadIdx.x >> 6] = m; }
   __syncthreads();
   if (threadIdx.x == 0) {
-    *loss_out += (part[0][0] + part[0][1]) + (part[0][2] + part[0][3]);
-    if (reg_out != nullptr) *reg_out += (part[1][0] + part[1][1]) + (part[1][2] + part[1][3]);
-    if (amax_out != nullptr) *amax_out = fmaxf(*amax_out, fmaxf(fmaxf(part[2][0], part[2][1]), fmaxf(part[2][2], part[2][3])));
-  }
+    const float loss = (part[0][0] + part[0][1]) + (part[0][2] + part[0][3]), reg = (part[1][0] + part[1][1]) + (part[1][2] + part[1][3]);
+    const float top = fmaxf(fmaxf(part[2][0], part[2][1]), fmaxf(part[2][2], part[2][3]));
+    *loss_out = store ? loss : *loss_out + loss;
+    if (reg_out != nullptr) *reg_out = store ? reg : *reg_out + reg;
+    if (amax_out != nullptr) *amax_out = store ? top : fmaxf(*amax_out, top);
+  }
+}
+
+__global__ void __launch_bounds__(256) composite_sums_kernel(const float* __restrict__ ws, int n_blocks, float* __restrict__ loss_out,
+                                                             float* __restrict__ reg_out, float* __restrict__ amax_out) {
+  composite_sums(ws, n_blocks, loss_out, reg_out, amax_out, false);
 }
 
 static int per_lane(int S) {
@@ -480,9 +508,28 @@
   const dim3 grid((unsigned)mse_blocks(n_rays, sum_ws != nullptr));
   DISPATCH_K(per_lane(n_samples), composite_mse_bwd_kernel, rgb, sigma, z, rays_d, bg, bg_rows, target, loss_weight,
              slot_of_sample, n_rays, n_samples, pred_out, loss_accum, d_rgb, d_sigma, amax_accum,
-             (const float*)nullptr, 0.0f, (float*)nullptr, (float*)nullptr, (float*)nullptr, reinterpret_cast<unsigned*>(sum_ws));
+             (const float*)nullptr, 0.0f, (float*)nullptr, (float*)nullptr, (float*)nullptr, reinterpret_cast<unsigned*>(sum_ws),
+             (unsigned*)nullptr);
   if (int rc = check_launch("nerf_composite_mse_bwd"); rc != NERF_OK) return rc;
   return finish_sums(sum_ws, grid.x, loss_accum, nullptr, amax_accum, stream);
+}
+
+extern "C" int nerf_composite_mse_bwd_fused(const float* rgb, const float* sigma, const int* slot_of_sample, const float* z,
+                                            const float* rays_d, const float* bg, int64_t bg_rows, const float* target,
+                                            float loss_weight, int64_t n_rays, int n_samples, float* pred_out, float* loss_out,
+                                            float* d_rgb, float* d_sigma, float* amax_out, float* sum_ws, uint32_t* ticket,
+                                            nerf_stream_t stream) {
+  NERF_REQUIRE(n_rays >= 1 && n_samples >= 1 && n_samples <= 64 * kMaxPerLane,
+               "nerf_composite_mse_bwd_fused: n_rays=%lld n_samples=%d (max %d)", (long long)n_rays, n_samples, 64 * kMaxPerLane);
+  NERF_REQUIRE(rgb && sigma && z && rays_d && target && loss_out && d_rgb && d_sigma && sum_ws && ticket,
+               "nerf_composite_mse_bwd_fused: NULL pointer");
+  NERF_REQUIRE(bg == nullptr || bg_rows == 1 || bg_rows == n_rays, "nerf_composite_mse_bwd_fused: bg_rows=%lld", (long long)bg_rows);
+  const dim3 grid((unsigned)mse_blocks(n_rays, true));
+  DISPATCH_K(per_lane(n_samples), composite_mse_bwd_kernel, rgb, sigma, z, rays_d, bg, bg_rows, target, loss_weight,
+             slot_of_sample, n_rays, n_samples, pred_out, loss_out, d_rgb, d_sigma, amax_out,
+             (const float*)nullptr, 0.0f, (float*)nullptr, (float*)nullptr, (float*)nullptr, reinterpret_cast<unsigned*>(sum_ws),
+             reinterpret_cast<unsigned*>(ticket));
+  return check_launch("nerf_composite_mse_bwd_fused");
 }
 
 extern "C" int nerf_composite_mse_reg_bwd(const float* rgb, const float* sigma, const int* slot_of_sample, const float* z,
@@ -499,7 +546,7 @@
   const dim3 grid((unsigned)mse_blocks(n_rays, sum_ws != nullptr));
   DISPATCH_K(per_lane(n_samples), composite_mse_bwd_kernel, rgb, sigma, z, rays_d, bg, bg_rows, target, loss_weight,
              slot_of_sample, n_rays, n_samples, pred_out, loss_accum, d_rgb, d_sigma, (float*)nullptr, extra, reg_weight, d_extra,
-             reg_accum, extra_map, reinterpret_cast<unsigned*>(sum_ws));
+             reg_accum, extra_map, reinterpret_cast<unsigned*>(sum_ws), (unsigned*)nullptr);
   if (int rc = check_launch("nerf_composite_mse_reg_bwd"); rc != NERF_OK) return rc;
   return finish_sums(sum_ws, grid.x, loss_accum, reg_accum, nullptr, stream);
 }
diff --git a/project-nerf_amd/csrc/mlp_bwd.hip b/project-nerf_amd/csrc/mlp_bwd.hip
--- a/project-nerf_amd/csrc/mlp_bwd.hip
+++ b/project-nerf_amd/csrc/mlp_bwd.hip
@@ -1,5 +1,7 @@
 #include "mlp_chain.h"
 #include "mlp_stash.h"
+#include "mlp_wgrad.h"
+#include <math.h>
 
 namespace nerf {
 using namespace plan;
@@ -205,7 +207,8 @@
 using namespace nerf;
 
 int nerf_launch_wgrad(const char* stash, const StashLayout& sl, const char* work, const BwdLayout& bl,
-                      int64_t n, float* grads, int part, hipStream_t stream, size_t zero_lo, size_t zero_hi);
+                      int64_t n, float* grads, int part, hipStream_t stream, size_t zero_lo, size_t zero_hi,
+                      const WgradTail* tail);
 
 extern "C" size_t nerf_mlp_bwd_workspace_bytes(int64_t n) { return n > 0 ? bwd_layout(n).total : 0; }
 
@@ -255,7 +258,7 @@
 }
 
 static int launch_wgrad(const void* stash, const void* workspace, int64_t n, float* grads_f32, int part,
-                        nerf_stream_t stream) {
+                        nerf_stream_t stream, const WgradTail* tail = nullptr) {
   NERF_REQUIRE(grads_f32 != nullptr, "nerf_mlp_bwd: grads_f32 is NULL");
   NERF_REQUIRE(part >= 0 && part <= 2, "nerf_mlp_bwd_wgrad_part: part=%d (0 all, 1 late layers, 2 early layers)", part);
   const size_t lo = part == 1 ? (size_t)plan::kW4 : 0, hi = part == 2 ? (size_t)plan::kW4 : (size_t)plan::kParamCount;
@@ -266,7 +269,7 @@
   }
   NERF_REQUIRE(stash && workspace, "nerf_mlp_bwd: NULL pointer");
   return nerf_launch_wgrad(static_cast<const char*>(stash), stash_layout(n), static_cast<const char*>(workspace),
-                           bwd_layout(n), n, grads_f32, part, as_stream(stream), lo, hi);
+                           bwd_layout(n), n, grads_f32, part, as_stream(stream), lo, hi, tail);
 }
 
 extern "C" int nerf_mlp_bwd_dgrad(const void* packed, const void* stash, const float* rgb, const float* sigma,
@@ -293,6 +296,24 @@
 extern "C" int nerf_mlp_bwd_wgrad_part(const void* stash, const void* workspace, int64_t n, float* grads_f32, int part,
                                        nerf_stream_t stream) {
   return launch_wgrad(stash, workspace, n, grads_f32, part, stream);
+}
+
+extern "C" int nerf_mlp_bwd_wgrad_adam(const void* stash, const void* workspace, int64_t n, float* grads_f32, float* params_f32,
+                                       float* exp_avg, float* exp_avg_sq, void* packed, int step, float lr, float beta1, float beta2,
+                                       float eps, nerf_stream_t stream) {
+  NERF_REQUIRE(n >= 0 && step >= 1, "nerf_mlp_bwd_wgrad_adam: n=%lld step=%d", (long long)n, step);
+  NERF_REQUIRE(grads_f32 && params_f32 && exp_avg && exp_avg_sq && packed, "nerf_mlp_bwd_wgrad_adam: NULL pointer");
+  NERF_REQUIRE(((uintptr_t)packed & 255) == 0, "nerf_mlp_bwd_wgrad_adam: packed buffer must be 256-byte aligned");
+  if (n == 0 || stash_layout(n).fp8 || options().wgrad_only >= 0) {
+    if (int rc = launch_wgrad(stash, workspace, n, grads_f32, 0, stream); rc != NERF_OK) return rc;
+    if (int rc = nerf_adam_step(params_f32, grads_f32, exp_avg, exp_avg_sq, plan::kParamCount, step, lr, beta1, beta2, eps, 0.0f, nullptr,
+                                stream); rc != NERF_OK) return rc;
+    return nerf_mlp_pack_streams(params_f32, packed, 1, stream);
+  }
+  const double bc1 = 1.0 - pow((double)beta1, step), bc2 = 1.0 - pow((double)beta2, step);
+  const WgradTail tail = {params_f32, exp_avg, exp_avg_sq, static_cast<char*>(packed), lr, beta1, beta2, eps,
+                          (float)(1.0 / bc1), (float)(1.0 / sqrt(bc2))};
+  return launch_wgrad(stash, workspace, n, grads_f32, 0, stream, &tail);
 }
 
 extern "C" int nerf_mlp_bwd(const void* packed, const void* stash, const float* rgb, const float* sigma,
diff --git a/project-nerf_amd/csrc/mlp_pack.hip b/project-nerf_amd/csrc/mlp_pack.hip
--- a/project-nerf_amd/csrc/mlp_pack.hip
+++ b/project-nerf_amd/csrc/mlp_pack.hip
@@ -1,48 +1,9 @@
 #include "common.h"
 #include "mlp_plan.h"
+#include "mlp_pack_index.h"
 
 namespace nerf {
 using namespace plan;
-
-struct FragTable {
-  int v[kFwdFrags + kBwdFrags];
-};
-
-constexpr FragTable make_frag_table() {
-  FragTable t{};
-  int f = 0;
-  for (int kind = 0; kind < kNumKinds; ++kind) {
-    const int ks = step_ks(kind);
-    for (int m = 0; m < step_of(kind).mt; ++m)
-      for (int k = 0; k < ks; ++k) t.v[f++] = (kind << 16) | (m << 8) | k;
-  }
-  return t;
-}
-__constant__ FragTable g_frag_table = make_frag_table();
-
-__device__ __forceinline__ int src_index(int kind, int row, int k, bool nat) {
-  if (kind <= F_PTS7) {
-    const int l = kind;
-    const int in_dim = pts_in_dim(l);
-    int col;
-    if (l == 0) col = k < 63 ? k : -1;
-    else if (l == 4) col = nat ? (k < 63 ? 256 + k : -1) : k;
-    else col = k;
-    return col < 0 ? -1 : pts_weight_off(l) + row * in_dim + col;
-  }
-  switch (kind) {
-    case F_HEAD: return row < 256 ? kWFeat + row * 256 + k : (row == 256 ? kWSigma + k : -1);
-    case F_VIEW: return nat ? (k < 27 ? kWView + row * 283 + 256 + k : -1) : kWView + row * 283 + k;
-    case F_RGB: return row < 3 ? kWRgb + row * 128 + k : -1;
-    case B_RGB: return k < 3 ? kWRgb + k * 128 + row : -1;
-    case B_VIEW: return kWView + k * 283 + row;
-    case B_HEAD: return nat ? (k == 0 ? kWSigma + row : -1) : kWFeat + k * 256 + row;
-    default: {
-      const int l = 7 - (kind - B_PTS7);
-      return pts_weight_off(l) + k * pts_in_dim(l) + row;
-    }
-  }
-}
 
 __global__ void __launch_bounds__(256) pack16_kernel(const float* __restrict__ params, __bf16* __restrict__ packed_fwd16) {
   const int total = kFwdFrags * 64;
@@ -73,18 +34,11 @@
   for (int t = blockIdx.x * blockDim.x + threadIdx.x; t < total; t += gridDim.x * blockDim.x) {
     const int frag = t >> 6, lane = t & 63;
     const int desc = g_frag_table.v[frag];
-    const int kind = desc >> 16, mt = (desc >> 8) & 0xFF, ks = desc & 0xFF;
-    const Step st = step_of(kind);
-    const int row = mt * 32 + (lane & 31), h = lane >> 5;
-    const bool nat = ks >= st.ks_acc;
     typedef __bf16 bf16x8 __attribute__((ext_vector_type(8)));
     bf16x8 out;
 #pragma unroll
     for (int j = 0; j < 8; ++j) {
-      int k;
-      if (nat) k = 16 * (ks - st.ks_acc) + 8 * h + j;
-      else k = 32 * (ks >> 1) + 16 * (ks & 1) + 8 * (j >> 2) + 4 * h + (j & 3);
-      const int src = src_index(kind, row, k, nat);
+      const int src = frag_elem_src(desc, lane, j);
       out[j] = (__bf16)(src >= 0 ? params[src] : 0.0f);
     }
     __bf16* dst = frag < kFwdFrags ? packed_fwd + (size_t)frag * 512 : packed_bwd + (size_t)(frag - kFwdFrags) * 512;
diff --git a/project-nerf_amd/csrc/mlp_pack_index.h b/project-nerf_amd/csrc/mlp_pack_index.h
--- /dev/null
+++ b/project-nerf_amd/csrc/mlp_pack_index.h
@@ -0,0 +1,60 @@
+#pragma once
+#include <hip/hip_runtime.h>
+#include "mlp_plan.h"
+
+namespace nerf {
+
+struct FragTable {
+  int v[plan::kFwdFrags + plan::kBwdFrags];
+};
+
+constexpr FragTable make_frag_table() {
+  using namespace plan;
+  FragTable t{};
+  int f = 0;
+  for (int kind = 0; kind < kNumKinds; ++kind) {
+    const int ks = step_ks(kind);
+    for (int m = 0; m < step_of(kind).mt; ++m)
+      for (int k = 0; k < ks; ++k) t.v[f++] = (kind << 16) | (m << 8) | k;
+  }
+  return t;
+}
+static __constant__ FragTable g_frag_table = make_frag_table();
+
+__host__ __device__ __forceinline__ int src_index(int kind, int row, int k, bool nat) {
+  using namespace plan;
+  if (kind <= F_PTS7) {
+    const int l = kind;
+    const int in_dim = pts_in_dim(l);
+    int col;
+    if (l == 0) col = k < 63 ? k : -1;
+    else if (l == 4) col = nat ? (k < 63 ? 256 + k : -1) : k;
+    else col = k;
+    return col < 0 ? -1 : pts_weight_off(l) + row * in_dim + col;
+  }
+  switch (kind) {
+    case F_HEAD: return row < 256 ? kWFeat + row * 256 + k : (row == 256 ? kWSigma + k : -1);
+    case F_VIEW: return nat ? (k < 27 ? kWView + row * 283 + 256 + k : -1) : kWView + row * 283 + k;
+    case F_RGB: return row < 3 ? kWRgb + row * 128 + k : -1;
+    case B_RGB: return k < 3 ? kWRgb + k * 128 + row : -1;
+    case B_VIEW: return kWView + k * 283 + row;
+    case B_HEAD: return nat ? (k == 0 ? kWSigma + row : -1) : kWFeat + k * 256 + row;
+    default: {
+      const int l = 7 - (kind - B_PTS7);
+      return pts_weight_off(l) + k * pts_in_dim(l) + row;
+    }
+  }
+}
+
+__host__ __device__ __forceinline__ int frag_elem_src(int desc, int lane, int j) {
+  const int kind = desc >> 16, mt = (desc >> 8) & 0xFF, ks = desc & 0xFF;
+  const plan::Step st = plan::step_of(kind);
+  const int row = mt * 32 + (lane & 31), h = lane >> 5;
+  const bool nat = ks >= st.ks_acc;
+  int k;
+  if (nat) k = 16 * (ks - st.ks_acc) + 8 * h + j;
+  else k = 32 * (ks >> 1) + 16 * (ks & 1) + 8 * (j >> 2) + 4 * h + (j & 3);
+  return src_index(kind, row, k, nat);
+}
+
+}
diff --git a/project-nerf_amd/csrc/mlp_wgrad.h b/project-nerf_amd/csrc/mlp_wgrad.h
--- a/project-nerf_amd/csrc/mlp_wgrad.h
+++ b/project-nerf_amd/csrc/mlp_wgrad.h
@@ -50,8 +50,16 @@
   int debug;
 };
 
+struct WgradTail {
+  float* params;
+  float* exp_avg;
+  float* exp_avg_sq;
+  char* packed;
+  float lr, beta1, beta2, eps, inv_bc1, inv_sqrt_bc2;
+};
+int wgrad_tail_launch(const WgradArgs& args, const WgradTail& tail, hipStream_t stream);
 
 int wgrad_launch(WgradArgs& args, int64_t n_samples, float* grads, hipStream_t stream, float* slab = nullptr,
-                 size_t slab_bytes = 0, size_t zero_lo = 0, size_t zero_hi = 0);
+                 size_t slab_bytes = 0, size_t zero_lo = 0, size_t zero_hi = 0, const WgradTail* tail = nullptr);
 
 }
diff --git a/project-nerf_amd/csrc/mlp_wgrad.hip b/project-nerf_amd/csrc/mlp_wgrad.hip
--- a/project-nerf_amd/csrc/mlp_wgrad.hip
+++ b/project-nerf_amd/csrc/mlp_wgrad.hip
@@ -671,8 +671,9 @@
 using namespace nerf;
 
 int nerf_launch_wgrad(const char* stash, const StashLayout& sl, const char* work, const BwdLayout& bl,
-                      int64_t n, float* grads, int part, hipStream_t stream, size_t zero_lo, size_t zero_hi) {
+                      int64_t n, float* grads, int part, hipStream_t stream, size_t zero_lo, size_t zero_hi, const WgradTail* tail) {
   WgradArgs args{};
+  if (tail != nullptr && (part != 0 || sl.fp8)) return fail(NERF_EINVAL, "nerf_mlp_bwd_wgrad_adam: the fused tail takes the whole bf16 step");
   const size_t np = (size_t)sl.n_pad, eb = sl.fp8 ? 1 : 2;
   if (sl.fp8 != bl.fp8) return fail(NERF_EINVAL, "nerf_mlp_bwd: stash and workspace disagree on the image width");
   args.amax = sl.fp8 ? reinterpret_cast<const float*>(work + bl.amax) : nullptr;
@@ -745,12 +746,13 @@
   }
   args.n_jobs = nj;
   float* slab = bl.slab_bytes ? reinterpret_cast<float*>(const_cast<char*>(work) + bl.slab) : nullptr;
-  return wgrad_launch(args, n, grads, stream, slab, bl.slab_bytes, zero_lo, zero_hi);
+  return wgrad_launch(args, n, grads, stream, slab, bl.slab_bytes, zero_lo, zero_hi, tail);
 }
 
 int nerf::wgrad_launch(WgradArgs& args, int64_t n, float* grads, hipStream_t stream, float* slab, size_t slab_bytes,
-                       size_t zero_lo, size_t zero_hi) {
+                       size_t zero_lo, size_t zero_hi, const WgradTail* tail) {
   int nj = args.n_jobs;
+  if (tail != nullptr && options().wgrad_only >= 0) return fail(NERF_EINVAL, "wgrad: option wgrad_only keeps one job, the fused tail needs all");
   const int overhead = options().wgrad_overhead;
   for (int j = 0; j < nj; ++j) {
     WgradJob& jb = args.jobs[j];
@@ -796,6 +798,7 @@
     small = small && jb.kind >= 6 && jb.a_bytes <= SmallStage::A && jb.b_acc_bytes <= SmallStage::B && jb.b_nat_bytes <= SmallStageP4::N;
   }
   if (p4 && !small) return fail(NERF_EINVAL, "wgrad: Part 4 job kinds run on the small-stage kernel only");
+  if (small && tail != nullptr) return fail(NERF_EINVAL, "wgrad: the fused tail belongs to the decoder's jobs");
   long long want = (long long)args.wave_tiles * nj / 4;
   if (options().wgrad_grid > 0 && options().wgrad_grid < n_cu) n_cu = options().wgrad_grid;
   int grid = (int)(want < 1 ? 1 : (want > n_cu ? n_cu : want));
@@ -852,6 +855,10 @@
   }
   if (fp8) hipLaunchKernelGGL(mlp_wgrad_kernel<true>, dim3(grid), dim3(512), kWgLds + kWgScratch, stream, args);
   else hipLaunchKernelGGL(mlp_wgrad_kernel<false>, dim3(grid), dim3(512), kWgLds + kWgScratch, stream, args);
+  if (tail != nullptr) {
+    if (int rc = check_launch("nerf_mlp_bwd (wgrad)"); rc != NERF_OK) return rc;
+    return wgrad_tail_launch(args, *tail, stream);
+  }
   if (args.slab != nullptr) {
     if (int rc = check_launch("nerf_mlp_bwd (wgrad)"); rc != NERF_OK) return rc;
     hipLaunchKernelGGL(wgrad_reduce_kernel, dim3(160, args.n_jobs), dim3(256), 0, stream, args);
diff --git a/project-nerf_amd/csrc/wgrad_tail.hip b/project-nerf_amd/csrc/wgrad_tail.hip
--- /dev/null
+++ b/project-nerf_amd/csrc/wgrad_tail.hip
@@ -0,0 +1,100 @@
+#include "common.h"
+#include "adam_update.h"
+#include "mlp_pack_index.h"
+#include "mlp_wgrad.h"
+#include "wgrad_tail_plan.h"
+
+namespace nerf {
+using namespace plan;
+
+__global__ void __launch_bounds__(256) wgrad_tail_kernel(const WgradArgs args, const WgradTail tl) {
+  __shared__ __bf16 tile[32][34];
+  const tail::Unit un = tail::unit_of(blockIdx.x);
+  const WgradJob& job = args.jobs[un.job];
+  const tail::JobShape js = {job.o_valid, job.w_ld, job.w_off, job.bias_off, job.n2, job.w2_off, job.bias2_off};
+  const int t = threadIdx.x;
+  const int rounds = un.region == tail::kWeights ? 4 : (un.region == tail::kSecond ? 1 : 2);
+  tail::Elem el[4];
+#pragma unroll
+  for (int q = 0; q < 4; ++q) el[q] = tail::elem_of(un, t + 256 * q, js);
+
+  float g[4];
+  if (args.slab != nullptr) {
+    const float* part = args.slab + job.slab_off;
+    float s[4][4];
+#pragma unroll
+    for (int q = 0; q < 4; ++q) s[q][0] = s[q][1] = s[q][2] = s[q][3] = 0.0f;
+    int p = 0;
+    for (; p + 4 <= job.n_parts; p += 4) {
+#pragma unroll
+      for (int u = 0; u < 4; ++u)
+#pragma unroll
+        for (int q = 0; q < 4; ++q)
+          if (q < rounds) s[q][u] += part[(long long)(p + u) * job.p_stride + el[q].tile_idx];
+    }
+    for (; p < job.n_parts; ++p)
+#pragma unroll
+      for (int q = 0; q < 4; ++q)
+        if (q < rounds) s[q][0] += part[(long long)p * job.p_stride + el[q].tile_idx];
+#pragma unroll
+    for (int q = 0; q < 4; ++q) {
+      g[q] = (s[q][0] + s[q][1]) + (s[q][2] + s[q][3]);
+      if (el[q].ok) args.grads[el[q].param] = g[q];
+    }
+  } else {
+#pragma unroll
+    for (int q = 0; q < 4; ++q) g[q] = el[q].ok ? args.grads[el[q].param] : 0.0f;
+  }
+
+  float* __restrict__ bias = reinterpret_cast<float*>(tl.packed + kPackBiasOff);
+#pragma unroll
+  for (int q = 0; q < 4; ++q) {
+    float pe = 0.0f;
+    if (el[q].ok) {
+      const int i = el[q].param;
+      pe = tl.params[i];
+      float me = tl.exp_avg[i], ve = tl.exp_avg_sq[i];
+      adam_update(pe, g[q], me, ve, tl.lr, tl.beta1, tl.beta2, tl.eps, 0.0f, tl.inv_bc1, tl.inv_sqrt_bc2);
+      tl.exp_avg[i] = me;
+      tl.exp_avg_sq[i] = ve;
+      tl.params[i] = pe;
+      if (un.region == tail::kBias) bias[tail::bias_slot(un, t + 256 * q)] = pe;
+    }
+    if (un.region != tail::kBias && q < rounds) tile[el[q].r][el[q].c] = (__bf16)pe;
+  }
+  if (un.region == tail::kBias) return;
+  __syncthreads();
+
+  int frag[4];
+  const int n_frag = tail::dest_frags(un, frag);
+  const int d = t >> 6, lane = t & 63;
+  if (d >= n_frag) return;
+  const int f = frag[d], desc = g_frag_table.v[f];
+  typedef __bf16 bf16x8 __attribute__((ext_vector_type(8)));
+  bf16x8 out;
+#pragma unroll
+  for (int j = 0; j < 8; ++j) {
+    const int src = frag_elem_src(desc, lane, j);
+    const int pos = src >= 0 ? tail::tile_pos(un, src, js) : -1;
+    out[j] = pos >= 0 ? tile[pos >> 5][pos & 31] : (__bf16)0.0f;
+  }
+  __bf16* dst = f < kFwdFrags ? reinterpret_cast<__bf16*>(tl.packed + kPackFwdOff) + (size_t)f * 512
+                              : reinterpret_cast<__bf16*>(tl.packed + kPackBwdOff) + (size_t)(f - kFwdFrags) * 512;
+  *reinterpret_cast<bf16x8*>(dst + lane * 8) = out;
+}
+
+int wgrad_tail_launch(const WgradArgs& args, const WgradTail& tl, hipStream_t stream) {
+  bool ok = args.n_jobs == tail::kJobs;
+  for (int j = 0; ok && j < tail::kJobs; ++j) {
+    const WgradJob& jb = args.jobs[j];
+    ok = jb.o_row0 == 0 && (jb.ones || jb.bias_nat_col >= 0) && (jb.o_valid + 31) / 32 == tail::row_tiles(j) &&
+         (jb.w_ld + 31) / 32 == tail::col_tiles(j) && (jb.n2 != 0) == (j == tail::kHeadJob);
+  }
+  ok = ok && args.jobs[0].w_off == kW0 && args.jobs[4].w_off == kW4 && args.jobs[tail::kHeadJob].w_off == kWFeat &&
+       args.jobs[tail::kHeadJob].w2_off == kWSigma && args.jobs[tail::kViewJob].w_off == kWView && args.jobs[tail::kRgbJob].w_off == kWRgb;
+  if (!ok) return fail(NERF_EINVAL, "wgrad tail: not the job table of the bf16 decoder step");
+  hipLaunchKernelGGL(wgrad_tail_kernel, dim3(tail::kUnits), dim3(256), 0, stream, args, tl);
+  return check_launch("nerf_mlp_bwd_wgrad_adam (tail)");
+}
+
+}
diff --git a/project-nerf_amd/csrc/wgrad_tail_plan.h b/project-nerf_amd/csrc/wgrad_tail_plan.h
--- /dev/null
+++ b/project-nerf_amd/csrc/wgrad_tail_plan.h
@@ -0,0 +1,106 @@
+#pragma once
+#include <hip/hip_runtime.h>
+#include "mlp_plan.h"
+
+namespace nerf {
+namespace tail {
+
+constexpr int kJobs = 11, kHeadJob = 8, kViewJob = 9, kRgbJob = 10;
+__host__ __device__ constexpr int row_tiles(int job) { return job <= kHeadJob ? 8 : (job == kViewJob ? 4 : 1); }
+__host__ __device__ constexpr int col_tiles(int job) {
+  return job == 0 ? 2 : (job == 4 ? 10 : (job <= kHeadJob ? 8 : (job == kViewJob ? 9 : 4)));
+}
+constexpr int weight_units() {
+  int n = 0;
+  for (int j = 0; j < kJobs; ++j) n += row_tiles(j) * col_tiles(j);
+  return n;
+}
+constexpr int kWeightUnits = weight_units(), kSigmaUnits = 8, kBiasUnits = kJobs;
+constexpr int kUnits = kWeightUnits + kSigmaUnits + kBiasUnits;
+static_assert(kWeightUnits == 584 && kUnits == 603, "unit count");
+
+enum Region : int { kWeights = 0, kSecond = 1, kBias = 2 };
+struct Unit { int job, region, a, b; };
+
+__host__ __device__ inline Unit unit_of(int u) {
+  if (u >= kWeightUnits + kSigmaUnits) return {u - kWeightUnits - kSigmaUnits, kBias, 0, 0};
+  if (u >= kWeightUnits) return {kHeadJob, kSecond, 0, u - kWeightUnits};
+  int job = 0;
+  for (; u >= row_tiles(job) * col_tiles(job); ++job) u -= row_tiles(job) * col_tiles(job);
+  return {job, kWeights, u / col_tiles(job), u % col_tiles(job)};
+}
+
+__host__ __device__ constexpr int fwd_kind(int job) {
+  return job < 8 ? job : (job == kHeadJob ? (int)plan::F_HEAD : (job == kViewJob ? (int)plan::F_VIEW : (int)plan::F_RGB));
+}
+__host__ __device__ constexpr int bwd_kind(int job) {
+  return job == 0 ? -1 : (job < 8 ? (int)plan::B_PTS7 + (7 - job)
+                                  : (job == kHeadJob ? (int)plan::B_HEAD : (job == kViewJob ? (int)plan::B_VIEW : (int)plan::B_RGB)));
+}
+__host__ __device__ constexpr int stream_frag(int kind, int mt, int ks) {
+  return (kind >= plan::B_RGB ? plan::kFwdFrags : 0) + plan::step_frag0(kind) + mt * plan::step_ks(kind) + ks;
+}
+
+__host__ __device__ inline int dest_frags(const Unit& un, int (&frag)[4]) {
+  using namespace plan;
+  int n = 0;
+  if (un.region == kBias) return 0;
+  if (un.region == kSecond) {
+    frag[n++] = stream_frag(F_HEAD, 8, 2 * un.b);
+    frag[n++] = stream_frag(F_HEAD, 8, 2 * un.b + 1);
+    frag[n++] = stream_frag(B_HEAD, un.b, step_of(B_HEAD).ks_acc);
+    return n;
+  }
+  const int F = fwd_kind(un.job), B = bwd_kind(un.job);
+  const int ks0 = un.b < 8 ? 2 * un.b : step_of(F).ks_acc + 2 * (un.b - 8);
+  for (int d = 0; d < 2; ++d)
+    if (ks0 + d < step_ks(F)) frag[n++] = stream_frag(F, un.a, ks0 + d);
+  if (B >= 0 && un.b < 8) {
+    if (B == B_RGB) frag[n++] = stream_frag(B, un.b, 0);
+    else {
+      frag[n++] = stream_frag(B, un.b, 2 * un.a);
+      frag[n++] = stream_frag(B, un.b, 2 * un.a + 1);
+    }
+  }
+  return n;
+}
+
+struct JobShape { int o_valid, w_ld, w_off, bias_off, n2, w2_off, bias2_off; };
+struct Elem { int tile_idx, param, r, c; bool ok; };
+__host__ __device__ inline Elem elem_of(const Unit& un, int e, const JobShape& js) {
+  const int n_w = js.o_valid * js.w_ld, n_b = n_w + js.o_valid;
+  Elem el{0, 0, e >> 5, e & 31, false};
+  if (un.region == kWeights) {
+    const int o = 32 * un.a + el.r, col = 32 * un.b + el.c;
+    el.ok = o < js.o_valid && col < js.w_ld;
+    el.tile_idx = o * js.w_ld + col;
+    el.param = js.w_off + el.tile_idx;
+  } else if (un.region == kSecond) {
+    el.ok = e < 32;
+    el.tile_idx = n_b + 32 * un.b + e;
+    el.param = js.w2_off + 32 * un.b + e;
+  } else if (e < js.o_valid) {
+    el.ok = true;
+    el.tile_idx = n_w + e;
+    el.param = js.bias_off + e;
+  } else if (e == js.o_valid && js.n2 > 0) {
+    el.ok = true;
+    el.tile_idx = n_b + js.n2 - 1;
+    el.param = js.bias2_off;
+  }
+  if (!el.ok) el.tile_idx = el.param = 0;
+  return el;
+}
+__host__ __device__ inline int bias_slot(const Unit& un, int e) { return plan::bias_off(fwd_kind(un.job)) + e; }
+__host__ __device__ inline int tile_pos(const Unit& un, int src, const JobShape& js) {
+  int r = 0, c;
+  if (un.region == kWeights) {
+    const int rel = src - js.w_off, o = rel / js.w_ld;
+    r = o - 32 * un.a;
+    c = rel - o * js.w_ld - 32 * un.b;
+  } else c = src - js.w2_off - 32 * un.b;
+  return (r >= 0 && r < 32 && c >= 0 && c < 32) ? 32 * r + c : -1;
+}
+
+}
+}
diff --git a/project-nerf_amd/engine.py b/project-nerf_amd/engine.py
--- a/project-nerf_amd/engine.py
+++ b/project-nerf_amd/engine.py
@@ -65,7 +65,8 @@
         self.world_size = world_size
         self.grad_scale = torch.full((1,), 1.0 / world_size, device=self.device)
         self._ws: Dict[Tuple[str, int], Tensor] = {}
-        self._scalars = torch.zeros(2, 1024, device=self.device)
+        self._scalars = torch.zeros(1, device=self.device)
+        self._ticket = torch.zeros(1, dtype=torch.int32, device=self.device)
         self.repack()
 
     def repack(self, training_only: bool = False) -> None:
@@ -91,10 +92,7 @@
             self._ws[key] = torch.empty(nbytes, dtype=torch.uint8, device=self.device)
         return self._ws[key]
 
-    def compute_gradients(self, rays_o: Tensor, rays_d: Tensor, target: Tensor, n_samples: int = 64,
-                   u: Optional[Tensor] = None, sync_grads=None, sync_grads_async=None, mark=None,
-                   z: Optional[Tensor] = None) -> Tensor:
-        mark = mark or (lambda name: None)
+    def _forward_loss(self, rays_o: Tensor, rays_d: Tensor, target: Tensor, n_samples: int, u, mark, z):
         R = rays_o.shape[0]
         n = R * n_samples
         if z is None:
@@ -105,24 +103,28 @@
         stash = self._buf("stash", ops.mlp_stash_bytes(n))
         rgb, sigma = ops.mlp_fwd(self.packed, rays_o, rays_d, z, stash)
         mark("fwd")
-        self._grad_calls = getattr(self, "_grad_calls", -1) + 1
-        slot = self._grad_calls % self._scalars.shape[1]
-        if slot == 0:
-            self._scalars.zero_()
-        loss, amax = self._scalars[0, slot:slot + 1], self._scalars[1, slot:slot + 1]
-        d_rgb, d_sigma, _ = ops.composite_mse_bwd(rgb.view(R, n_samples, 3), sigma.view(R, n_samples), z, rays_d, self.bg,
-                                                  target, loss, amax_accum=amax)
+        loss = torch.empty((), device=self.device)
+        d_rgb, d_sigma, _ = ops.composite_mse_bwd_fused(rgb.view(R, n_samples, 3), sigma.view(R, n_samples), z, rays_d, self.bg,
+                                                        target, loss, self._ticket, amax_out=self._scalars)
         mark("loss")
+        return stash, rgb, sigma, d_rgb.view(n, 3), d_sigma.view(n), loss, n
+
+    def compute_gradients(self, rays_o: Tensor, rays_d: Tensor, target: Tensor, n_samples: int = 64,
+                   u: Optional[Tensor] = None, sync_grads=None, sync_grads_async=None, mark=None,
+                   z: Optional[Tensor] = None) -> Tensor:
+        mark = mark or (lambda name: None)
+        stash, rgb, sigma, d_rgb, d_sigma, loss, n = self._forward_loss(rays_o, rays_d, target, n_samples, u, mark, z)
+        amax = self._scalars
         if sync_grads_async is not None:
-            ops.mlp_bwd_overlapped(self.packed, stash, rgb, sigma, d_rgb.view(n, 3), d_sigma.view(n), self.grads,
+            ops.mlp_bwd_overlapped(self.packed, stash, rgb, sigma, d_rgb, d_sigma, self.grads,
                                    self._buf("bwd", ops.mlp_bwd_workspace_bytes(n)), sync_grads_async, amax=amax, mark=mark)
         else:
-            ops.mlp_bwd(self.packed, stash, rgb, sigma, d_rgb.view(n, 3), d_sigma.view(n), self.grads,
+            ops.mlp_bwd(self.packed, stash, rgb, sigma, d_rgb, d_sigma, self.grads,
                         self._buf("bwd", ops.mlp_bwd_workspace_bytes(n)), amax=amax, mark=mark)
         mark("wgrad")
         if sync_grads is not None:
             sync_grads(self.grads)
-        return loss[0].clone()
+        return loss
 
     def apply_gradients(self) -> None:
         self.step_count += 1
@@ -133,11 +135,21 @@
     def train_step(self, rays_o: Tensor, rays_d: Tensor, target: Tensor, n_samples: int = 64,
                    u: Optional[Tensor] = None, sync_grads=None, sync_grads_async=None, mark=None,
                    z: Optional[Tensor] = None) -> Tensor:
-        loss = self.compute_gradients(rays_o, rays_d, target, n_samples, u=u, sync_grads=sync_grads,
-                                      sync_grads_async=sync_grads_async, mark=mark, z=z)
-        self.apply_gradients()
-        if mark is not None:
-            mark("adam+pack")
+        if self.world_size != 1 or sync_grads is not None or sync_grads_async is not None:
+            loss = self.compute_gradients(rays_o, rays_d, target, n_samples, u=u, sync_grads=sync_grads,
+                                          sync_grads_async=sync_grads_async, mark=mark, z=z)
+            self.apply_gradients()
+            if mark is not None:
+                mark("adam+pack")
+            return loss
+        mark = mark or (lambda name: None)
+        stash, rgb, sigma, d_rgb, d_sigma, loss, n = self._forward_loss(rays_o, rays_d, target, n_samples, u, mark, z)
+        self.step_count += 1
+        ops.mlp_bwd_adam(self.packed, stash, rgb, sigma, d_rgb, d_sigma, self.grads, self._buf("bwd", ops.mlp_bwd_workspace_bytes(n)),
+                         self._scalars, self.params, self.exp_avg, self.exp_avg_sq, self.step_count, self.lr, mark=mark)
+        self._infer_stale = True
+        mark("wgrad")
+        mark("adam+pack")
         return loss
 
     @torch.no_grad()
diff --git a/project-nerf_amd/ops.py b/project-nerf_amd/ops.py
--- a/project-nerf_amd/ops.py
+++ b/project-nerf_amd/ops.py
@@ -404,6 +404,30 @@
     return d_rgb, d_sigma, pred
 
 
+def composite_mse_bwd_fused(rgb: Tensor, sigma: Tensor, z: Tensor, rays_d: Tensor, bg: Optional[Tensor], target: Tensor,
+                            loss_out: Tensor, ticket: Tensor, slots: Optional[Tensor] = None, amax_out: Optional[Tensor] = None,
+                            loss_weight: Optional[float] = None, want_pred: bool = False):
+    lib = _lib.load()
+    rgb, sigma, z, rays_d, target = _dev(rgb, "rgb"), _dev(sigma, "sigma"), _dev(z, "z"), _dev(rays_d, "rays_d"), _dev(target, "target")
+    R, S = z.shape
+    bg_rows = 0
+    if bg is not None:
+        bg = _dev(bg, "bg")
+        bg_rows = 1 if bg.dim() == 1 else bg.shape[0]
+    for t, nm in ((loss_out, "loss_out"), (amax_out, "amax_out")):
+        if t is not None and (t.dtype != torch.float32 or t.numel() != 1 or t.device != z.device):
+            raise ValueError(f"{nm} must be one float32 element on the inputs' device")
+    if ticket.dtype != torch.int32 or ticket.numel() != 1 or ticket.device != z.device:
+        raise ValueError("ticket must be one int32 element on the inputs' device")
+    d_rgb, d_sigma = torch.empty_like(rgb), torch.empty_like(sigma)
+    pred = torch.empty(R, 3, device=z.device) if want_pred else None
+    w = 1.0 / (3 * R) if loss_weight is None else loss_weight
+    _lib.check(lib.nerf_composite_mse_bwd_fused(_p(rgb), _p(sigma), _p(slots), _p(z), _p(rays_d), _p(bg), bg_rows, _p(target), w, R, S,
+                                                _p(pred), _p(loss_out), _p(d_rgb), _p(d_sigma), _p(amax_out),
+                                                _p(sum_ws(z.device)), _p(ticket), _stream()), "nerf_composite_mse_bwd_fused")
+    return d_rgb, d_sigma, pred
+
+
 class _Composite(torch.autograd.Function):
 
     @staticmethod
@@ -512,6 +536,24 @@
             mark("dgrad")
         _lib.check(lib.nerf_mlp_bwd_wgrad(_p(stash), _p(workspace), n, _p(grads), _stream()), "nerf_mlp_bwd_wgrad")
     return grads
+
+
+def mlp_bwd_adam(packed: Tensor, stash: Tensor, rgb: Tensor, sigma: Tensor, d_rgb: Tensor, d_sigma: Tensor, grads: Tensor,
+                 workspace: Tensor, amax: Tensor, params: Tensor, exp_avg: Tensor, exp_avg_sq: Tensor, step: int, lr: float,
+                 beta1: float = 0.9, beta2: float = 0.999, eps: float = 1e-8, mark=None) -> None:
+    lib = _lib.load()
+    rgb, sigma = _dev(rgb, "rgb"), _dev(sigma, "sigma")
+    d_rgb, d_sigma = _dev(d_rgb, "d_rgb"), _dev(d_sigma, "d_sigma")
+    for t, nm in ((params, "params"), (grads, "grads"), (exp_avg, "exp_avg"), (exp_avg_sq, "exp_avg_sq")):
+        if _dev(t, nm) is not t or t.numel() != MLP_PARAM_COUNT or t.dtype != torch.float32:
+            raise ValueError(f"{nm} must be a contiguous float32 tensor of {MLP_PARAM_COUNT} elements")
+    n = sigma.numel()
+    _lib.check(lib.nerf_mlp_bwd_dgrad_ex(_p(packed), _p(stash), _p(rgb), _p(sigma), _p(d_rgb), _p(d_sigma), n,
+                                         _p(workspace), _p(amax), _stream()), "nerf_mlp_bwd_dgrad_ex")
+    if mark is not None:
+        mark("dgrad")
+    _lib.check(lib.nerf_mlp_bwd_wgrad_adam(_p(stash), _p(workspace), n, _p(grads), _p(params), _p(exp_avg), _p(exp_avg_sq),
+                                           _p(packed), step, lr, beta1, beta2, eps, _stream()), "nerf_mlp_bwd_wgrad_adam")
 
 
 def mlp_bwd_overlapped(packed: Tensor, stash: Tensor, rgb: Tensor, sigma: Tensor, d_rgb: Tensor, d_sigma: Tensor,
```

After: 3.831 million rays/s. -2.3%, worse.
